# navi0105/LyricAlignment

Measured on AMD Instinct MI355X. Metric: aligned audio-sec/sec (RTF^-1), Whisper-medium 30 s clips, higher is better.
Workload: dtype bf16; 1 GPU; whisper-medium encoder + BiGRU/FC head + CTC forced alignment, batch 32 x 30 s mel per GPU (BASELINE.json configs[1]); clips_per_gpu=32, frames=1500, vocab=21129, labels_per_clip=5..26 (one per sung note), pipeline=2 encoder stream(s) + 1 head stream, head over 4 batches

## Files before the change

include/lyricalign.h:

```cpp
#ifndef LYRICALIGN_H
#define LYRICALIGN_H

#include <stddef.h>
#include <stdint.h>

#ifdef __cplusplus
extern "C" {
#endif

typedef enum la_status {
    LA_OK = 0,
    LA_EINVAL = 1,
    LA_EINFEASIBLE = 2,
    LA_EEMPTY = 3,
    LA_EHIP = 4,
    LA_ETIMEOUT = 5,
    LA_EUNSUPPORTED = 6
} la_status;

typedef enum la_dtype {
    LA_F32 = 0,
    LA_BF16 = 1,
    LA_F16 = 2
} la_dtype;

#define LA_Q_LOG2 0x100


typedef enum la_variant {
    LA_VARIANT_PLAIN = 0,
    LA_VARIANT_CTC = 1
} la_variant;

int la_version(void);
const char *la_last_error(void);
int la_device_arch_ok(void);

int la_timer_enable(const char *name);
int la_timer_disable(void);
int la_timer_read(double *total_ms, int64_t *launches);
int la_timer_reset(void);
int la_timer_sample(int32_t period);
int la_timer_read_work(double *total_ms, int64_t *timed_launches, double *timed_work, int64_t *all_launches);

int la_set_option(const char *name, int64_t value);
int la_get_option(const char *name, int64_t *value);
int la_has_experiments(void);

int la_viterbi_workspace_bytes(int32_t batch, int32_t max_frames, int32_t max_labels, size_t *bytes);

int la_viterbi_batch(const float *em, int64_t em_batch_stride, int64_t em_row_stride,
                     const int32_t *labels, int32_t labels_stride,
                     const int32_t *n_labels, const int32_t *n_frames,
                     int32_t batch, int32_t max_frames, int32_t max_labels,
                     int32_t *onset, int32_t *offset, int32_t out_stride,
                     double *final_score, int32_t *status,
                     void *workspace, size_t workspace_bytes, void *stream);

int la_viterbi_core(const float *em, int64_t em_row_stride, const int32_t *labels, int32_t n_labels_host,
                    int32_t n_frames_host, const int32_t *n_labels, const int32_t *n_frames,
                    double *dp, long long *bt, int32_t *scratch_i32, double *scratch_f64,
                    void *workspace, size_t workspace_bytes, void *stream);

int la_viterbi_spans_workspace_bytes(int32_t batch, int32_t max_frames, int32_t max_labels, size_t *bytes);

int la_viterbi_spans_batch(const float *em, int64_t em_batch_stride, int64_t em_row_stride,
                           const int32_t *labels, int32_t labels_stride,
                           const int32_t *n_labels, const int32_t *n_frames,
                           int32_t batch, int32_t max_frames, int32_t max_labels,
                           int32_t *onset, int32_t *offset, int32_t out_stride,
                           double *final_score, int32_t *status,
                           const int32_t *skip_from, int32_t skip_stride, double skip_penalty,
                           void *workspace, size_t workspace_bytes, void *stream);

int la_viterbi_windows_workspace_bytes(int32_t batch, int32_t max_frames, int32_t max_labels, size_t *bytes);

int la_viterbi_windows_batch(const float *em, int64_t em_batch_stride, int64_t em_row_stride,
                             const int32_t *labels, int32_t labels_stride,
                             const int32_t *n_labels, const int32_t *n_frames,
// ... 166 lines not shown
                               int32_t vocab, const int32_t *labels, int32_t labels_stride, const int32_t *n_labels,
                               const int32_t *n_frames, int32_t max_labels, const int32_t *skip_from, int32_t skip_stride,
                               double skip_penalty, const int32_t *win_lo, const int32_t *win_hi, int32_t win_stride, float scale,
                               float *loss, double *nll, int32_t *status, float *dlogits, int64_t d_batch_stride,
                               int64_t d_row_stride, void *workspace, size_t workspace_bytes, void *stream);

int la_grad_sqnorm_f32(const float *grad, int64_t n, double *sum_sq, void *stream);
int la_adamw_step_f32(float *param, const float *grad, float *exp_avg, float *exp_avg_sq, int64_t n, float lr,
                      float beta1, float beta2, float eps, float weight_decay, int32_t step,
                      const double *clip_sum_sq, float max_norm, float grad_prescale, void *stream);

int la_gru_layer_train_fwd(const float *gi, const float *w_hh, const float *b_hh, float *out, float *gates,
                           int32_t batch, int32_t frames, int32_t hidden, void *workspace, size_t workspace_bytes,
                           int32_t *timeout_flag, void *stream);
int la_gru_layer_bwd(const float *gates, const float *out, const float *dout, const float *w_hh, float *dgi, float *dgh,
                     int32_t batch, int32_t frames, int32_t hidden, void *workspace, size_t workspace_bytes,
                     int32_t *timeout_flag, void *stream);
int la_transpose_pad_f32(const float *in, int64_t ld_in, int32_t rows, int32_t cols, float *out, int64_t ld_out,
                         int32_t out_rows, int32_t out_cols, void *stream);
int la_colsum_f32(const float *in, int64_t ld, int32_t rows, int32_t cols, float *out, void *stream);
int la_mish_f32(const float *x, float *y, int64_t n, void *stream);
int la_mish_bwd_f32(const float *x, const float *dy, float *dx, int64_t n, void *stream);
int la_mask_scale_f32(const float *x, const unsigned char *mask, float scale, float *y, int64_t n, void *stream);

int la_gemm_fused_ln(int32_t dtype, int32_t M, int32_t N, int32_t K, int32_t batch, const void *A, int64_t lda, int64_t strideA,
                     const void *W, void *C, int64_t ldc, int64_t strideC, const float *bias, const float *residual, int64_t ldr,
                     int64_t strideR, int32_t epilogue, void *C2, int64_t ldc2, int64_t strideC2, const float *ln_stats,
                     const float *ln_csum, float *ln_part, void *stream);
int la_gemm_split(int32_t dtype, int32_t M, int32_t N, int32_t K, int32_t batch, const void *A, int64_t lda, int64_t strideA,
                  const void *W, void *hi, void *lo, int64_t ld, int64_t stride, const float *bias, const float *residual,
                  int64_t ldr, int64_t strideR, int32_t epilogue, float *ln_part, void *stream);
int la_layernorm_split(int32_t dtype, const void *hi, const void *lo, int64_t ldx, int32_t M, int32_t d, const float *gamma,
                       const float *beta, void *y, int64_t ldy, int32_t out_dtype, void *stream);
int la_ln_stats_finalize(const float *part, int32_t slots, int32_t M, float eps, float *stats, void *stream);
int la_row_stats16(int32_t dtype, const void *x, int64_t ldx, int32_t M, int32_t d, float eps, float *stats, void *stream);

int la_split_f16x2(const float *x, int64_t ldx, int32_t rows, int32_t cols, void *planes, int64_t kp, float *inv_scale, void *stream);
int la_split_f16x2_t(const float *x, int64_t ldx, int32_t rows, int32_t cols, void *planes_t, int64_t mp, float *inv_scale_t, void *stream);
int la_split_f16x2_act(const float *x, int64_t ldx, int32_t rows, int32_t cols, void *planes, int64_t kp, float *inv_scale, int32_t act, void *stream);
int la_split_f16x2_t_act(const float *x, int64_t ldx, int32_t rows, int32_t cols, void *planes_t, int64_t mp, float *inv_scale_t, int32_t act, void *stream);
int la_split_f16x2_t_colsum(const float *x, int64_t ldx, int32_t rows, int32_t cols, void *planes_t, int64_t mp, float *inv_scale_t, int32_t act,
                            float *colsum, void *stream);
int la_split_f16x2_max(const float *x, int64_t ldx, int32_t rows, int32_t cols, void *planes, int64_t kp, float *inv_scale, int32_t act,
                       uint32_t *tmax, void *stream);
int la_split_f16x2_t_tmax(const float *x, int64_t ldx, int32_t rows, int32_t cols, void *planes_t, int64_t mp, float *inv_scale_t, int32_t act,
                          float *colsum, const uint32_t *tmax, void *stream);
int la_gemm_f16x2(int32_t M, int32_t N, int32_t K, int32_t slots, const void *A, const float *sa, const void *W, const float *sw,
                  float *C, int64_t ldc, const float *bias, const float *residual, int64_t ldr, int32_t epilogue, void *stream);
int la_gemm_f16x2_small(int32_t M, int32_t N, int32_t K, int32_t slots, const void *A, const float *sa, const void *W, const float *sw,
                        float *C, int64_t ldc, const float *bias, const float *residual, int64_t ldr, int32_t epilogue, void *stream);
int la_gemm_f16x2_small_slots(int32_t M, int32_t N, int32_t K);
int la_layernorm_f16x2(const float *x, int64_t ldx, int32_t rows, int32_t d, const float *gamma, const float *beta, void *planes, int64_t kp,
                       float *inv_scale, void *stream);

int la_gemm_ex(int32_t dtype, int32_t M, int32_t N, int32_t K, int32_t batch, const void *A, int64_t lda, int64_t strideA,
               const void *W, int64_t ldw, int64_t strideW, void *C, int64_t ldc, int64_t strideC, const float *bias,
               int32_t epilogue, void *stream);
int la_transpose_pad_batched_f32(const float *in, int64_t ld_in, int64_t batch_stride_in, int32_t rows, int32_t cols,
                                 float *out, int64_t ld_out, int64_t batch_stride_out, int32_t out_rows, int32_t out_cols,
                                 int32_t batch, void *stream);
int la_gelu_f32(const float *x, float *y, int64_t n, void *stream);
int la_gelu_bwd_f32(const float *x, const float *dy, float *dx, int64_t n, void *stream);
int la_add_f32(const float *a, const float *b, float *y, int64_t n, void *stream);
int la_scale_f32(const float *x, float alpha, float *y, int64_t n, void *stream);
int la_layernorm_bwd_f32(const float *x, const float *dy, const float *gamma, int32_t M, int32_t d, float *dx, float *dy_xhat,
                         void *stream);
int la_layernorm_bwd_sums_f32(const float *x, const float *dy, const float *gamma, const float *residual, int32_t M, int32_t d, float *dx,
                              float *dgamma, float *dbeta, float *scratch, void *stream);
int la_softmax_rows_f32(float *s, int64_t ld, int64_t rows, int32_t cols, int32_t causal_q_len, void *stream);
int la_softmax_bwd_rows_f32(const float *p, float *dp, int64_t ld, int64_t rows, int32_t cols, void *stream);
int la_attention_bwd_workspace_bytes(int32_t batch, int32_t q_len, int32_t n_head, size_t *bytes);
int la_attention_bwd_f32(const float *q, int64_t ld_q, const float *k, const float *v, int64_t ld_kv, const float *o, int64_t ld_o,
                         const float *dout, int64_t ld_do, float *dq, int64_t ld_dq, float *dk, float *dv, int64_t ld_dkv,
                         int32_t batch, int32_t q_len, int32_t kv_len, int32_t n_head, int32_t causal, const float *lse,
                         void *workspace, size_t workspace_bytes, void *stream);
int la_attention_bwd_stats_f32(const float *q, int64_t ld_q, const float *k, int64_t ld_kv, const float *o, int64_t ld_o, const float *dout,
                               int64_t ld_do, int32_t batch, int32_t q_len, int32_t kv_len, int32_t n_head, int32_t causal,
                               const float *lse_in, float *lse, float *dvec, void *stream);
int la_attention_lse_f32(const float *q, int64_t ld_q, const float *k, const float *v, int64_t ld_kv, float *out, int64_t ld_out,
                         int32_t batch, int32_t q_len, int32_t kv_len, int32_t n_head, int32_t causal, float *lse, void *stream);
int la_attention_f16x2_workspace_bytes(int32_t batch, int32_t q_len, int32_t kv_len, int32_t n_head, size_t *bytes);
int la_attention_lse_f16x2(const float *q, int64_t ld_q, const float *k, const float *v, int64_t ld_kv, float *out, int64_t ld_out,
                           int32_t batch, int32_t q_len, int32_t kv_len, int32_t n_head, int32_t causal, float *lse, void *workspace,
                           size_t workspace_bytes, void *stream);
int la_attention_bwd_f16x2_workspace_bytes(int32_t batch, int32_t q_len, int32_t kv_len, int32_t n_head, size_t *bytes);
int la_attention_bwd_f16x2(const float *q, int64_t ld_q, const float *k, const float *v, int64_t ld_kv, const float *o, int64_t ld_o,
                           const float *dout, int64_t ld_do, float *dq, int64_t ld_dq, float *dk, float *dv, int64_t ld_dkv,
                           int32_t batch, int32_t q_len, int32_t kv_len, int32_t n_head, int32_t causal, const float *lse,
                           void *workspace, size_t workspace_bytes, void *stream);
int la_embed_tokens_bwd_f32(const float *dx, const int64_t *tokens, int32_t batch, int32_t n, int32_t d, int32_t n_vocab, float *dtok,
                            float *dpos, void *stream);
int la_cross_entropy_f32(const float *logits, int64_t ld, int32_t rows, int32_t vocab, const int64_t *target, float scale,
                         float *loss2, float *row_ws, float *dlogits, int64_t ld_d, void *stream);
int la_col2im3_f32(const float *dcols, int32_t batch, int32_t t_out, int32_t stride, int32_t channels, float *out,
                   int32_t rows_out, void *stream);

int la_resample_poly_f32(const float *x, int64_t n_in, const float *h, int64_t h_len, int32_t up, int32_t down,
                         int64_t skip, float *y, int64_t n_out, void *stream);

int la_cast_f32_to_bf16(const float *x, void *y, int64_t n, void *stream);
int la_cast_bf16_to_f32(const void *x, float *y, int64_t n, void *stream);

typedef struct la_encoder_block {
    const float *ln1_g, *ln1_b;
    const void *wqkv; const float *bqkv;
    const void *wo; const float *bo;
    const float *ln2_g, *ln2_b;
    const void *w1; const float *b1;
    const void *w2; const float *b2;
    const void *wqkv_ln; const float *cqkv, *bqkv_ln;
    const void *w1_ln; const float *c1, *b1_ln;
    const void *wqkv_x2; const float *wqkv_x2s;
    const void *wo_x2; const float *wo_x2s;
    const void *w1_x2; const float *w1_x2s;
    const void *w2_x2; const float *w2_x2s;
} la_encoder_block;

typedef struct la_encoder_weights {
    int32_t dtype, d, n_head, n_layer, n_mels;
    const void *conv1_w; const float *conv1_b;
    const void *conv2_w; const float *conv2_b;
    const float *pos;
    const float *lnp_g, *lnp_b;
    const la_encoder_block *blocks;
} la_encoder_weights;

int la_encoder_workspace_bytes(const la_encoder_weights *w, int32_t batch, size_t *bytes);
int la_encoder_forward(const la_encoder_weights *w, const float *mel, int64_t mel_batch_stride, int64_t mel_row_stride,
                       int32_t batch, void *out, int64_t ld_out, int32_t out_dtype, void *workspace, size_t workspace_bytes,
                       void *stream);

typedef struct la_head_weights {
    int32_t dtype, hidden, in_dim, vocab, n_layers;
    const void *w_ih[2]; const float *b_ih[2];
    const void *w_hh[2]; const float *b_hh[2];
    const void *w_fc; const float *b_fc;
    const void *w_ih_x2[2]; const float *w_ih_x2s[2];
    const void *w_fc_x2; const float *w_fc_x2s;
} la_head_weights;

int la_align_head_workspace_bytes(const la_head_weights *w, int32_t batch, int32_t frames, int32_t max_labels, size_t *bytes);
int la_align_head_forward(const la_head_weights *w, const void *feats, int64_t ld_feats, int64_t clip_stride_rows,
                          int32_t batch, int32_t frames, int32_t variant, const int32_t *labels, int32_t labels_stride,
                          const int32_t *n_labels, int32_t max_labels, int32_t *onset, int32_t *offset, int32_t out_stride,
                          double *final_score, int32_t *status, float *emissions_out, void *workspace, size_t workspace_bytes,
                          int32_t *timeout_flag, void *stream);
int la_align_head_forward_ragged(const la_head_weights *w, const void *feats, int64_t ld_feats, int64_t clip_stride_rows,
                                 int32_t batch, int32_t frames, const int32_t *n_frames, int32_t variant, const int32_t *labels,
                                 int32_t labels_stride, const int32_t *n_labels, int32_t max_labels, int32_t *onset, int32_t *offset,
                                 int32_t out_stride, double *final_score, int32_t *status, float *emissions_out, void *workspace,
                                 size_t workspace_bytes, int32_t *timeout_flag, void *stream);

#ifdef __cplusplus
}
#endif
#endif
```

lyricalignment_amd/_lib.py:

```python
from __future__ import annotations

import ctypes
import os
from ctypes import POINTER, c_char_p, c_double, c_int32, c_int64, c_size_t, c_void_p

import torch

HERE = os.path.dirname(os.path.abspath(__file__))
LIB_PATH = os.environ.get("LA_LIB_PATH") or os.path.join(HERE, "liblyricalign_hip.so")

LA_OK, LA_EINVAL, LA_EINFEASIBLE, LA_EEMPTY, LA_EHIP, LA_ETIMEOUT, LA_EUNSUPPORTED = range(7)
LA_F32, LA_BF16, LA_F16 = 0, 1, 2
LA_Q_LOG2 = 0x100
LA_VARIANT_PLAIN, LA_VARIANT_CTC = 0, 1
EPI_BIAS, EPI_GELU, EPI_RESIDUAL, EPI_OUT_F32, EPI_MISH = 1, 2, 4, 8, 16
EPI_GELU_ERF = 4096
EPI_RES_GELU_GRAD = 32
GEMM_TRANS_A, GEMM_TRANS_W = 512, 1024

_I32, _I64, _P, _SZ = c_int32, c_int64, c_void_p, c_size_t
SYMBOLS = {
    "la_version": (c_int32, []),
    "la_last_error": (c_char_p, []),
    "la_device_arch_ok": (c_int32, []),
    "la_timer_enable": (c_int32, [c_char_p]),
    "la_timer_disable": (c_int32, []),
    "la_timer_read": (c_int32, [POINTER(c_double), POINTER(c_int64)]),
    "la_timer_reset": (c_int32, []),
    "la_timer_sample": (c_int32, [c_int32]),
    "la_timer_read_work": (c_int32, [POINTER(c_double), POINTER(c_int64), POINTER(c_double), POINTER(c_int64)]),
    "la_split_f16x2": (c_int32, [_P, _I64, _I32, _I32, _P, _I64, _P, _P]),
    "la_split_f16x2_t": (c_int32, [_P, _I64, _I32, _I32, _P, _I64, _P, _P]),
    "la_split_f16x2_act": (c_int32, [_P, _I64, _I32, _I32, _P, _I64, _P, _I32, _P]),
    "la_split_f16x2_t_act": (c_int32, [_P, _I64, _I32, _I32, _P, _I64, _P, _I32, _P]),
    "la_split_f16x2_t_colsum": (c_int32, [_P, _I64, _I32, _I32, _P, _I64, _P, _I32, _P, _P]),
    "la_split_f16x2_max": (c_int32, [_P, _I64, _I32, _I32, _P, _I64, _P, _I32, _P, _P]),
    "la_split_f16x2_t_tmax": (c_int32, [_P, _I64, _I32, _I32, _P, _I64, _P, _I32, _P, _P, _P]),
    "la_gemm_f16x2": (c_int32, [_I32, _I32, _I32, _I32, _P, _P, _P, _P, _P, _I64, _P, _P, _I64, _I32, _P]),
    "la_gemm_f16x2_small": (c_int32, [_I32, _I32, _I32, _I32, _P, _P, _P, _P, _P, _I64, _P, _P, _I64, _I32, _P]),
    "la_gemm_f16x2_small_slots": (c_int32, [_I32, _I32, _I32]),
    "la_layernorm_f16x2": (c_int32, [_P, _I64, _I32, _I32, _P, _P, _P, _I64, _P, _P]),
    "la_fc_emissions_x2_workspace_bytes": (c_int32, [_I32, _I32, _I32, _I32, _I32, POINTER(_SZ)]),
    "la_fc_emissions_x2": (c_int32, [_P, _I64, _P, _P, _P, _P, _I32, _I32, _I32, _I32, _I32, _P, _I32, _P, _I32, _P, _I64, _I64, _P, _SZ, _P]),
    "la_set_option": (c_int32, [c_char_p, c_int64]),
    "la_get_option": (c_int32, [c_char_p, POINTER(c_int64)]),
    "la_has_experiments": (c_int32, []),
    "la_viterbi_workspace_bytes": (c_int32, [_I32, _I32, _I32, POINTER(_SZ)]),
    "la_viterbi_batch": (c_int32, [_P, _I64, _I64, _P, _I32, _P, _P, _I32, _I32, _I32, _P, _P, _I32, _P, _P, _P, _SZ, _P]),
    "la_viterbi_core": (c_int32, [_P, _I64, _P, _I32, _I32, _P, _P, _P, _P, _P, _P, _P, _SZ, _P]),
    "la_viterbi_spans_workspace_bytes": (c_int32, [_I32, _I32, _I32, POINTER(_SZ)]),
    "la_viterbi_spans_batch": (c_int32, [_P, _I64, _I64, _P, _I32, _P, _P, _I32, _I32, _I32, _P, _P, _I32, _P, _P, _P, _I32, c_double,
                                         _P, _SZ, _P]),
    "la_viterbi_windows_workspace_bytes": (c_int32, [_I32, _I32, _I32, POINTER(_SZ)]),
    "la_viterbi_windows_batch": (c_int32, [_P, _I64, _I64, _P, _I32, _P, _P, _I32, _I32, _I32, _P, _P, _I32, _P, _P, _P, _I32, c_double,
                                           _P, _P, _I32, _P, _SZ, _P]),
    "la_viterbi_lattice_workspace_bytes": (c_int32, [_I32, _I32, _I32, POINTER(_SZ)]),
    "la_viterbi_lattice_batch": (c_int32, [_P, _I64, _I64, _P, _I32, _P, _P, _I32, _I32, _I32, _P, _P, _I32, _P, _P, _P, _I32, c_double,
                                           _P, _P, _I32, _P, _SZ, _P]),
    "la_alignment_posteriors_workspace_bytes": (c_int32, [_I32, _I32, _I32, POINTER(_SZ)]),
    "la_alignment_posteriors": (c_int32, [_P, _I64, _I64, _P, _I32, _P, _P, _I32, _I32, _I32, _P, _P, _I32, _I32, _P, _P, _P, _P, _P,
                                          _P, _I64, _I64, _P, _SZ, _P]),
    "la_alignment_posteriors_spans_workspace_bytes": (c_int32, [_I32, _I32, _I32, POINTER(_SZ)]),
    "la_alignment_posteriors_spans": (c_int32, [_P, _I64, _I64, _P, _I32, _P, _P, _I32, _I32, _I32, _P, _P, _I32, _I32, _P, _I32, c_double,
                                                _P, _P, _P, _P, _P, _P, _P, _P, _I64, _I64, _P, _SZ, _P]),
    "la_alignment_posteriors_windows_workspace_bytes": (c_int32, [_I32, _I32, _I32, POINTER(_SZ)]),
    "la_alignment_posteriors_windows": (c_int32, [_P, _I64, _I64, _P, _I32, _P, _P, _I32, _I32, _I32, _P, _P, _I32, _I32, _P, _I32, c_double,
                                                  _P, _P, _I32, _P, _P, _P, _P, _P, _P, _P, _P, _I64, _I64, _P, _SZ, _P]),
    "la_emissions_from_logits": (c_int32, [_P, _I64, _I64, _I32, _I32, _I32, _I32, _P, _I32, _P, _I32, _P, _I64, _I64, _P]),
    "la_logmel_workspace_bytes": (c_int32, [_I32, _I32, POINTER(_SZ)]),
    "la_logmel_f32": (c_int32, [_P, _I32, _I32, _P, _P, _P, _I64, _I64, _P, _SZ, _P]),
    "la_logmel_constants_bytes": (c_int32, [POINTER(_SZ)]),
    "la_logmel_constants": (c_int32, [_P, _P, _P, _SZ, _P]),
    "la_logmel_f32_prepared": (c_int32, [_P, _I32, _I32, _P, _P, _I64, _I64, _P, _SZ, _P]),
    "la_gemm": (c_int32, [_I32, _I32, _I32, _I32, _I32, _P, _I64, _I64, _P, _P, _I64, _I64, _P, _P, _I64, _I64, _I32, _P]),
    "la_layernorm": (c_int32, [_P, _I64, _I32, _I32, _P, _P, _P, _I64, _I32, _P]),
    "la_attention": (c_int32, [_I32, _P, _I64, _P, _I64, _I32, _I32, _I32, _P]),
    "la_attention_ex": (c_int32, [_I32, _P, _I64, _P, _P, _I64, _P, _I64, _I32, _I32, _I32, _I32, _I32, _P]),
    "la_embed_tokens": (c_int32, [_P, _I32, _I32, _P, _I32, _P, _I32, _P, _P]),
    "la_mel_to_rows": (c_int32, [_P, _I64, _I64, _I32, _I32, _I32, _P, _I32, _I32, _P]),
    "la_gru_workspace_bytes": (c_int32, [_I32, _I32, _I32, POINTER(_SZ)]),
    "la_gru_layer": (c_int32, [_I32, _P, _P, _P, _P, _P, _I32, _I32, _I32, _P, _SZ, _P, _P]),
    "la_fc_emissions_workspace_bytes": (c_int32, [_I32, _I32, _I32, _I32, _I32, _I32, POINTER(_SZ)]),
    "la_fc_emissions": (c_int32, [_I32, _P, _I64, _P, _P, _I32, _I32, _I32, _I32, _I32, _P, _I32, _P, _I32, _P, _I64, _I64, _P, _SZ, _P]),
    "la_multitask_loss_workspace_bytes": (c_int32, [_I32, _I32, _I32, POINTER(_SZ)]),
    "la_multitask_loss": (c_int32, [_P, _I64, _I64, _I32, _I32, _I32, _P, _P, _I32, _P, _I32, _I32, _I32, ctypes.c_float, _P, _P, _I64, _I64, _P, _SZ, _P]),
    "la_anchored_alignment_loss_workspace_bytes": (c_int32, [_I32, _I32, _I32, POINTER(_SZ)]),
    "la_anchored_alignment_loss": (c_int32, [_P, _I64, _I64, _I32, _I32, _I32, _P, _I32, _P, _P, _I32, _P, _I32, c_double, _P, _P, _I32,
                                             ctypes.c_float, _P, _P, _P, _P, _I64, _I64, _P, _SZ, _P]),
    "la_grad_sqnorm_f32": (c_int32, [_P, _I64, _P, _P]),
    "la_adamw_step_f32": (c_int32, [_P, _P, _P, _P, _I64, ctypes.c_float, ctypes.c_float, ctypes.c_float, ctypes.c_float, ctypes.c_float, _I32, _P, ctypes.c_float, ctypes.c_float, _P]),
    "la_gru_layer_train_fwd": (c_int32, [_P, _P, _P, _P, _P, _I32, _I32, _I32, _P, _SZ, _P, _P]),
    "la_gru_layer_bwd": (c_int32, [_P, _P, _P, _P, _P, _P, _I32, _I32, _I32, _P, _SZ, _P, _P]),
    "la_transpose_pad_f32": (c_int32, [_P, _I64, _I32, _I32, _P, _I64, _I32, _I32, _P]),
    "la_colsum_f32": (c_int32, [_P, _I64, _I32, _I32, _P, _P]),
# ... 9 lines not shown
    "la_gemm_split": (c_int32, [_I32, _I32, _I32, _I32, _I32, _P, _I64, _I64, _P, _P, _P, _I64, _I64, _P, _P, _I64, _I64, _I32, _P, _P]),
    "la_layernorm_split": (c_int32, [_I32, _P, _P, _I64, _I32, _I32, _P, _P, _P, _I64, _I32, _P]),
    "la_row_stats16": (c_int32, [_I32, _P, _I64, _I32, _I32, ctypes.c_float, _P, _P]),
    "la_gemm_ex": (c_int32, [_I32, _I32, _I32, _I32, _I32, _P, _I64, _I64, _P, _I64, _I64, _P, _I64, _I64, _P, _I32, _P]),
    "la_transpose_pad_batched_f32": (c_int32, [_P, _I64, _I64, _I32, _I32, _P, _I64, _I64, _I32, _I32, _I32, _P]),
    "la_gelu_f32": (c_int32, [_P, _P, _I64, _P]),
    "la_gelu_bwd_f32": (c_int32, [_P, _P, _P, _I64, _P]),
    "la_add_f32": (c_int32, [_P, _P, _P, _I64, _P]),
    "la_scale_f32": (c_int32, [_P, ctypes.c_float, _P, _I64, _P]),
    "la_layernorm_bwd_f32": (c_int32, [_P, _P, _P, _I32, _I32, _P, _P, _P]),
    "la_layernorm_bwd_sums_f32": (c_int32, [_P, _P, _P, _P, _I32, _I32, _P, _P, _P, _P, _P]),
    "la_softmax_rows_f32": (c_int32, [_P, _I64, _I64, _I32, _I32, _P]),
    "la_attention_bwd_workspace_bytes": (c_int32, [_I32, _I32, _I32, POINTER(_SZ)]),
    "la_attention_bwd_stats_f32": (c_int32, [_P, _I64, _P, _I64, _P, _I64, _P, _I64, _I32, _I32, _I32, _I32, _I32, _P, _P, _P, _P]),
    "la_attention_bwd_f32": (c_int32, [_P, _I64, _P, _P, _I64, _P, _I64, _P, _I64, _P, _I64, _P, _P, _I64, _I32, _I32, _I32, _I32, _I32, _P, _P,
                                       _SZ, _P]),
    "la_attention_lse_f32": (c_int32, [_P, _I64, _P, _P, _I64, _P, _I64, _I32, _I32, _I32, _I32, _I32, _P, _P]),
    "la_attention_f16x2_workspace_bytes": (c_int32, [_I32, _I32, _I32, _I32, POINTER(_SZ)]),
    "la_attention_lse_f16x2": (c_int32, [_P, _I64, _P, _P, _I64, _P, _I64, _I32, _I32, _I32, _I32, _I32, _P, _P, _SZ, _P]),
    "la_attention_bwd_f16x2_workspace_bytes": (c_int32, [_I32, _I32, _I32, _I32, POINTER(_SZ)]),
    "la_attention_bwd_f16x2": (c_int32, [_P, _I64, _P, _P, _I64, _P, _I64, _P, _I64, _P, _I64, _P, _P, _I64, _I32, _I32, _I32, _I32, _I32, _P, _P,
                                         _SZ, _P]),
    "la_embed_tokens_bwd_f32": (c_int32, [_P, _P, _I32, _I32, _I32, _I32, _P, _P, _P]),
    "la_cross_entropy_f32": (c_int32, [_P, _I64, _I32, _I32, _P, ctypes.c_float, _P, _P, _P, _I64, _P]),
    "la_softmax_bwd_rows_f32": (c_int32, [_P, _P, _I64, _I64, _I32, _P]),
    "la_col2im3_f32": (c_int32, [_P, _I32, _I32, _I32, _I32, _P, _I32, _P]),
    "la_resample_poly_f32": (c_int32, [_P, _I64, _P, _I64, _I32, _I32, _I64, _P, _I64, _P]),
    "la_cast_f32_to_bf16": (c_int32, [_P, _P, _I64, _P]),
    "la_encoder_workspace_bytes": (c_int32, [_P, _I32, POINTER(_SZ)]),
    "la_encoder_forward": (c_int32, [_P, _P, _I64, _I64, _I32, _P, _I64, _I32, _P, _SZ, _P]),
    "la_align_head_workspace_bytes": (c_int32, [_P, _I32, _I32, _I32, POINTER(_SZ)]),
    "la_align_head_forward": (c_int32, [_P, _P, _I64, _I64, _I32, _I32, _I32, _P, _I32, _P, _I32, _P, _P, _I32, _P, _P, _P, _P, _SZ, _P, _P]),
    "la_cast_bf16_to_f32": (c_int32, [_P, _P, _I64, _P]),
    "la_logmel_ragged_workspace_bytes": (c_int32, [_I32, _I32, POINTER(_SZ)]),
    "la_logmel_ragged_f32_prepared": (c_int32, [_P, _P, _I32, _I32, _P, _P, _I64, _I64, _I32, _P, _SZ, _P]),
    "la_gru_layer_ragged": (c_int32, [_I32, _P, _P, _P, _P, _P, _I32, _I32, _P, _I32, _P, _SZ, _P, _P]),
    "la_align_head_forward_ragged": (c_int32, [_P, _P, _I64, _I64, _I32, _I32, _P, _I32, _P, _I32, _P, _I32, _P, _P, _I32, _P, _P, _P, _P, _SZ, _P, _P]),
}

LAB_SYMBOLS = {}




class EncoderBlockC(ctypes.Structure):
    _fields_ = [(n, c_void_p) for n in ("ln1_g", "ln1_b", "wqkv", "bqkv", "wo", "bo", "ln2_g", "ln2_b", "w1", "b1", "w2", "b2",
                                        "wqkv_ln", "cqkv", "bqkv_ln", "w1_ln", "c1", "b1_ln",
                                        "wqkv_x2", "wqkv_x2s", "wo_x2", "wo_x2s", "w1_x2", "w1_x2s", "w2_x2", "w2_x2s")]


class EncoderWeightsC(ctypes.Structure):
    _fields_ = [("dtype", c_int32), ("d", c_int32), ("n_head", c_int32), ("n_layer", c_int32), ("n_mels", c_int32),
                ("conv1_w", c_void_p), ("conv1_b", c_void_p), ("conv2_w", c_void_p), ("conv2_b", c_void_p), ("pos", c_void_p),
                ("lnp_g", c_void_p), ("lnp_b", c_void_p), ("blocks", POINTER(EncoderBlockC))]


class HeadWeightsC(ctypes.Structure):
    _fields_ = [("dtype", c_int32), ("hidden", c_int32), ("in_dim", c_int32), ("vocab", c_int32), ("n_layers", c_int32),
                ("w_ih", c_void_p * 2), ("b_ih", c_void_p * 2), ("w_hh", c_void_p * 2), ("b_hh", c_void_p * 2),
                ("w_fc", c_void_p), ("b_fc", c_void_p),
                ("w_ih_x2", c_void_p * 2), ("w_ih_x2s", c_void_p * 2), ("w_fc_x2", c_void_p), ("w_fc_x2s", c_void_p)]


_lib = None


class LyricAlignHipError(RuntimeError):
    pass


def lib() -> ctypes.CDLL:
    global _lib
    if _lib is None:
        if not os.path.exists(LIB_PATH):
            raise LyricAlignHipError(
                f"{LIB_PATH} is missing: the HIP extension is the product path and has no fallback. "
                "Build it with `python -m lyricalignment_amd.build`.")
        L = ctypes.CDLL(LIB_PATH)
        for name, (res, args) in SYMBOLS.items():
            fn = getattr(L, name)
            fn.restype = res
            fn.argtypes = args
        if L.la_has_experiments():
            for name, (res, args) in LAB_SYMBOLS.items():
                fn = getattr(L, name)
                fn.restype = res
                fn.argtypes = args
        _lib = L
    return _lib


def last_error() -> str:
    msg = lib().la_last_error()
    return msg.decode() if msg else ""


def check(rc: int, what: str = "") -> None:
    if rc == LA_OK:
        return
    detail = f"{what}: {last_error()}" if what else last_error()
    if rc == LA_EINVAL:
        raise ValueError(f"liblyricalign_hip invalid argument: {detail}")
    if rc == LA_EUNSUPPORTED:
        raise NotImplementedError(f"liblyricalign_hip unsupported shape: {detail}")
    if rc == LA_ETIMEOUT:
        raise TimeoutError(f"liblyricalign_hip in-kernel wait timed out: {detail}")
    raise LyricAlignHipError(f"liblyricalign_hip status {rc}: {detail}")
# ... 57 lines not shown
```

lyricalignment_amd/csrc/la_attention_f16x2.hip:

```cpp
#include <type_traits>

#include "la_x2.h"

namespace {

typedef __attribute__((ext_vector_type(16))) float f32x16;
typedef __attribute__((ext_vector_type(8))) _Float16 f16x8;
typedef __attribute__((ext_vector_type(4))) short s16x4;
typedef __attribute__((ext_vector_type(8))) short s16x8;

#ifndef LA_X2F_KO
#define LA_X2F_KO 0
#endif
constexpr int KT = 64;
constexpr int IMG = KT * 128;
constexpr float kLog2e = 1.4426950408889634f;
constexpr float kLn2 = 0.6931471805599453f;

struct FwdParams {
    const unsigned short *qp, *kp, *vp;
    const float *sq, *sk, *sv;
    float *out;
    int64_t ld_out;
    float *lse;
    int q_len, kv_len, n_head, causal, batch;
};

__global__ __launch_bounds__(1024) void heads_split_kernel(const float *x, int64_t ld, int T, int H, unsigned short *planes, float *inv_scale) {
    __shared__ float red[16];
    const int head = blockIdx.x, clip = blockIdx.y, tid = threadIdx.x;
    const int c4 = tid & 15, r0 = tid >> 4;
    const float *src = x + (int64_t)clip * T * ld + head * 64 + c4 * 4;
    constexpr int NV = 24;
    const bool cached = T <= 64 * NV;
    float4 v[NV];
    float mx = 0.f;
    if (cached) {
#pragma unroll
        for (int j = 0; j < NV; ++j) {
            const int r = r0 + 64 * j;
            v[j] = make_float4(0.f, 0.f, 0.f, 0.f);
            if (r < T) v[j] = *reinterpret_cast<const float4 *>(src + (int64_t)r * ld);
        }
#pragma unroll
        for (int j = 0; j < NV; ++j) mx = fmaxf(mx, fmaxf(fmaxf(fabsf(v[j].x), fabsf(v[j].y)), fmaxf(fabsf(v[j].z), fabsf(v[j].w))));
    } else {
        for (int r = r0; r < T; r += 64) {
            const float4 w = *reinterpret_cast<const float4 *>(src + (int64_t)r * ld);
            mx = fmaxf(mx, fmaxf(fmaxf(fabsf(w.x), fabsf(w.y)), fmaxf(fabsf(w.z), fabsf(w.w))));
        }
    }
#pragma unroll
    for (int o = 1; o < 64; o <<= 1) mx = fmaxf(mx, __shfl_xor(mx, o));
    if ((tid & 63) == 0) red[tid >> 6] = mx;
    __syncthreads();
    mx = red[0];
#pragma unroll
    for (int i = 1; i < 16; ++i) mx = fmaxf(mx, red[i]);
    float inv;
    const float s = la::x2::scale_for(mx, &inv);
    if (tid == 0 && blockIdx.z == 0) inv_scale[clip * H + head] = inv;
    const int64_t C = 64 * (int64_t)H;
    const int parts = gridDim.z, part = blockIdx.z;
    unsigned short *dst = planes + (int64_t)clip * T * 2 * C + head * 64 + c4 * 4;
    auto put = [&](int r, const float4 &w) {
        const unsigned a = la::x2::pack_hi_lo(w.x * s), b = la::x2::pack_hi_lo(w.y * s), c = la::x2::pack_hi_lo(w.z * s), d = la::x2::pack_hi_lo(w.w * s);
        *reinterpret_cast<uint2 *>(dst + (int64_t)r * 2 * C) = make_uint2((a & 0xffffu) | (b << 16), (c & 0xffffu) | (d << 16));
        *reinterpret_cast<uint2 *>(dst + (int64_t)r * 2 * C + C) = make_uint2((a >> 16) | (b & 0xffff0000u), (c >> 16) | (d & 0xffff0000u));
    };
    if (cached) {
#pragma unroll
        for (int j = 0; j < NV; ++j) {
            const int r = r0 + 64 * j;
            if (r < T && j % parts == part) put(r, v[j]);
        }
    } else {
        for (int r = r0, j = 0; r < T; r += 64, ++j)
            if (j % parts == part) put(r, *reinterpret_cast<const float4 *>(src + (int64_t)r * ld));
// ... 2 lines not shown

struct BlockCoord { int qt, head, clip; };
__device__ __forceinline__ BlockCoord block_coord(int nq, int n_head, int batch) {
    const int L = blockIdx.x, pairs = n_head * batch;
    int pair, qt;
    if ((pairs & 7) == 0) {
        const int x = L & 7, idx = L >> 3;
        pair = x + 8 * (idx / nq);
        qt = idx % nq;
    } else {
        pair = L / nq;
        qt = L % nq;
    }
    return BlockCoord{qt, pair % n_head, pair / n_head};
}
__device__ __forceinline__ int acc_row(int reg, int h) { return (reg & 3) + 8 * (reg >> 2) + 4 * h; }
__device__ __forceinline__ int kswz(int r) { return (r >> 1) & 7; }
__device__ __forceinline__ int vswz(int r) { return ((r >> 1) & 1) << 2; }
__device__ __forceinline__ f32x16 mfma(f16x8 a, f16x8 b, f32x16 c) { return __builtin_amdgcn_mfma_f32_32x32x16_f16(a, b, c, 0, 0, 0); }

template <int PER> struct KvOff { unsigned k[PER], v[PER]; };
template <int PER>
__device__ __forceinline__ KvOff<PER> kv_offsets(int64_t C, int key0, int T, int wave, int lane) {
    KvOff<PER> o;
#pragma unroll
    for (int i = 0; i < PER; ++i) {
        const int r = (wave * PER + i) * 8 + (lane >> 3), ps = lane & 7;
        const int rr = key0 + r < T ? r : T - 1 - key0;
        o.k[i] = (unsigned)(rr * C * 4) + ((ps ^ kswz(r)) << 4);
        o.v[i] = (unsigned)(rr * C * 4) + ((ps ^ vswz(r)) << 4);
    }
    return o;
}
template <int PER>
__device__ __forceinline__ void stage_tile(const unsigned short *base, int64_t C, int key0, const unsigned (&off)[PER], unsigned buf, int wave) {
    const unsigned short *src = base + (int64_t)key0 * 2 * C;
#pragma unroll
    for (int i = 0; i < PER; ++i) {
        const unsigned piece = (wave * PER + i) * 1024;
        la::glds16_so(off[i], src, buf + piece);
        la::glds16_so(off[i], src + C, buf + IMG + piece);
    }
}

__device__ __forceinline__ void split_pair(float a, float b, unsigned &hi, unsigned &lo) {
    typedef _Float16 h2 __attribute__((ext_vector_type(2)));
    const h2 hv = {(_Float16)a, (_Float16)b};
    hi = __builtin_bit_cast(unsigned, hv);
    asm("s_nop 0\n\tv_fma_mixlo_f16 %0, %1, -1.0, %2 op_sel_hi:[1,0,0]\n\ts_nop 0\n\tv_fma_mixhi_f16 %0, %1, -1.0, %3 op_sel:[1,0,0] op_sel_hi:[1,0,0]\n\ts_nop 1"
        : "=&v"(lo)
        : "v"(hi), "v"(a), "v"(b));
}

template <int NW>
__global__ __launch_bounds__(64 * NW, 2) void attention_x2_fwd_kernel(FwdParams p) {
    constexpr int QT = 32 * NW, PER = 8 / NW;
    __shared__ __attribute__((aligned(16))) unsigned char lds[8 * IMG];
    const int T = p.kv_len;
    const int64_t C = 64 * (int64_t)p.n_head;
    const BlockCoord bc = block_coord((p.q_len + QT - 1) / QT, p.n_head, p.batch);
    const int qt = bc.qt, head = bc.head, clip = bc.clip;
    const int tid = threadIdx.x, lane = tid & 63;
    const int wave = __builtin_amdgcn_readfirstlane(tid >> 6);
    const int i32 = lane & 31, h = lane >> 5;
    const unsigned short *kbase = p.kp + (int64_t)clip * T * 2 * C + head * 64;
    const unsigned short *vbase = p.vp + (int64_t)clip * T * 2 * C + head * 64;
    const int bh = clip * p.n_head + head;
    const float kScale = p.sq[bh] * p.sk[bh] * kLog2e;

    int qrow = qt * QT + wave * 32 + i32;
    const bool q_valid = qrow < p.q_len;
    qrow = q_valid ? qrow : p.q_len - 1;
    uint4 qh[4], ql[4];
    {
        const unsigned short *qb = p.qp + ((int64_t)clip * p.q_len + qrow) * 2 * C + head * 64 + 8 * h;
#pragma unroll
        for (int c = 0; c < 4; ++c) {
            qh[c] = *reinterpret_cast<const uint4 *>(qb + 16 * c);
            ql[c] = *reinterpret_cast<const uint4 *>(qb + C + 16 * c);
        }
    }
    f32x16 o[2];
#pragma unroll
    for (int b = 0; b < 2; ++b)
#pragma unroll
        for (int r = 0; r < 16; ++r) o[b][r] = 0.f;
    float m_run = -INFINITY, l_part = 0.f;

    int nkv = (T + KT - 1) / KT;
    const int nkv_all = nkv;
    if (p.causal) nkv = min(nkv, (min(p.q_len, (qt + 1) * QT) - 1) / KT + 1);
    const unsigned lds0 = __builtin_amdgcn_readfirstlane(la::lds_addr_u32(lds));
    const KvOff<PER> off_full = kv_offsets<PER>(C, 0, KT, wave, lane);
    const KvOff<PER> off_last = kv_offsets<PER>(C, (nkv_all - 1) * KT, T, wave, lane);
    auto stage = [&](int t, unsigned buf) __attribute__((always_inline)) {
        stage_tile<PER>(kbase, C, t * KT, t == nkv_all - 1 ? off_last.k : off_full.k, buf, wave);
        stage_tile<PER>(vbase, C, t * KT, t == nkv_all - 1 ? off_last.v : off_full.v, buf + 2 * IMG, wave);
    };
    stage(0, lds0);
    asm volatile("s_waitcnt vmcnt(0)" ::: "memory");
#pragma unroll
    for (int c = 0; c < 4; ++c) {
        typedef unsigned u32x4 __attribute__((ext_vector_type(4)));
        u32x4 t0 = __builtin_bit_cast(u32x4, qh[c]), t1 = __builtin_bit_cast(u32x4, ql[c]);
        asm volatile("" : "+v"(t0), "+v"(t1));
        qh[c] = __builtin_bit_cast(uint4, t0);
        ql[c] = __builtin_bit_cast(uint4, t1);
// ... 87 lines not shown
                for (int r = 0; r < 16; ++r) o[b][r] *= alpha;
        }
#pragma unroll
        for (int sub = 0; sub < 2; ++sub)
#pragma unroll
            for (int ks = 0; ks < 2; ++ks) {
                uint4 ph, pl;
                split_pair(s[sub][8 * ks + 0], s[sub][8 * ks + 1], ph.x, pl.x);
                split_pair(s[sub][8 * ks + 2], s[sub][8 * ks + 3], ph.y, pl.y);
                split_pair(s[sub][8 * ks + 4], s[sub][8 * ks + 5], ph.z, pl.z);
                split_pair(s[sub][8 * ks + 6], s[sub][8 * ks + 7], ph.w, pl.w);
                const f16x8 phv = __builtin_bit_cast(f16x8, ph), plv = __builtin_bit_cast(f16x8, pl);
#pragma unroll
                for (int b = 0; b < 2; ++b) {
                    const int key0 = sub * 32 + 16 * ks + 4 * (g >> 1);
                    const int slot = b * 4 + 2 * (g & 1) + (pp >> 1);
                    const int r0 = key0 + q4, r1 = key0 + 8 + q4;
                    const int a0 = r0 * 128 + ((slot ^ vswz(r0)) << 4) + (pp & 1) * 8, a1 = r1 * 128 + ((slot ^ vswz(r1)) << 4) + (pp & 1) * 8;
                    typedef __attribute__((address_space(3))) s16x4 *lds_s16x4;
                    f16x8 vh, vlo;
                    if constexpr (LA_X2F_KO & 2) {
                        vh = __builtin_bit_cast(f16x8, qh[(2 * sub + ks + b) & 3]);
                        vlo = __builtin_bit_cast(f16x8, ql[(2 * sub + ks + b) & 3]);
                    } else {
                        const s16x4 h0 = __builtin_amdgcn_ds_read_tr16_b64_v4i16((lds_s16x4)(vl + a0)), h1 = __builtin_amdgcn_ds_read_tr16_b64_v4i16((lds_s16x4)(vl + a1));
                        const s16x4 l0 = __builtin_amdgcn_ds_read_tr16_b64_v4i16((lds_s16x4)(vl + IMG + a0)), l1 = __builtin_amdgcn_ds_read_tr16_b64_v4i16((lds_s16x4)(vl + IMG + a1));
                        vh = __builtin_bit_cast(f16x8, __builtin_shufflevector(h0, h1, 0, 1, 2, 3, 4, 5, 6, 7));
                        vlo = __builtin_bit_cast(f16x8, __builtin_shufflevector(l0, l1, 0, 1, 2, 3, 4, 5, 6, 7));
                    }
                    if constexpr (LA_X2F_KO & 16) {
                        o[b][2 * sub + ks] += (float)vh[0] + (float)vlo[7] + (float)phv[0] + (float)plv[7];
                    } else {
                        o[b] = mfma(vlo, phv, o[b]);
                        o[b] = mfma(vh, plv, o[b]);
                        o[b] = mfma(vh, phv, o[b]);
                    }
                }
            }
        asm volatile("s_waitcnt vmcnt(0)" ::: "memory");
        if constexpr (!(LA_X2F_KO & 32)) __syncthreads();
    };
    auto step = [&](int t, auto curc) __attribute__((always_inline)) {
        if (__builtin_expect((t + 1) * KT > T || p.causal, 0)) tile(t, curc, std::true_type{});
        else tile(t, curc, std::false_type{});
    };
    for (int t = 0; t < nkv; t += 2) {
        step(t, std::integral_constant<int, 0>{});
        if (t + 1 < nkv) step(t + 1, std::integral_constant<int, 1>{});
    }

    const float l = l_part + __shfl_xor(l_part, 32);
    const float inv = p.sv[bh] / l;
    if (p.lse && q_valid && h == 0) p.lse[((int64_t)clip * p.n_head + head) * p.q_len + qrow] = fmaf(m_run - 13.0f, kLn2, __logf(l));
    if (q_valid) {
        float *orow = p.out + ((int64_t)clip * p.q_len + qrow) * p.ld_out + head * 64;
#pragma unroll
        for (int b = 0; b < 2; ++b)
#pragma unroll
            for (int r4 = 0; r4 < 4; ++r4)
                *reinterpret_cast<float4 *>(orow + 32 * b + 8 * r4 + 4 * h) =
                    make_float4(o[b][4 * r4 + 0] * inv, o[b][4 * r4 + 1] * inv, o[b][4 * r4 + 2] * inv, o[b][4 * r4 + 3] * inv);
    }
}

struct BwdParams {
    const unsigned short *qp, *kp, *vp, *dop;
    const float *sq, *sk, *sv, *sdo;
    const float *lse, *dvec;
    float *dq, *dk, *dv;
    int64_t ld_dq, ld_dkv;
    int q_len, kv_len, n_head, causal, batch;
};

__device__ __forceinline__ f16x8 row_frag(const unsigned char *img, int row, int c, int h) {
    return __builtin_bit_cast(f16x8, *reinterpret_cast<const uint4 *>(img + row * 128 + (((2 * c + h) ^ kswz(row)) << 4)));
}
struct TrLane { int g, q4, pp; };
__device__ __forceinline__ f16x8 tr_frag(const unsigned char *img, int tok0, int b, const TrLane &L) {
    const int key0 = tok0 + 4 * (L.g >> 1);
    const int slot = b * 4 + 2 * (L.g & 1) + (L.pp >> 1);
    const int r0 = key0 + L.q4, r1 = key0 + 8 + L.q4;
    typedef __attribute__((address_space(3))) s16x4 *lds_s16x4;
    const s16x4 v0 = __builtin_amdgcn_ds_read_tr16_b64_v4i16((lds_s16x4)(img + r0 * 128 + ((slot ^ vswz(r0)) << 4) + (L.pp & 1) * 8));
    const s16x4 v1 = __builtin_amdgcn_ds_read_tr16_b64_v4i16((lds_s16x4)(img + r1 * 128 + ((slot ^ vswz(r1)) << 4) + (L.pp & 1) * 8));
    return __builtin_bit_cast(f16x8, __builtin_shufflevector(v0, v1, 0, 1, 2, 3, 4, 5, 6, 7));
}
__device__ __forceinline__ f32x16 mma3(f16x8 ah, f16x8 al, f16x8 bh, f16x8 bl, f32x16 acc) {
    acc = mfma(al, bh, acc);
    acc = mfma(ah, bl, acc);
    return mfma(ah, bh, acc);
}
__device__ __forceinline__ void split8(const f32x16 &s, int ks, f16x8 &hi, f16x8 &lo) {
    uint4 ph, pl;
    split_pair(s[8 * ks + 0], s[8 * ks + 1], ph.x, pl.x);
    split_pair(s[8 * ks + 2], s[8 * ks + 3], ph.y, pl.y);
    split_pair(s[8 * ks + 4], s[8 * ks + 5], ph.z, pl.z);
    split_pair(s[8 * ks + 6], s[8 * ks + 7], ph.w, pl.w);
    hi = __builtin_bit_cast(f16x8, ph);
    lo = __builtin_bit_cast(f16x8, pl);
}

constexpr int BWD_NW = 8;
constexpr int KV_BUF = 8 * IMG;
constexpr int KV_LDS = 2 * KV_BUF + 2 * 2 * 64 * 4;
constexpr int Q_BUF = 6 * IMG;
constexpr int Q_LDS = 2 * Q_BUF;

// ... 300 lines not shown
    const int64_t row = item / H;
    const int head = (int)(item % H);
    const float4 a = *reinterpret_cast<const float4 *>(o + row * ld_o + head * 64 + part * 4);
    const float4 g = *reinterpret_cast<const float4 *>(dout + row * ld_do + head * 64 + part * 4);
    float s = (a.x * g.x + a.y * g.y) + (a.z * g.z + a.w * g.w);
    s += __shfl_xor(s, 1); s += __shfl_xor(s, 2); s += __shfl_xor(s, 4); s += __shfl_xor(s, 8);
    if (part == 0) dvec[((int64_t)(row / Tq) * H + head) * Tq + row % Tq] = s;
}

struct FwdWorkspace {
    unsigned short *qp, *kp, *vp;
    float *sq, *sk, *sv;
    size_t bytes;
};
FwdWorkspace fwd_workspace(void *base, int B, int Tq, int Tk, int H) {
    auto up = [](size_t x) { return (x + 255) & ~(size_t)255; };
    const size_t C = 64 * (size_t)H;
    size_t off = 0;
    auto take = [&](size_t n) { size_t o = off; off += up(n); return o; };
    const size_t oq = take((size_t)B * Tq * 2 * C * 2), ok = take((size_t)B * Tk * 2 * C * 2), ov = take((size_t)B * Tk * 2 * C * 2);
    const size_t osq = take((size_t)B * H * 4), osk = take((size_t)B * H * 4), osv = take((size_t)B * H * 4);
    char *b = reinterpret_cast<char *>(base);
    return FwdWorkspace{reinterpret_cast<unsigned short *>(b + oq), reinterpret_cast<unsigned short *>(b + ok), reinterpret_cast<unsigned short *>(b + ov),
                        reinterpret_cast<float *>(b + osq), reinterpret_cast<float *>(b + osk), reinterpret_cast<float *>(b + osv), off};
}

}

extern "C" int la_attention_f16x2_workspace_bytes(int32_t batch, int32_t q_len, int32_t kv_len, int32_t n_head, size_t *bytes) {
    LA_CHECK_ARG(bytes && batch >= 0 && q_len >= 0 && kv_len >= 0 && n_head > 0, "attention_f16x2_workspace_bytes: bad arguments");
    *bytes = fwd_workspace(nullptr, batch, q_len, kv_len, n_head).bytes;
    return LA_OK;
}

extern "C" int la_attention_lse_f16x2(const float *q, int64_t ld_q, const float *k, const float *v, int64_t ld_kv, float *out, int64_t ld_out,
                                      int32_t batch, int32_t q_len, int32_t kv_len, int32_t n_head, int32_t causal, float *lse, void *workspace,
                                      size_t workspace_bytes, void *stream_) {
    hipStream_t stream = (hipStream_t)stream_;
    if (batch == 0 || q_len == 0) return LA_OK;
    LA_CHECK_ARG(q && k && v && out && batch > 0 && q_len > 0 && kv_len > 0 && n_head > 0, "attention_lse_f16x2: bad arguments");
    LA_CHECK_ARG(!causal || q_len == kv_len, "attention_lse_f16x2: causal masking is defined for self-attention (q_len == kv_len)");
    LA_CHECK_ARG(ld_q >= n_head * 64 && ld_kv >= n_head * 64 && ld_out >= n_head * 64, "attention_lse_f16x2: leading dimensions too small");
    LA_CHECK_ARG(ld_q % 4 == 0 && ld_kv % 4 == 0 && ld_out % 4 == 0 && (uintptr_t)q % 16 == 0 && (uintptr_t)k % 16 == 0 && (uintptr_t)v % 16 == 0 &&
                     (uintptr_t)out % 16 == 0, "attention_lse_f16x2: rows must be 16-byte aligned");
    const FwdWorkspace ws = fwd_workspace(workspace, batch, q_len, kv_len, n_head);
    LA_CHECK_ARG(workspace && (uintptr_t)workspace % 256 == 0 && workspace_bytes >= ws.bytes, "attention_lse_f16x2: workspace missing, misaligned or too small");
    la::TimerScope ts("attention_f16x2", stream);
    const dim3 sgrid = heads_split_grid(n_head, batch);
    hipLaunchKernelGGL(heads_split_kernel, sgrid, dim3(1024), 0, stream, q, ld_q, q_len, n_head, ws.qp, ws.sq);
    hipLaunchKernelGGL(heads_split_kernel, sgrid, dim3(1024), 0, stream, k, ld_kv, kv_len, n_head, ws.kp, ws.sk);
    hipLaunchKernelGGL(heads_split_kernel, sgrid, dim3(1024), 0, stream, v, ld_kv, kv_len, n_head, ws.vp, ws.sv);
    FwdParams p{ws.qp, ws.kp, ws.vp, ws.sq, ws.sk, ws.sv, out, ld_out, lse, q_len, kv_len, n_head, causal ? 1 : 0, batch};
    hipLaunchKernelGGL((attention_x2_fwd_kernel<8>), dim3(la::cdiv(q_len, 256) * n_head * batch), dim3(512), 0, stream, p);
    LA_LAUNCH_CHECK();
    return LA_OK;
}

namespace {
struct BwdWorkspace {
    unsigned short *qp, *kp, *vp, *dop;
    float *sq, *sk, *sv, *sdo, *lse, *dvec;
    size_t bytes;
};
BwdWorkspace bwd_workspace(void *base, int B, int Tq, int Tk, int H) {
    auto up = [](size_t x) { return (x + 255) & ~(size_t)255; };
    const size_t C = 64 * (size_t)H;
    size_t off = 0;
    auto take = [&](size_t n) { size_t o = off; off += up(n); return o; };
    const size_t oq = take((size_t)B * Tq * 2 * C * 2), ok = take((size_t)B * Tk * 2 * C * 2), ov = take((size_t)B * Tk * 2 * C * 2),
                 og = take((size_t)B * Tq * 2 * C * 2);
    const size_t osq = take((size_t)B * H * 4), osk = take((size_t)B * H * 4), osv = take((size_t)B * H * 4), osg = take((size_t)B * H * 4);
    const size_t ol = take((size_t)B * H * Tq * 4), od = take((size_t)B * H * Tq * 4);
    char *b = reinterpret_cast<char *>(base);
    auto us = [&](size_t o) { return reinterpret_cast<unsigned short *>(b + o); };
    auto fl = [&](size_t o) { return reinterpret_cast<float *>(b + o); };
    return BwdWorkspace{us(oq), us(ok), us(ov), us(og), fl(osq), fl(osk), fl(osv), fl(osg), fl(ol), fl(od), off};
}
}

extern "C" int la_attention_bwd_stats_f32(const float *q, int64_t ld_q, const float *k, int64_t ld_kv, const float *o, int64_t ld_o, const float *dout,
                                          int64_t ld_do, int32_t batch, int32_t q_len, int32_t kv_len, int32_t n_head, int32_t causal,
                                          const float *lse_in, float *lse, float *dvec, void *stream);

extern "C" int la_attention_bwd_f16x2_workspace_bytes(int32_t batch, int32_t q_len, int32_t kv_len, int32_t n_head, size_t *bytes) {
    LA_CHECK_ARG(bytes && batch >= 0 && q_len >= 0 && kv_len >= 0 && n_head > 0, "attention_bwd_f16x2_workspace_bytes: bad arguments");
    *bytes = bwd_workspace(nullptr, batch, q_len, kv_len, n_head).bytes;
    return LA_OK;
}

extern "C" int la_attention_bwd_f16x2(const float *q, int64_t ld_q, const float *k, const float *v, int64_t ld_kv, const float *o, int64_t ld_o,
                                      const float *dout, int64_t ld_do, float *dq, int64_t ld_dq, float *dk, float *dv, int64_t ld_dkv,
                                      int32_t batch, int32_t q_len, int32_t kv_len, int32_t n_head, int32_t causal, const float *lse,
                                      void *workspace, size_t workspace_bytes, void *stream_) {
    hipStream_t stream = (hipStream_t)stream_;
    if (batch == 0 || q_len == 0 || kv_len == 0) return LA_OK;
    LA_CHECK_ARG(q && k && v && o && dout && dq && dk && dv && workspace, "attention_bwd_f16x2: null pointer");
    LA_CHECK_ARG(batch > 0 && q_len > 0 && kv_len > 0 && n_head > 0, "attention_bwd_f16x2: bad sizes");
    LA_CHECK_ARG(!causal || q_len == kv_len, "attention_bwd_f16x2: the causal mask needs q_len == kv_len");
    LA_CHECK_ARG(ld_q % 4 == 0 && ld_kv % 4 == 0 && ld_o % 4 == 0 && ld_do % 4 == 0 && ld_dq % 4 == 0 && ld_dkv % 4 == 0 &&
                     ld_q >= n_head * 64 && ld_kv >= n_head * 64 && ld_o >= n_head * 64 && ld_do >= n_head * 64 && ld_dq >= n_head * 64 &&
                     ld_dkv >= n_head * 64, "attention_bwd_f16x2: leading dimensions must be multiples of 4 and at least n_head * 64");
    LA_CHECK_ARG(((uintptr_t)q | (uintptr_t)k | (uintptr_t)v | (uintptr_t)o | (uintptr_t)dout | (uintptr_t)dq | (uintptr_t)dk | (uintptr_t)dv) % 16 == 0,
                 "attention_bwd_f16x2: operands must be 16-byte aligned");
    const BwdWorkspace ws = bwd_workspace(workspace, batch, q_len, kv_len, n_head);
    LA_CHECK_ARG((uintptr_t)workspace % 256 == 0 && workspace_bytes >= ws.bytes, "attention_bwd_f16x2: workspace misaligned or too small");
    static la::DeviceOnce attr_once;
// ... 29 lines not shown
```

lyricalignment_amd/csrc/la_common.h:

```cpp
#pragma once
#include <hip/hip_runtime.h>
#include <stdint.h>
#include <stdio.h>
#include <stdlib.h>
#include <string.h>

#include "../../include/lyricalign.h"

namespace la {

char *err_buf();
void set_error(const char *fmt, ...);

enum { SCRATCH_SPLITK = 0, SCRATCH_COLSUM = 1, SCRATCH_X2 = 2 };
void *stream_scratch(hipStream_t stream, int purpose, size_t bytes);

#define LA_CHECK_ARG(cond, ...)                \
    do {                                       \
        if (!(cond)) {                         \
            la::set_error(__VA_ARGS__);        \
            return LA_EINVAL;                  \
        }                                      \
    } while (0)

#define LA_HIP(expr)                                                                     \
    do {                                                                                 \
        hipError_t _e = (expr);                                                          \
        if (_e != hipSuccess) {                                                          \
            la::set_error("%s:%d %s -> %s", __FILE__, __LINE__, #expr, hipGetErrorString(_e)); \
            return LA_EHIP;                                                              \
        }                                                                                \
    } while (0)

#define LA_LAUNCH_CHECK()                                                               \
    do {                                                                                \
        hipError_t _e = hipGetLastError();                                              \
        if (_e != hipSuccess) {                                                         \
            la::set_error("%s:%d launch -> %s", __FILE__, __LINE__, hipGetErrorString(_e)); \
            return LA_EHIP;                                                             \
        }                                                                               \
    } while (0)

struct Options {
    int gemm_tile = 0, gemm_loop = 0, gemm_splitk = 1, attn_nw = 0, gru_nw = 0, gru_fence = 0, gru_handoff = 0, gru_poll_delay = 0, viterbi_dpp = 1,
        head_clip_cap = 0, ln_fusion = 1, resid_split = 1, x2_inference = 1, gru_timeout_us = 0, gru_fault_step = 0, x2_small = 0;
};
Options &opts();
#ifdef LA_EXPERIMENTS
inline const char *dev_env(const char *name) { return getenv(name); }
#define LA_DEV_BIT(word, bits) ((word) & (bits))
#else
inline const char *dev_env(const char *) { return nullptr; }
#define LA_DEV_BIT(word, bits) false
#endif

struct DeviceOnce {
    unsigned long long done[4] = {0, 0, 0, 0};
    static int current() {
        int d = 0;
        if (hipGetDevice(&d) != hipSuccess) d = 0;
        return d & 255;
    }
    bool pending() const {
        const int d = current();
        return !((__atomic_load_n(&done[d >> 6], __ATOMIC_ACQUIRE) >> (d & 63)) & 1ull);
    }
    void mark() {
        const int d = current();
        __atomic_fetch_or(&done[d >> 6], 1ull << (d & 63), __ATOMIC_RELEASE);
    }
};

struct TimerScope {
    bool active;
    hipStream_t stream;
    TimerScope(const char *family, hipStream_t s, double work = 0.0);
    ~TimerScope();
};

int gemm_run(int dtype, int M, int N, int K, int batch, const void *A, int64_t lda, int64_t strideA, const void *W,
             int64_t strideW, void *C, int64_t ldc, int64_t strideC, const float *bias, int64_t strideBias,
             const float *residual, int64_t ldr, int64_t strideR, int epilogue, hipStream_t stream);

inline int64_t round_up(int64_t x, int64_t m) { return (x + m - 1) / m * m; }
inline int cdiv(int64_t a, int64_t b) { return (int)((a + b - 1) / b); }

typedef unsigned short bf16_t;

__device__ __forceinline__ float bf16_to_f32(bf16_t v) { return __uint_as_float(((unsigned)v) << 16); }

__device__ __forceinline__ bf16_t f32_to_bf16(float f) {
    __bf16 b = (__bf16)f;
    return __builtin_bit_cast(unsigned short, b);
}

typedef _Float16 f16_t;

template <typename T> struct Pack4;
// ... 158 lines not shown
```

lyricalignment_amd/csrc/la_f32x2.hip:

```cpp
#include <algorithm>

#include "la_gemm_core.h"
#include "la_gemm_epilogue.h"
#include "la_gemm_params.h"

using namespace la::gemm;

namespace {

__device__ __forceinline__ float x2_scale(float mx, float *inv) {
    if (!(mx > 0.f) || !(mx < 3.0e38f)) { *inv = 1.f; return 1.f; }
    int e;
    (void)frexpf(mx, &e);
    int sh = 14 - e;
    sh = sh > 126 ? 126 : (sh < -126 ? -126 : sh);
    *inv = ldexpf(1.f, -sh);
    return ldexpf(1.f, sh);
}

__device__ __forceinline__ void x2_split(float xs, unsigned short &hi, unsigned short &lo) {
    const _Float16 h = (_Float16)xs;
    const _Float16 l = (_Float16)(xs - (float)h);
    hi = __builtin_bit_cast(unsigned short, h);
    lo = __builtin_bit_cast(unsigned short, l);
}

__device__ __forceinline__ float x2_act(float v, int act) { return act == 1 ? la::gelu_erf(v) : v; }

__global__ __launch_bounds__(256) void split_rows_kernel(const float *x, int64_t ldx, int rows, int cols, unsigned short *planes, int64_t kp,
                                                         float *inv_scale, int act, unsigned *tmax) {
    const int lane = threadIdx.x & 63;
    const int row = blockIdx.x * 4 + (threadIdx.x >> 6);
    if (row >= rows) return;
    const float *xr = x + (int64_t)row * ldx;
    const bool vec = (ldx % 4 == 0) && ((uintptr_t)x % 16 == 0);
    const int c4 = vec ? cols / 4 : 0;
    unsigned short *hi = planes + (int64_t)row * 2 * kp, *lo = hi + kp;
    float mx = 0.f;
    constexpr int NV = 16;
    const bool cached = c4 <= 64 * NV;
    float4 v[NV];
    if (cached) {
#pragma unroll
        for (int j = 0; j < NV; ++j) {
            const int i = lane + 64 * j;
            v[j] = make_float4(0.f, 0.f, 0.f, 0.f);
            if (i < c4) v[j] = reinterpret_cast<const float4 *>(xr)[i];
        }
#pragma unroll
        for (int j = 0; j < NV; ++j) {
            if (act) v[j] = make_float4(x2_act(v[j].x, act), x2_act(v[j].y, act), x2_act(v[j].z, act), x2_act(v[j].w, act));
            mx = fmaxf(mx, fmaxf(fmaxf(fabsf(v[j].x), fabsf(v[j].y)), fmaxf(fabsf(v[j].z), fabsf(v[j].w))));
        }
    } else {
        for (int i = lane; i < c4; i += 64) {
            const float4 w = reinterpret_cast<const float4 *>(xr)[i];
            mx = fmaxf(mx, fmaxf(fmaxf(fabsf(x2_act(w.x, act)), fabsf(x2_act(w.y, act))), fmaxf(fabsf(x2_act(w.z, act)), fabsf(x2_act(w.w, act)))));
        }
    }
    for (int i = c4 * 4 + lane; i < cols; i += 64) mx = fmaxf(mx, fabsf(x2_act(xr[i], act)));
#pragma unroll
    for (int o = 32; o > 0; o >>= 1) mx = fmaxf(mx, __shfl_xor(mx, o));
    float inv;
    const float s = x2_scale(mx, &inv);
    if (tmax && lane == 0) atomicMax(tmax + (row & 63) * 32, __float_as_uint(mx != mx ? __uint_as_float(0x7f800000u) : mx));
    if (cached) {
#pragma unroll
        for (int j = 0; j < NV; ++j) {
            const int i = lane + 64 * j;
            if (i < c4) {
                ushort4 h, l;
                x2_split(v[j].x * s, h.x, l.x); x2_split(v[j].y * s, h.y, l.y); x2_split(v[j].z * s, h.z, l.z); x2_split(v[j].w * s, h.w, l.w);
                reinterpret_cast<ushort4 *>(hi)[i] = h;
                reinterpret_cast<ushort4 *>(lo)[i] = l;
            }
        }
    } else {
        for (int i = lane; i < c4; i += 64) {
            const float4 w = reinterpret_cast<const float4 *>(xr)[i];
            ushort4 h, l;
            x2_split(x2_act(w.x, act) * s, h.x, l.x); x2_split(x2_act(w.y, act) * s, h.y, l.y); x2_split(x2_act(w.z, act) * s, h.z, l.z);
            x2_split(x2_act(w.w, act) * s, h.w, l.w);
            reinterpret_cast<ushort4 *>(hi)[i] = h;
            reinterpret_cast<ushort4 *>(lo)[i] = l;
        }
    }
    for (int i = c4 * 4 + lane; i < kp; i += 64) {
        unsigned short h = 0, l = 0;
        if (i < cols) x2_split(x2_act(xr[i], act) * s, h, l);
        hi[i] = h; lo[i] = l;
    }
    if (lane == 0) inv_scale[row] = inv;
}

__global__ __launch_bounds__(256) void ln_split_rows_kernel(const float *x, int64_t ldx, int rows, int d, const float *gamma, const float *beta,
                                                            unsigned short *planes, int64_t kp, float *inv_scale) {
    const int lane = threadIdx.x & 63;
    const int row = blockIdx.x * 4 + (threadIdx.x >> 6);
    if (row >= rows) return;
    const float *xr = x + (int64_t)row * ldx;
    constexpr int NV = 16;
    float4 v[NV];
    float sum = 0.f;
#pragma unroll
    for (int j = 0; j < NV; ++j) {
        const int c = (lane + 64 * j) * 4;
        v[j] = make_float4(0.f, 0.f, 0.f, 0.f);
        if (c < d) {
            v[j] = *reinterpret_cast<const float4 *>(xr + c);
            sum += (v[j].x + v[j].y) + (v[j].z + v[j].w);
        }
    }
#pragma unroll
    for (int o = 32; o > 0; o >>= 1) sum += __shfl_xor(sum, o);
    const float mean = sum / (float)d;
    float sq = 0.f;
#pragma unroll
    for (int j = 0; j < NV; ++j) {
        const int c = (lane + 64 * j) * 4;
        if (c < d) {
            const float a = v[j].x - mean, b = v[j].y - mean, c2 = v[j].z - mean, d2 = v[j].w - mean;
            sq += (a * a + b * b) + (c2 * c2 + d2 * d2);
        }
    }
#pragma unroll
    for (int o = 32; o > 0; o >>= 1) sq += __shfl_xor(sq, o);
    const float rstd = 1.0f / sqrtf(sq / (float)d + 1e-5f);
    float mx = 0.f;
#pragma unroll
    for (int j = 0; j < NV; ++j) {
        const int c = (lane + 64 * j) * 4;
        if (c < d) {
            const float4 g = *reinterpret_cast<const float4 *>(gamma + c), bt = *reinterpret_cast<const float4 *>(beta + c);
            v[j] = make_float4((v[j].x - mean) * rstd * g.x + bt.x, (v[j].y - mean) * rstd * g.y + bt.y, (v[j].z - mean) * rstd * g.z + bt.z,
                               (v[j].w - mean) * rstd * g.w + bt.w);
            mx = fmaxf(mx, fmaxf(fmaxf(fabsf(v[j].x), fabsf(v[j].y)), fmaxf(fabsf(v[j].z), fabsf(v[j].w))));
        }
    }
#pragma unroll
    for (int o = 32; o > 0; o >>= 1) mx = fmaxf(mx, __shfl_xor(mx, o));
    float inv;
    const float s = x2_scale(mx, &inv);
    unsigned short *hi = planes + (int64_t)row * 2 * kp, *lo = hi + kp;
#pragma unroll
    for (int j = 0; j < NV; ++j) {
        const int i = lane + 64 * j;
        if (i * 4 < d) {
            ushort4 h, l;
            x2_split(v[j].x * s, h.x, l.x); x2_split(v[j].y * s, h.y, l.y); x2_split(v[j].z * s, h.z, l.z); x2_split(v[j].w * s, h.w, l.w);
            reinterpret_cast<ushort4 *>(hi)[i] = h;
            reinterpret_cast<ushort4 *>(lo)[i] = l;
        }
    }
    for (int i = d + lane; i < kp; i += 64) { hi[i] = 0; lo[i] = 0; }
    if (lane == 0) inv_scale[row] = inv;
}

__global__ __launch_bounds__(256) void colmax_kernel(const float *x, int64_t ldx, int rows, int cols, int rows_per_block, unsigned *colmax, int act) {
    __shared__ float red[4][64];
    const int cx = threadIdx.x & 63, ry = threadIdx.x >> 6;
    const int col = blockIdx.x * 64 + cx;
    const int r0 = blockIdx.y * rows_per_block, r1 = min(rows, r0 + rows_per_block);
    float mx = 0.f;
    if (col < cols)
        for (int r = r0 + ry; r < r1; r += 4) mx = fmaxf(mx, fabsf(x2_act(x[(int64_t)r * ldx + col], act)));
    red[ry][cx] = mx;
    __syncthreads();
    if (ry == 0 && col < cols) {
        mx = fmaxf(fmaxf(red[0][cx], red[1][cx]), fmaxf(red[2][cx], red[3][cx]));
        if (mx != mx) mx = __uint_as_float(0x7f800000u);
        atomicMax(colmax + col, __float_as_uint(mx));
    }
}

template <bool SUMS>
__global__ __launch_bounds__(256) void colmax4_kernel(const float *x, int64_t ldx, int rows, int cols, int rows_per_block, unsigned *colmax, int act,
                                                      double *part) {
    __shared__ float4 red[4][64];
    __shared__ double reds[SUMS ? 4 : 1][SUMS ? 64 : 1][4];
    double sm[4] = {0.0, 0.0, 0.0, 0.0};
    const int cx = threadIdx.x & 63, ry = threadIdx.x >> 6;
    const int col = blockIdx.x * 256 + cx * 4;
    const int r0 = blockIdx.y * rows_per_block, r1 = min(rows, r0 + rows_per_block);
    float4 mx = make_float4(0.f, 0.f, 0.f, 0.f);
    auto take = [&](const float4 &v) {
        mx.x = fmaxf(mx.x, fabsf(x2_act(v.x, act))); mx.y = fmaxf(mx.y, fabsf(x2_act(v.y, act)));
        mx.z = fmaxf(mx.z, fabsf(x2_act(v.z, act))); mx.w = fmaxf(mx.w, fabsf(x2_act(v.w, act)));
        if constexpr (SUMS) { sm[0] += (double)v.x; sm[1] += (double)v.y; sm[2] += (double)v.z; sm[3] += (double)v.w; }
    };
    if (col < cols) {
        const float *p = x + col;
        int r = r0 + ry;
        for (; r + 12 < r1; r += 16) {
            const float4 a = *reinterpret_cast<const float4 *>(p + (int64_t)r * ldx), b = *reinterpret_cast<const float4 *>(p + (int64_t)(r + 4) * ldx);
            const float4 c = *reinterpret_cast<const float4 *>(p + (int64_t)(r + 8) * ldx), d = *reinterpret_cast<const float4 *>(p + (int64_t)(r + 12) * ldx);
            take(a); take(b); take(c); take(d);
        }
        for (; r < r1; r += 4) take(*reinterpret_cast<const float4 *>(p + (int64_t)r * ldx));
    }
    red[ry][cx] = mx;
    if constexpr (SUMS) {
#pragma unroll
        for (int e = 0; e < 4; ++e) reds[ry][cx][e] = sm[e];
    }
    __syncthreads();
    if (ry == 0 && col < cols) {
        if constexpr (SUMS) {
#pragma unroll
// ... 78 lines not shown
    if (i >= (int64_t)M * N) return;
    const int m = (int)(i / N), n = (int)(i - (int64_t)m * N);
    float v = 0.f;
    for (int s = 0; s < S; ++s) v += P[(int64_t)s * M * N + i];
    if ((epilogue & LA_EPI_BIAS) && bias) v += bias[n];
    if (epilogue & LA_EPI_GELU) v = la::gelu_erf(v);
    if ((epilogue & LA_EPI_RESIDUAL) && residual) {
        const float t = residual[(int64_t)m * ldr + n];
        v = (epilogue & LA_EPI_RES_GELU_GRAD) ? v * la::gelu_erf_grad(t) : v + t;
    }
    C[(int64_t)m * ldc + n] = v;
}

}

extern "C" int la_split_f16x2_max(const float *x, int64_t ldx, int32_t rows, int32_t cols, void *planes, int64_t kp, float *inv_scale,
                                  int32_t act, uint32_t *tmax, void *stream_) {
    if (rows == 0) return LA_OK;
    LA_CHECK_ARG(act == 0 || act == 1, "split_f16x2: act is 0 (none) or 1 (GELU)");
    LA_CHECK_ARG(x && planes && inv_scale && rows > 0 && cols > 0, "split_f16x2: bad arguments");
    LA_CHECK_ARG(kp >= cols && kp % 8 == 0 && ldx >= cols && (uintptr_t)planes % 16 == 0, "split_f16x2: kp must be >= cols and a multiple of 8, planes 16-byte aligned");
    hipStream_t stream = (hipStream_t)stream_;
    la::TimerScope ts("split_f16x2", stream, (double)rows * cols * 8.0);
    hipLaunchKernelGGL(split_rows_kernel, dim3(la::cdiv(rows, 4)), dim3(256), 0, stream, x, ldx, rows, cols,
                       reinterpret_cast<unsigned short *>(planes), kp, inv_scale, act, tmax);
    LA_LAUNCH_CHECK();
    return LA_OK;
}

extern "C" int la_split_f16x2_act(const float *x, int64_t ldx, int32_t rows, int32_t cols, void *planes, int64_t kp, float *inv_scale,
                                  int32_t act, void *stream_) {
    return la_split_f16x2_max(x, ldx, rows, cols, planes, kp, inv_scale, act, nullptr, stream_);
}

extern "C" int la_split_f16x2(const float *x, int64_t ldx, int32_t rows, int32_t cols, void *planes, int64_t kp, float *inv_scale, void *stream_) {
    return la_split_f16x2_act(x, ldx, rows, cols, planes, kp, inv_scale, 0, stream_);
}

extern "C" int la_layernorm_f16x2(const float *x, int64_t ldx, int32_t rows, int32_t d, const float *gamma, const float *beta, void *planes,
                                  int64_t kp, float *inv_scale, void *stream_) {
    if (rows == 0) return LA_OK;
    LA_CHECK_ARG(x && gamma && beta && planes && inv_scale && rows > 0, "layernorm_f16x2: bad arguments");
    LA_CHECK_ARG(d > 0 && d % 4 == 0 && d <= 4096 && ldx % 4 == 0 && ldx >= d && (uintptr_t)x % 16 == 0 && (uintptr_t)gamma % 16 == 0 && (uintptr_t)beta % 16 == 0,
                 "layernorm_f16x2: d=%d unsupported (a multiple of 4, at most 4096) or misaligned rows", d);
    LA_CHECK_ARG(kp >= d && kp % 8 == 0 && (uintptr_t)planes % 16 == 0, "layernorm_f16x2: kp must be >= d and a multiple of 8, planes 16-byte aligned");
    hipStream_t stream = (hipStream_t)stream_;
    la::TimerScope ts("split_f16x2", stream, (double)rows * d * 8.0);
    hipLaunchKernelGGL(ln_split_rows_kernel, dim3(la::cdiv(rows, 4)), dim3(256), 0, stream, x, ldx, rows, d, gamma, beta,
                       reinterpret_cast<unsigned short *>(planes), kp, inv_scale);
    LA_LAUNCH_CHECK();
    return LA_OK;
}

extern "C" int la_colsum_f32(const float *in, int64_t ld, int32_t rows, int32_t cols, float *out, void *stream);

extern "C" int la_split_f16x2_t_tmax(const float *x, int64_t ldx, int32_t rows, int32_t cols, void *planes_t, int64_t mp, float *inv_scale_t,
                                     int32_t act, float *colsum, const uint32_t *tmax, void *stream_) {
    if (cols == 0) return LA_OK;
    LA_CHECK_ARG(act == 0 || act == 1, "split_f16x2_t: act is 0 (none) or 1 (GELU)");
    LA_CHECK_ARG(!colsum || act == 0, "split_f16x2_t: column sums are those of x itself (act = 0)");
    LA_CHECK_ARG(x && planes_t && inv_scale_t && rows > 0 && cols > 0, "split_f16x2_t: bad arguments");
    LA_CHECK_ARG(mp >= rows && mp % 16 == 0 && ldx >= cols && (uintptr_t)planes_t % 16 == 0, "split_f16x2_t: mp must be >= rows and a multiple of 16, planes 16-byte aligned");
    hipStream_t stream = (hipStream_t)stream_;
    la::TimerScope ts("split_f16x2", stream, (double)rows * cols * 12.0);
    unsigned short *pl = reinterpret_cast<unsigned short *>(planes_t);
    const dim3 tgrid(la::cdiv(cols, 64), la::cdiv(mp, 64));
    if (tmax) {
        if (colsum) {
            double *part = static_cast<double *>(la::stream_scratch(stream, la::SCRATCH_COLSUM, sizeof(double) * (size_t)tgrid.y * cols));
            if (!part) { la::set_error("split_f16x2_t: scratch allocation failed"); return LA_EHIP; }
            hipLaunchKernelGGL((split_transposed_kernel<true, true>), tgrid, dim3(256), 0, stream, x, ldx, rows, cols, tmax, pl, mp, inv_scale_t, act, part);
            hipLaunchKernelGGL(colsum_blocks_kernel, dim3(la::cdiv(cols, 32)), dim3(256), 0, stream, part, (int)tgrid.y, cols, colsum);
        } else {
            hipLaunchKernelGGL((split_transposed_kernel<true, false>), tgrid, dim3(256), 0, stream, x, ldx, rows, cols, tmax, pl, mp, inv_scale_t, act,
                               (double *)nullptr);
        }
        LA_LAUNCH_CHECK();
        return LA_OK;
    }
    unsigned *colmax = static_cast<unsigned *>(la::stream_scratch(stream, la::SCRATCH_X2, (size_t)cols * sizeof(unsigned)));
    if (!colmax) { la::set_error("split_f16x2_t: scratch allocation failed"); return LA_EHIP; }
    LA_HIP(hipMemsetAsync(colmax, 0, (size_t)cols * sizeof(unsigned), stream));
    const int rpb = 512;
    if (cols % 4 == 0 && ldx % 4 == 0 && (uintptr_t)x % 16 == 0) {
        const dim3 grid(la::cdiv(cols, 256), la::cdiv(rows, 128));
        if (colsum) {
            double *part = static_cast<double *>(la::stream_scratch(stream, la::SCRATCH_COLSUM, sizeof(double) * (size_t)grid.y * cols));
            if (!part) { la::set_error("split_f16x2_t: scratch allocation failed"); return LA_EHIP; }
            hipLaunchKernelGGL(colmax4_kernel<true>, grid, dim3(256), 0, stream, x, ldx, rows, cols, 128, colmax, act, part);
            hipLaunchKernelGGL(colsum_blocks_kernel, dim3(la::cdiv(cols, 32)), dim3(256), 0, stream, part, (int)grid.y, cols, colsum);
        } else {
            hipLaunchKernelGGL(colmax4_kernel<false>, grid, dim3(256), 0, stream, x, ldx, rows, cols, 128, colmax, act, (double *)nullptr);
        }
    } else {
        hipLaunchKernelGGL(colmax_kernel, dim3(la::cdiv(cols, 64), la::cdiv(rows, rpb)), dim3(256), 0, stream, x, ldx, rows, cols, rpb, colmax, act);
        if (colsum) {
            const int rc = la_colsum_f32(x, ldx, rows, cols, colsum, stream_);
            if (rc != LA_OK) return rc;
        }
    }
    LA_LAUNCH_CHECK();
    hipLaunchKernelGGL((split_transposed_kernel<false, false>), tgrid, dim3(256), 0, stream, x, ldx, rows, cols, colmax, pl, mp, inv_scale_t, act,
                       (double *)nullptr);
    LA_LAUNCH_CHECK();
    return LA_OK;
}

extern "C" int la_split_f16x2_t_colsum(const float *x, int64_t ldx, int32_t rows, int32_t cols, void *planes_t, int64_t mp, float *inv_scale_t,
                                       int32_t act, float *colsum, void *stream_) {
    return la_split_f16x2_t_tmax(x, ldx, rows, cols, planes_t, mp, inv_scale_t, act, colsum, nullptr, stream_);
}

extern "C" int la_split_f16x2_t_act(const float *x, int64_t ldx, int32_t rows, int32_t cols, void *planes_t, int64_t mp, float *inv_scale_t,
                                    int32_t act, void *stream_) {
    return la_split_f16x2_t_colsum(x, ldx, rows, cols, planes_t, mp, inv_scale_t, act, nullptr, stream_);
}

extern "C" int la_split_f16x2_t(const float *x, int64_t ldx, int32_t rows, int32_t cols, void *planes_t, int64_t mp, float *inv_scale_t, void *stream_) {
    return la_split_f16x2_t_act(x, ldx, rows, cols, planes_t, mp, inv_scale_t, 0, stream_);
}

extern "C" int la_gemm_f16x2(int32_t M, int32_t N, int32_t K, int32_t slots, const void *A, const float *sa, const void *W, const float *sw,
                             float *C, int64_t ldc, const float *bias, const float *residual, int64_t ldr, int32_t epilogue, void *stream_) {
    if (M == 0 || N == 0) return LA_OK;
    LA_CHECK_ARG(A && sa && W && sw && C, "gemm_f16x2: null pointer");
    LA_CHECK_ARG(M > 0 && N > 0 && K > 0 && slots >= 1, "gemm_f16x2: bad sizes");
    LA_CHECK_ARG((epilogue & ~(LA_EPI_BIAS | LA_EPI_GELU | LA_EPI_RESIDUAL | LA_EPI_RES_GELU_GRAD)) == 0,
                 "gemm_f16x2: epilogue takes BIAS, GELU, RESIDUAL, RES_GELU_GRAD only");
    LA_CHECK_ARG(!(epilogue & LA_EPI_RES_GELU_GRAD) || (epilogue & LA_EPI_RESIDUAL), "gemm_f16x2: RES_GELU_GRAD reads the residual operand (set RESIDUAL too)");
    LA_CHECK_ARG(!(epilogue & LA_EPI_BIAS) || bias, "gemm_f16x2: bias epilogue without pointer");
    LA_CHECK_ARG(!(epilogue & LA_EPI_RESIDUAL) || residual, "gemm_f16x2: residual epilogue without pointer");
    LA_CHECK_ARG((uintptr_t)A % 16 == 0 && (uintptr_t)W % 16 == 0, "gemm_f16x2: planes must be 16-byte aligned");
    const int Kc = K / slots;
    if (K % slots != 0 || Kc % 128 != 0 || Kc < 256 || N <= 128 || (int64_t)la::cdiv(M, 256) * la::cdiv(N, 256) * slots < 192) {
        la::set_error("gemm_f16x2: M=%d N=%d K=%d slots=%d outside the 256x256 kernel's domain (K / slots a multiple of 128 and >= 256, N > 128, "
                      ">= 192 tiles x slots)", M, N, K, slots);
        return LA_EUNSUPPORTED;
    }
    hipStream_t stream = (hipStream_t)stream_;
    float *out = C;
    int64_t out_ld = ldc, out_stride = 0;
    int epi = epilogue | LA_EPI_OUT_F32;
    if (slots > 1) {
        out = static_cast<float *>(la::stream_scratch(stream, la::SCRATCH_SPLITK, (size_t)slots * M * N * sizeof(float)));
        if (!out) { la::set_error("gemm_f16x2: split-K scratch allocation failed"); return LA_EHIP; }
        out_ld = N; out_stride = (int64_t)M * N;
        epi = LA_EPI_OUT_F32;
    }
    GemmParams p{M, N, Kc, A, (int64_t)2 * K, (int64_t)Kc, W, (int64_t)2 * K, (int64_t)Kc, out, out_ld, out_stride,
                 slots > 1 ? nullptr : bias, 0, slots > 1 ? nullptr : residual, ldr, 0, epi, 0, la::cdiv(N, BN), pick_group(3 * Kc, 2, la::cdiv(N, BN))};
    p.plane_a = K; p.plane_w = K;
    p.ln_stats = sa; p.ln_csum = sw;
    const int rc = launch_x2_f16(p, slots, stream);
    if (rc != LA_OK || slots == 1) return rc;
    const int64_t total = (int64_t)M * N;
    hipLaunchKernelGGL(x2_reduce_kernel, dim3((unsigned)la::cdiv(total, (int64_t)256)), dim3(256), 0, stream, out, slots, M, N, C, ldc, bias,
                       residual, ldr, epilogue);
    LA_LAUNCH_CHECK();
    return LA_OK;
}

namespace {

typedef Cfg<2, 2> SmallX2;

__device__ __forceinline__ unsigned x2s_off(int s, bool is_w, unsigned plane_bytes) {
    const int col = s / 3, seg = s - 3 * col;
    const bool lo = is_w ? seg == 1 : seg == 0;
    return (lo ? plane_bytes : 0u) + (unsigned)col * 64u;
}

__device__ __forceinline__ void x2s_stage(const unsigned char *src, int64_t ld_bytes, int row0, int last_row, unsigned off0, unsigned off1,
                                          unsigned char *lds_tile, int wave, int lane) {
    const int r8 = lane >> 3, slot = lane & 7;
#pragma unroll
    for (int i = 0; i < 4; ++i) {
        const int piece = wave * 4 + i;
        const int rt = piece * 8 + r8;
        int row = row0 + rt;
        row = row > last_row ? last_row : row;
        const int ls = slot ^ swz(rt);
        const unsigned off = (ls < 4 ? off0 : off1) + (unsigned)(ls & 3) * 16u;
        la::glds16(src + (int64_t)row * ld_bytes + off, lds_tile + piece * 1024);
    }
}

__global__ __launch_bounds__(SmallX2::THREADS, 2) void gemm_f16x2_small_kernel(GemmParams p) {
    extern __shared__ __attribute__((aligned(16))) unsigned char lds[];
    const int nwg = p.tiles_m * p.tiles_n;
    const int tile = xcd_remap(blockIdx.x, nwg);
    const TileCoord tc = tile_coord(tile, p.tiles_m, p.tiles_n, p.group);
    const int m0 = tc.tm * SmallX2::TM, n0 = tc.tn * BN;
    const int z = blockIdx.y;
    const unsigned char *A = reinterpret_cast<const unsigned char *>(p.A) + (int64_t)z * p.strideA * 2;
    const unsigned char *W = reinterpret_cast<const unsigned char *>(p.W) + (int64_t)z * p.strideW * 2;
    const int tid = threadIdx.x, lane = tid & 63, wave = tid >> 6;
    const int wm = wave >> 1, wn = wave & 1;
    const int r = lane & 15, q = lane >> 4;
    const int64_t lda_b = p.lda * 2, ldw_b = p.ldw * 2;
    const unsigned pa = (unsigned)(p.plane_a * 2), pw = (unsigned)(p.plane_w * 2);
    const int nsub = 3 * (p.K / 32), nk = (nsub + 1) / 2;

    f32x4 acc[4][4];
#pragma unroll
    for (int mi = 0; mi < 4; ++mi)
#pragma unroll
        for (int ni = 0; ni < 4; ++ni) acc[mi][ni] = f32x4{0.f, 0.f, 0.f, 0.f};

    auto stage = [&](int kt, int buf) {
        unsigned char *st = lds + buf * SmallX2::STAGE;
        const int s0 = 2 * kt, s1 = 2 * kt + 1 < nsub ? 2 * kt + 1 : s0;
        x2s_stage(A, lda_b, m0, p.M - 1, x2s_off(s0, false, pa), x2s_off(s1, false, pa), st, wave, lane);
// ... 157 lines not shown
```

lyricalignment_amd/csrc/la_gemm_epilogue.h:

```cpp
#pragma once
#include <type_traits>

#include "la_gemm_params.h"
#include "la_gemm_pp.h"

namespace la {
namespace gemm {

__device__ __forceinline__ float row16_sum(float x) {
    x += __int_as_float(__builtin_amdgcn_update_dpp(0, __float_as_int(x), 0xB1, 0xf, 0xf, true));
    x += __int_as_float(__builtin_amdgcn_update_dpp(0, __float_as_int(x), 0x4E, 0xf, 0xf, true));
    x += __int_as_float(__builtin_amdgcn_update_dpp(0, __float_as_int(x), 0x124, 0xf, 0xf, true));
    x += __int_as_float(__builtin_amdgcn_update_dpp(0, __float_as_int(x), 0x128, 0xf, 0xf, true));
    return x;
}
__device__ __forceinline__ float half_bits_to_f32(unsigned short b, bf16_t) { return __uint_as_float((unsigned)b << 16); }
__device__ __forceinline__ float half_bits_to_f32(unsigned short b, la::f16_t) { return (float)__builtin_bit_cast(_Float16, b); }

template <typename T16>
__device__ __forceinline__ float2 segment_stats(const ushort4 pk) {
    const float e0 = half_bits_to_f32(pk.x, T16{}), e1 = half_bits_to_f32(pk.y, T16{}), e2 = half_bits_to_f32(pk.z, T16{}),
                e3 = half_bits_to_f32(pk.w, T16{});
    const float mean = row16_sum((e0 + e1) + (e2 + e3)) * (1.0f / 64.0f);
    const float d0 = e0 - mean, d1 = e1 - mean, d2 = e2 - mean, d3 = e3 - mean;
    return make_float2(mean, row16_sum(fmaf(d0, d0, d1 * d1) + fmaf(d2, d2, d3 * d3)));
}

constexpr int EPI_PITCH = 272;
template <bool OUT_F32, int LNM>
__device__ __forceinline__ void epi_quad(f32x4 &v, const float (&b4)[4], const float (&cs4)[4], float2 st, bool has_bias, bool do_gelu, int epilogue) {
    if constexpr (LNM == 2) {
        const float rs = st.y, bm = -st.x * st.y;
#pragma unroll
        for (int j = 0; j < 4; ++j) v[j] = fmaf(v[j], rs, fmaf(bm, cs4[j], b4[j]));
    } else if constexpr (LNM == 6) {
        const float rs = st.y;
#pragma unroll
        for (int j = 0; j < 4; ++j) v[j] = fmaf(v[j] * rs, cs4[j], b4[j]);
    } else if (has_bias) {
#pragma unroll
        for (int j = 0; j < 4; ++j) v[j] += b4[j];
    }
    if (do_gelu) {
        if constexpr (!OUT_F32) {
            if (epilogue & 4096) {
                const la::f32x2 lo = la::gelu_pk(la::f32x2{v[0], v[1]}), hi = la::gelu_pk(la::f32x2{v[2], v[3]});
                v = f32x4{lo.x, lo.y, hi.x, hi.y};
            } else if (LA_DEV_BIT(epilogue, 8192)) {
#pragma unroll
                for (int j = 0; j < 4; ++j) v[j] = la::gelu_sig(v[j]);
            } else {
                const la::f32x2 lo = la::gelu_sig2(la::f32x2{v[0], v[1]}), hi = la::gelu_sig2(la::f32x2{v[2], v[3]});
                v = f32x4{lo.x, lo.y, hi.x, hi.y};
            }
        } else {
#pragma unroll
            for (int j = 0; j < 4; ++j) v[j] = la::gelu_erf(v[j]);
        }
    }
}

template <bool OUT_F32, typename T16, int LNM, int STG = 0>
__device__ __forceinline__ void wave_epilogue(const GemmParams &p, int z, f32x4 (&acc)[8][4], int wrow0, int wcol0, bool has_bias,
                                              float bias_l, float csum_l, unsigned char *reg, const float2 *stats_tab = nullptr,
                                              int tile_m0 = 0, unsigned char *reg_edge = nullptr, float2 sr0 = float2{0.f, 1.f},
                                              float2 sr1 = float2{0.f, 1.f}, int lane_in = -1) {
    constexpr bool LNC = LNM == 2 || LNM == 4 || LNM == 5 || LNM == 6;
    constexpr int EQ = LNM == 6 ? 6 : (LNC ? 2 : LNM);
    constexpr int NPASS = STG ? 8 : 4, NIT = STG ? 4 : 8, RP = STG ? 16 : 32;
    const int lane = lane_in >= 0 ? lane_in : (int)(threadIdx.x & 63);
    const int r = lane & 15, q = lane >> 4;
    typedef typename std::conditional<OUT_F32, float, T16>::type TC;
    TC *C = reinterpret_cast<TC *>(p.C) + (int64_t)z * p.strideC;
    const float *R = p.residual ? p.residual + (int64_t)z * p.strideR : nullptr;
    const bool do_gelu = p.epilogue & LA_EPI_GELU;
    const bool do_res = (p.epilogue & LA_EPI_RESIDUAL) && R;
    const int epi = p.epilogue;
    float b4[4], cs4[4];
#pragma unroll
    for (int j = 0; j < 4; ++j) {
        b4[j] = __int_as_float(__builtin_amdgcn_ds_bpermute((r * 4 + j) * 4, __float_as_int(bias_l)));
        cs4[j] = LNC ? __int_as_float(__builtin_amdgcn_ds_bpermute((r * 4 + j) * 4, __float_as_int(csum_l))) : 0.f;
    }
    const float2 *stats = reinterpret_cast<const float2 *>(p.ln_stats);
    constexpr int PITCH = EPI_PITCH;
    const bool fast_c = ((p.ldc * (int64_t)sizeof(TC)) % 16 == 0) && ((uintptr_t)C % 16 == 0);
    const bool fast_r = do_res && (p.ldr % 4 == 0) && ((uintptr_t)R % 16 == 0);
    if (wrow0 + 128 <= p.M && wcol0 + 64 <= p.N && fast_c && (!do_res || fast_r)) {
        TC *cw = C + (int64_t)wrow0 * p.ldc + wcol0 + r * 4;
        const float *rw = do_res ? R + (int64_t)wrow0 * p.ldr + wcol0 + r * 4 : nullptr;
        T16 *c2w = nullptr;
        float2 *part = nullptr;
        if constexpr (LNM == 1 && OUT_F32) {
            c2w = reinterpret_cast<T16 *>(p.C2) + (int64_t)z * p.strideC + (int64_t)wrow0 * p.ldc + wcol0 + r * 4;
            if (p.ln_part) part = reinterpret_cast<float2 *>(p.ln_part) + (int64_t)(wcol0 >> 6) * p.M + wrow0;
        }
        auto fast = [&](auto resc) {
            constexpr bool RES = decltype(resc)::value;
#pragma unroll
            for (int h = 0; h < NPASS; ++h) {
                float4 t[NIT];
                float2 st[NIT];
                if constexpr (RES) {
                    if (LA_DEV_BIT(epi, 1 << 16)) {
#pragma unroll
                        for (int it = 0; it < NIT; ++it) t[it] = make_float4(0.f, 0.f, 0.f, 0.f);
                    } else {
#pragma unroll
                        for (int it = 0; it < NIT; ++it) t[it] = *reinterpret_cast<const float4 *>(rw + (int64_t)(h * RP + it * 4 + q) * p.ldr);
                    }
                }
                if constexpr (LNM == 2) {
#pragma unroll
                    for (int it = 0; it < NIT; ++it) st[it] = stats[wrow0 + h * RP + it * 4 + q];
                }
                if constexpr (LNM == 4 || LNM == 6) {
#pragma unroll
                    for (int it = 0; it < NIT; ++it) st[it] = stats_tab[wrow0 - tile_m0 + h * RP + it * 4 + q];
                }
                if constexpr (LNM == 5) {
#pragma unroll
                    for (int it = 0; it < NIT; ++it) {
                        const int src = (((h * RP + it * 4) & 63) + q) * 4;
                        const float2 sr = h * RP >= 64 ? sr1 : sr0;
                        st[it] = make_float2(__int_as_float(__builtin_amdgcn_ds_bpermute(src, __float_as_int(sr.x))),
                                             __int_as_float(__builtin_amdgcn_ds_bpermute(src, __float_as_int(sr.y))));
                    }
                }
                if constexpr (STG == 0) {
#pragma unroll
                    for (int mm = 0; mm < 2; ++mm)
#pragma unroll
                        for (int ni = 0; ni < 4; ++ni)
                            *reinterpret_cast<f32x4 *>(reg + (mm * 16 + r) * PITCH + (ni * 16 + q * 4) * 4) = acc[2 * h + mm][ni];
                } else {
#pragma unroll
                    for (int ni = 0; ni < 4; ++ni)
                        *reinterpret_cast<f32x4 *>(reg + r * 256 + (((ni * 4 + q) ^ r) << 4)) = acc[h][ni];
                }
#pragma unroll
                for (int it = 0; it < NIT; ++it) {
                    const int rl = it * 4 + q;
                    f32x4 v = STG == 0 ? *reinterpret_cast<const f32x4 *>(reg + rl * PITCH + r * 16)
                                       : *reinterpret_cast<const f32x4 *>(reg + rl * 256 + ((r ^ rl) << 4));
                    epi_quad<OUT_F32, EQ>(v, b4, cs4, LNC ? st[it] : make_float2(0.f, 0.f), has_bias, do_gelu, epi);
                    if constexpr (RES) {
                        if (LNM == 6 && (epi & LA_EPI_RES_GELU_GRAD)) {
                            v[0] *= la::gelu_erf_grad(t[it].x); v[1] *= la::gelu_erf_grad(t[it].y);
                            v[2] *= la::gelu_erf_grad(t[it].z); v[3] *= la::gelu_erf_grad(t[it].w);
                        } else { v[0] += t[it].x; v[1] += t[it].y; v[2] += t[it].z; v[3] += t[it].w; }
                    }
                    const int64_t off = (int64_t)(h * RP + rl) * p.ldc;
                    TC *c = cw + off;
                    if constexpr (sizeof(TC) == 4) {
                        if (!LA_DEV_BIT(epi, 2 << 16) || v[0] == 12345.678f)
                            *reinterpret_cast<float4 *>(c) = make_float4(v[0], v[1], v[2], v[3]);
                        if constexpr (LNM == 1) {
                            const ushort4 pk = la::Pack4<T16>::run(v[0], v[1], v[2], v[3]);
                            if (!LA_DEV_BIT(epi, 4 << 16) || v[1] == 12345.678f)
                                *reinterpret_cast<ushort4 *>(c2w + off) = pk;
                            if (part) {
                                const float2 sg = segment_stats<T16>(pk);
                                if (r == 0) part[h * RP + rl] = sg;
                            }
                        }
                    } else {
                        if (!LA_DEV_BIT(epi, 2 << 16) || v[0] == 12345.678f)
                            *reinterpret_cast<ushort4 *>(c) = la::Pack4<TC>::run(v[0], v[1], v[2], v[3]);
                    }
                }
            }
        };
        if (do_res) fast(std::true_type{}); else fast(std::false_type{});
        return;
    }
    T16 *C2 = nullptr;
    if constexpr (LNM == 1 && OUT_F32) C2 = reinterpret_cast<T16 *>(p.C2) + (int64_t)z * p.strideC;
    if (reg_edge) reg = reg_edge;
#pragma unroll
    for (int h = 0; h < 4; ++h) {
#pragma unroll
        for (int mm = 0; mm < 2; ++mm)
#pragma unroll
            for (int ni = 0; ni < 4; ++ni)
                *reinterpret_cast<f32x4 *>(reg + (mm * 16 + r) * PITCH + (ni * 16 + q * 4) * 4) = acc[2 * h + mm][ni];
#pragma unroll
        for (int it = 0; it < 8; ++it) {
            const int rl = it * 4 + q;
            const int m = wrow0 + h * 32 + rl;
            const int n = wcol0 + r * 4;
            f32x4 v = *reinterpret_cast<const f32x4 *>(reg + rl * PITCH + r * 16);
            float2 st = make_float2(0.f, 0.f);
            if constexpr (LNM == 2) st = stats[min(m, p.M - 1)];
            if constexpr (LNM == 4 || LNM == 6) st = stats_tab[wrow0 - tile_m0 + h * 32 + rl];
            if constexpr (LNM == 5) {
                const int src = (((h * 32 + it * 4) & 63) + q) * 4;
                const float2 sr = h * 32 >= 64 ? sr1 : sr0;
                st = make_float2(__int_as_float(__builtin_amdgcn_ds_bpermute(src, __float_as_int(sr.x))),
                                 __int_as_float(__builtin_amdgcn_ds_bpermute(src, __float_as_int(sr.y))));
            }
            epi_quad<OUT_F32, EQ>(v, b4, cs4, st, has_bias, do_gelu, epi);
            if (m >= p.M || n >= p.N) continue;
            const int nv = min(4, p.N - n);
            if (do_res) {
                const float *rr = R + (int64_t)m * p.ldr + n;
                if (LNM == 6 && (epi & LA_EPI_RES_GELU_GRAD)) {
                    for (int j = 0; j < nv; ++j) v[j] *= la::gelu_erf_grad(rr[j]);
                } else if (fast_r && nv == 4) {
                    const float4 t = *reinterpret_cast<const float4 *>(rr);
                    v[0] += t.x; v[1] += t.y; v[2] += t.z; v[3] += t.w;
                } else {
                    for (int j = 0; j < nv; ++j) v[j] += rr[j];
                }
            }
            TC *c = C + (int64_t)m * p.ldc + n;
            if (fast_c && nv == 4) {
                if constexpr (sizeof(TC) == 4) {
                    *reinterpret_cast<float4 *>(c) = make_float4(v[0], v[1], v[2], v[3]);
                } else {
                    *reinterpret_cast<ushort4 *>(c) = la::Pack4<TC>::run(v[0], v[1], v[2], v[3]);
                }
            } else {
                for (int j = 0; j < nv; ++j) la::Elem<TC>::store(c + j, v[j]);
            }
            if constexpr (LNM == 1) {
                for (int j = 0; j < nv; ++j) la::Elem<T16>::store(C2 + (int64_t)m * p.ldc + n + j, v[j]);
                if (p.ln_part) {
                    const float2 sg = segment_stats<T16>(la::Pack4<T16>::run(v[0], v[1], v[2], v[3]));
                    if (r == 0) reinterpret_cast<float2 *>(p.ln_part)[(int64_t)(wcol0 >> 6) * p.M + m] = sg;
                }
            }
        }
    }
}

template <typename T16, int STG = 0>
__device__ __forceinline__ void wave_epilogue_split(const GemmParams &p, int z, f32x4 (&acc)[8][4], int wrow0, int wcol0, bool has_bias,
                                                    float bias_l, unsigned char *reg, unsigned char *reg_edge = nullptr, int lane_in = -1) {
    constexpr int NPASS = STG ? 8 : 4, NIT = STG ? 4 : 8, RP = STG ? 16 : 32;
    const int lane = lane_in >= 0 ? lane_in : (int)(threadIdx.x & 63);
    const int r = lane & 15, q = lane >> 4;
    unsigned char *LO = reinterpret_cast<unsigned char *>(p.C) + (int64_t)z * p.strideC;
    T16 *HI = reinterpret_cast<T16 *>(p.C2) + (int64_t)z * p.strideC;
    const float *R = p.residual ? p.residual + (int64_t)z * p.strideR : nullptr;
    const bool do_gelu = p.epilogue & LA_EPI_GELU;
    const bool res_f32 = (p.epilogue & LA_EPI_RESIDUAL) && R;
    const bool res_split = p.epilogue & LA_EPI_SPLIT_INPLACE;
    const int epi = p.epilogue;
    float b4[4];
    const float cs4[4] = {0.f, 0.f, 0.f, 0.f};
#pragma unroll
    for (int j = 0; j < 4; ++j) b4[j] = __int_as_float(__builtin_amdgcn_ds_bpermute((r * 4 + j) * 4, __float_as_int(bias_l)));
    constexpr int PITCH = EPI_PITCH;
    const bool fast_c = (p.ldc % 4 == 0) && ((uintptr_t)LO % 4 == 0) && ((uintptr_t)HI % 8 == 0) && (p.strideC % 4 == 0);
    const bool fast_r = res_f32 && (p.ldr % 4 == 0) && ((uintptr_t)R % 16 == 0);
    if (wrow0 + 128 <= p.M && wcol0 + 64 <= p.N && fast_c && (!res_f32 || fast_r)) {
// ... 121 lines not shown
```

lyricalignment_amd/csrc/la_gemm_params.h:

```cpp
#pragma once
#include "la_common.h"

namespace la {
namespace gemm {

struct GemmParams {
    int M, N, K;
    const void *A;
    int64_t lda, strideA;
    const void *W;
    int64_t ldw, strideW;
    void *C;
    int64_t ldc, strideC;
    const float *bias;
    int64_t strideBias;
    const float *residual;
    int64_t ldr, strideR;
    int epilogue;
    int tiles_m, tiles_n, group;
    int mblock = 0;
    void *C2 = nullptr;
    int64_t ldc2 = 0, strideC2 = 0;
    const float *ln_stats = nullptr;
    const float *ln_csum = nullptr;
    int K_tail = 0;
    int64_t plane_a = 0, plane_w = 0;
    float *ln_part = nullptr;
};

constexpr int LA_EPI_SPLIT_INPLACE = 1 << 20;
constexpr int LA_EPI_SPLIT_PASS32 = 1 << 21;
constexpr int LA_EPI_Q4_PRIO = 1 << 23;

int launch_pp_bf16(GemmParams p, int batch, bool out_f32, hipStream_t stream);
int launch_pp_f16(GemmParams p, int batch, bool out_f32, hipStream_t stream);
int launch_split_bf16(GemmParams p, int batch, hipStream_t stream);
int launch_split_f16(GemmParams p, int batch, hipStream_t stream);
int launch_x2_f16(GemmParams p, int batch, hipStream_t stream);

#ifdef LA_EXPERIMENTS
bool lab_try_launch(GemmParams &p, int batch, bool out_f32, int lnm, bool duo, hipStream_t stream, int *rc);
int lab_set_tile_stamps(void *buf);
#endif

}
}
```

lyricalignment_amd/csrc/la_gemm_pp_f16.hip:

```cpp
#ifdef LA_TILE_STAMPS
#undef LA_TILE_STAMPS
#endif
#include "la_gemm_pp_kernel.h"

namespace la {
namespace gemm {

int launch_pp_f16(GemmParams p, int batch, bool out_f32, hipStream_t stream) {
    return out_f32 ? launch_pp<true, la::f16_t>(p, batch, stream) : launch_pp<false, la::f16_t>(p, batch, stream);
}

int launch_split_f16(GemmParams p, int batch, hipStream_t stream) { return launch_split<la::f16_t>(p, batch, stream); }

int launch_x2_f16(GemmParams p, int batch, hipStream_t stream) { return launch_pp_loop<true, true, la::f16_t, 6>(p, batch, stream); }

}
}
```

lyricalignment_amd/csrc/la_gemm_pp_kernel.h:

```cpp
#pragma once
#include <algorithm>

#include "la_gemm_epilogue.h"

namespace la {
namespace gemm {

#ifdef LA_TILE_STAMPS
static __device__ unsigned long long *g_tile_stamps = nullptr;
static inline int set_tile_stamps_here(void *buf) {
    unsigned long long *b = static_cast<unsigned long long *>(buf);
    return hipMemcpyToSymbol(HIP_SYMBOL(g_tile_stamps), &b, sizeof(b)) == hipSuccess ? LA_OK : LA_EHIP;
}
#endif

template <bool OUT_F32, bool DUO, typename T16, int LNM = 0>
__global__ __launch_bounds__(PP::THREADS, 2) void gemm_pp_kernel(GemmParams p) {
    extern __shared__ __attribute__((aligned(16))) unsigned char lds[];
#ifdef LA_TILE_STAMPS
    const unsigned long long stamp_t0 = __builtin_amdgcn_s_memrealtime();
    unsigned long long stamp_t1 = stamp_t0;
#endif
    const int nwg = p.tiles_m * p.tiles_n;
    const int tile = xcd_remap(blockIdx.x, nwg);
    const TileCoord tc = tile_coord_mb(tile, p.tiles_m, p.tiles_n, p.group, p.mblock);
    const int m0 = tc.tm * PP::TM, n0 = tc.tn * PP::TN;
    const int z = blockIdx.y;
    const T16 *A = reinterpret_cast<const T16 *>(p.A) + (int64_t)z * p.strideA;
    const T16 *W = reinterpret_cast<const T16 *>(p.W) + (int64_t)z * p.strideW;
    const float *bias = p.bias ? p.bias + (int64_t)z * p.strideBias : nullptr;

    const int lane = threadIdx.x & 63, wave = threadIdx.x >> 6;
    const int wr = wave >> 2, wc = wave & 3;
    const bool has_bias = (p.epilogue & LA_EPI_BIAS) && bias;
    const int ncol = min(n0 + wc * 64 + lane, p.N - 1);
    const float bias_l = has_bias ? bias[ncol] : 0.f;
    float csum_l = 0.f;
    if constexpr (LNM == 2 || LNM == 4 || LNM == 6) csum_l = p.ln_csum[ncol];
    float2 st_pre = make_float2(0.f, 1.f);
    if constexpr (LNM == 2) {
        if (lane < 32) st_pre = reinterpret_cast<const float2 *>(p.ln_stats)[min(m0 + wr * 128 + wc * 32 + lane, p.M - 1)];
    }
    if constexpr (LNM == 6) {
        if (lane < 32) st_pre = make_float2(0.f, p.ln_stats[min(m0 + wr * 128 + wc * 32 + lane, p.M - 1)]);
    }

    f32x4 acc[8][4];
#ifdef LA_TILE_STAMPS
#define LA_STAMP_ARG , stamp_t1
#else
#define LA_STAMP_ARG
#endif
    float sacc[4] = {0.f, 0.f, 0.f, 0.f};
    float2 *stats_tab = reinterpret_cast<float2 *>(lds + 120 * 1024);
    if constexpr (LNM == 4) {
        static_assert(DUO || LNM != 4, "the main loop takes the row statistics only in its hand-placed form");
        const int wc_u = __builtin_amdgcn_readfirstlane(wc);
        switch (wc_u) {
            case 0: mainloop_duo_asm<T16, 0>(A, p.lda, p.M, W, p.ldw, p.N, p.K, m0, n0, lds, acc LA_STAMP_ARG, sacc); break;
            case 1: mainloop_duo_asm<T16, 1>(A, p.lda, p.M, W, p.ldw, p.N, p.K, m0, n0, lds, acc LA_STAMP_ARG, sacc); break;
            case 2: mainloop_duo_asm<T16, 2>(A, p.lda, p.M, W, p.ldw, p.N, p.K, m0, n0, lds, acc LA_STAMP_ARG, sacc); break;
            default: mainloop_duo_asm<T16, 3>(A, p.lda, p.M, W, p.ldw, p.N, p.K, m0, n0, lds, acc LA_STAMP_ARG, sacc); break;
        }
        const float inv_k = 1.0f / (float)p.K;
#pragma unroll
        for (int i = 0; i < 2; ++i) {
            float s1 = sacc[2 * i], s2 = sacc[2 * i + 1];
            s1 += __shfl_xor(s1, 16); s2 += __shfl_xor(s2, 16);
            s1 += __shfl_xor(s1, 32); s2 += __shfl_xor(s2, 32);
            const float mean = s1 * inv_k;
            const float var = fmaxf(fmaf(-mean, mean, s2 * inv_k), 0.f);
            if (lane < 16) stats_tab[wr * 128 + (2 * wc + i) * 16 + lane] = make_float2(mean, 1.0f / sqrtf(var + 1e-5f));
        }
    } else if constexpr (LNM == 6) {
        static_assert(DUO || LNM != 6, "the segmented-K loop is the hand-placed one");
        mainloop_duo_seg_asm<T16>(A, p.lda, p.M, W, p.ldw, p.N, p.K, p.plane_a, p.plane_w, m0, n0, lds, acc);
    } else if constexpr (DUO) {
        mainloop_duo_asm<T16>(A, p.lda, p.M, W, p.ldw, p.N, p.K, m0, n0, lds, acc LA_STAMP_ARG);
    } else {
        mainloop_pp<T16>(A, p.lda, p.M, W, p.ldw, p.N, p.K, m0, n0, lds, acc);
    }
    if constexpr (LNM == 2 || LNM == 6) {
        if (lane < 32) stats_tab[wr * 128 + wc * 32 + lane] = st_pre;
    }
#ifdef LA_TILE_STAMPS
    const unsigned long long stamp_t2 = __builtin_amdgcn_s_memrealtime();
#endif

    __syncthreads();
    if constexpr (LNM == 3) {
        if (p.epilogue & LA_EPI_SPLIT_PASS32) wave_epilogue_split<T16, 0>(p, z, acc, m0 + wr * 128, n0 + wc * 64, has_bias, bias_l, lds + wave * (32 * EPI_PITCH));
        else wave_epilogue_split<T16, 1>(p, z, acc, m0 + wr * 128, n0 + wc * 64, has_bias, bias_l, lds + wave * (32 * EPI_PITCH), lds + wave * (32 * EPI_PITCH));
    } else wave_epilogue<OUT_F32, T16, LNM == 2 ? 4 : LNM>(p, z, acc, m0 + wr * 128, n0 + wc * 64, has_bias, bias_l, csum_l, lds + wave * (32 * EPI_PITCH), stats_tab, m0);
#ifdef LA_TILE_STAMPS
    if (threadIdx.x == 0 && g_tile_stamps) {
        unsigned long long *o = g_tile_stamps + ((size_t)blockIdx.y * gridDim.x + blockIdx.x) * 8;
        o[0] = stamp_t0; o[1] = stamp_t1; o[2] = stamp_t2; o[3] = __builtin_amdgcn_s_memrealtime();
        unsigned hw_id, xcc_id;
        asm volatile("s_getreg_b32 %0, hwreg(HW_REG_HW_ID)" : "=s"(hw_id));
        asm volatile("s_getreg_b32 %0, hwreg(HW_REG_XCC_ID)" : "=s"(xcc_id));
        o[4] = hw_id; o[5] = xcc_id;
        o[6] = tile;
    }
#endif
}

template <bool OUT_F32, bool DUO, typename T16, int LNM = 0>
int launch_pp_loop(GemmParams p, int batch, hipStream_t stream) {
    auto kern = gemm_pp_kernel<OUT_F32, DUO, T16, LNM>;
    static la::DeviceOnce attr_once;
    if (attr_once.pending()) {
        LA_HIP(hipFuncSetAttribute(reinterpret_cast<const void *>(kern), hipFuncAttributeMaxDynamicSharedMemorySize, PP::LDS));
        attr_once.mark();
    }
    p.tiles_m = la::cdiv(p.M, PP::TM);
    p.tiles_n = la::cdiv(p.N, PP::TN);
    p.group = la::dev_env("LA_GEMM_GROUP") ? std::min(p.group, p.tiles_n) : std::min(p.tiles_n, std::max(4, p.group / 2));
    p.mblock = p.tiles_n > p.group ? (LNM == 6 ? 8 : 32) : 0;
    if (const char *g = la::dev_env("LA_GEMM_MBLOCK")) p.mblock = atoi(g);
    if (const char *g = la::dev_env("LA_GELU_PK")) p.epilogue |= atoi(g) == 2 ? 8192 : 4096;
    if (const char *g = la::dev_env("LA_EPI_PROBE")) p.epilogue |= (atoi(g) & 7) << 16;
    la::TimerScope ts(LNM == 6 ? "gemm_f16x2" : "gemm_bf16", stream, 2.0 * p.M * p.N * p.K * batch);
    hipLaunchKernelGGL(kern, dim3(p.tiles_m * p.tiles_n, batch), dim3(PP::THREADS), PP::LDS, stream, p);
    LA_LAUNCH_CHECK();
    return LA_OK;
}

template <bool OUT_F32, typename T16>
int launch_pp(GemmParams p, int batch, hipStream_t stream) {
    const bool duo = p.K % 128 == 0 && p.K >= 256 && la::opts().gemm_loop != 99;
    const int lnm = p.ln_stats ? 2 : (p.ln_csum ? 4 : ((OUT_F32 && p.C2) ? 1 : 0));
#ifdef LA_EXPERIMENTS
    if constexpr (std::is_same<T16, bf16_t>::value) {
        int rc = LA_OK;
        if (lab_try_launch(p, batch, OUT_F32, lnm, duo, stream, &rc)) return rc;
    }
#endif
    if (lnm == 4) {
        la::set_error("gemm_fused_ln: the in-loop row statistics (ln_csum without ln_stats) were measured slower than la_row_stats16 and live "
                      "in the experiment build only (tools/build_variant.sh, bfloat16)");
        return LA_EUNSUPPORTED;
    }
    if (lnm == 2) return duo ? launch_pp_loop<OUT_F32, true, T16, 2>(p, batch, stream) : launch_pp_loop<OUT_F32, false, T16, 2>(p, batch, stream);
    if constexpr (OUT_F32) {
        if (lnm == 1) return duo ? launch_pp_loop<OUT_F32, true, T16, 1>(p, batch, stream) : launch_pp_loop<OUT_F32, false, T16, 1>(p, batch, stream);
    }
    return duo ? launch_pp_loop<OUT_F32, true, T16>(p, batch, stream) : launch_pp_loop<OUT_F32, false, T16>(p, batch, stream);
}

template <typename T16>
int launch_split(GemmParams p, int batch, hipStream_t stream) {
    const bool duo = p.K % 128 == 0 && p.K >= 256 && la::opts().gemm_loop != 99;
    if (const char *e = la::dev_env("LA_EPI_SPLIT_PASS")) { if (atoi(e) == 32) p.epilogue |= LA_EPI_SPLIT_PASS32; }
#ifdef LA_EXPERIMENTS
    if constexpr (std::is_same<T16, bf16_t>::value) {
        int rc = LA_OK;
        if (lab_try_launch(p, batch, true, 3, duo, stream, &rc)) return rc;
    }
#endif
    return duo ? launch_pp_loop<true, true, T16, 3>(p, batch, stream) : launch_pp_loop<true, false, T16, 3>(p, batch, stream);
}

}
}
```

lyricalignment_amd/csrc/la_model.cpp:

```cpp
#include "la_common.h"

namespace {

constexpr int N_FRAMES = 3000, N_CTX = 1500, C_PAD = 128;

struct Carve {
    unsigned char *base;
    size_t off = 0;
    explicit Carve(void *p) : base(static_cast<unsigned char *>(p)) {}
    void *take(size_t bytes) {
        void *p = base ? base + off : nullptr;
        off += (size_t)la::round_up((int64_t)bytes, 256);
        return p;
    }
};

size_t esize(int dtype) { return dtype == LA_F32 ? 4 : 2; }

struct EncBufs {
    void *rows0, *y1, *h, *qkv, *att, *u;
    float *x, *stats;
    void *pl_d = nullptr, *pl_u = nullptr, *attn_ws = nullptr;
    float *inv = nullptr;
    size_t attn_ws_bytes = 0;
    size_t total;
};

bool x2_big_ok(int64_t M, int N, int K) { return K % 128 == 0 && K >= 256 && N > 128 && la::cdiv(M, 256) * la::cdiv(N, 256) >= 192; }

bool encoder_x2(const la_encoder_weights *w, int batch) {
    if ((w->dtype & 0xff) != LA_F32 || w->n_layer < 1 || !la::opts().x2_inference) return false;
    const int d = w->d;
    const bool small = la::opts().x2_small != 0;
    if (small ? (d % 32 != 0 || d > 1024 * 4) : (d % 128 != 0 || d < 256 || d > 1024 * 4)) return false;
    for (int l = 0; l < w->n_layer; ++l) {
        const la_encoder_block &k = w->blocks[l];
        if (!(k.wqkv_x2 && k.wqkv_x2s && k.wo_x2 && k.wo_x2s && k.w1_x2 && k.w1_x2s && k.w2_x2 && k.w2_x2s)) return false;
    }
    return small || la::cdiv((int64_t)batch * N_CTX, 256) * la::cdiv(d, 256) >= 192;
}

int x2_gemm(int M, int N, int K, const void *A, const float *sa, const void *W, const float *sw, float *C, int64_t ldc, const float *bias,
            const float *residual, int64_t ldr, int epilogue, hipStream_t stream) {
    if (x2_big_ok(M, N, K)) return la_gemm_f16x2(M, N, K, 1, A, sa, W, sw, C, ldc, bias, residual, ldr, epilogue, stream);
    return la_gemm_f16x2_small(M, N, K, 0, A, sa, W, sw, C, ldc, bias, residual, ldr, epilogue, stream);
}

EncBufs carve_encoder(void *ws, int dtype, int batch, int d, bool x2 = false, int n_head = 0) {
    Carve c(ws);
    const size_t es = esize(dtype), M = (size_t)batch * N_CTX;
    EncBufs b;
    const size_t stem = (size_t)la::round_up((int64_t)((size_t)batch * (N_FRAMES + 2) * C_PAD * es), 256) + (size_t)batch * (N_FRAMES + 2) * d * es;
    const size_t u_bytes = M * 4 * d * es;
    b.u = c.take(u_bytes > stem ? u_bytes : stem);
    b.rows0 = b.u;
    b.y1 = b.u ? static_cast<unsigned char *>(b.u) + (size_t)la::round_up((int64_t)((size_t)batch * (N_FRAMES + 2) * C_PAD * es), 256) : nullptr;
    b.x = static_cast<float *>(c.take(M * d * 4));
    b.h = c.take(M * d * es);
    b.qkv = c.take(M * 3 * d * es);
    b.att = c.take(M * d * es);
    b.stats = static_cast<float *>(c.take(M * 2 * 4));
    if (x2) {
        b.pl_d = c.take(M * 2 * d * 2);
        b.pl_u = c.take(M * 2 * 4 * d * 2);
        b.inv = static_cast<float *>(c.take(M * 4));
        la_attention_f16x2_workspace_bytes(batch, N_CTX, N_CTX, n_head, &b.attn_ws_bytes);
        b.attn_ws = c.take(b.attn_ws_bytes);
    }
    b.total = c.off;
    return b;
}

bool encoder_fused_ln(const la_encoder_weights *w, int batch) {
    if ((w->dtype & 0xff) == LA_F32 || w->n_layer < 1 || !w->blocks[0].wqkv_ln || w->d <= 128) return false;
    if (!la::opts().ln_fusion) return false;
    const int64_t M = (int64_t)batch * N_CTX;
    return la::cdiv(M, 256) * la::cdiv(w->d, 256) >= 192 && (int64_t)la::cdiv(N_CTX, 256) * la::cdiv(w->d, 256) * batch >= 192;
}

#define LA_TRY(expr)                   \
    do {                               \
        const int rc_ = (expr);        \
        if (rc_ != LA_OK) return rc_;  \
    } while (0)

}

extern "C" int la_encoder_workspace_bytes(const la_encoder_weights *w, int32_t batch, size_t *bytes) {
    LA_CHECK_ARG(w && bytes && batch > 0 && w->d > 0, "encoder_workspace_bytes: bad arguments");
    *bytes = carve_encoder(nullptr, w->dtype & 0xff, batch, w->d, encoder_x2(w, batch), w->n_head).total;
    return LA_OK;
}

extern "C" int la_encoder_forward(const la_encoder_weights *w, const float *mel, int64_t mel_batch_stride, int64_t mel_row_stride,
                                  int32_t batch, void *out, int64_t ld_out, int32_t out_dtype, void *workspace,
                                  size_t workspace_bytes, void *stream_) {
    hipStream_t stream = (hipStream_t)stream_;
    if (batch == 0) return LA_OK;
    LA_CHECK_ARG(w && mel && out && workspace && batch > 0, "encoder_forward: null pointer / bad batch");
    LA_CHECK_ARG(((w->dtype & 0xff) == LA_F32 && !(w->dtype & LA_Q_LOG2)) || (w->dtype & ~LA_Q_LOG2) == LA_BF16 || (w->dtype & ~LA_Q_LOG2) == LA_F16,
                 "encoder_forward: bad compute dtype");
    LA_CHECK_ARG(w->d > 0 && w->d % 64 == 0 && w->n_head * 64 == w->d, "encoder_forward: kernels are built for head_dim 64 (d = %d, heads = %d)", w->d, w->n_head);
    LA_CHECK_ARG(w->n_mels > 0 && w->n_mels <= C_PAD && w->n_layer >= 0 && (w->n_layer == 0 || w->blocks), "encoder_forward: bad dimensions");
    LA_CHECK_ARG((uintptr_t)workspace % 256 == 0, "encoder_forward: workspace must be 256-byte aligned");
    const int dt = w->dtype & 0xff, dt_attn = w->dtype, d = w->d, M = batch * N_CTX;
    const bool x2 = encoder_x2(w, batch);
    const EncBufs b = carve_encoder(workspace, dt, batch, d, x2, w->n_head);
    LA_CHECK_ARG(workspace_bytes >= b.total, "encoder_forward: workspace too small (%zu < %zu)", workspace_bytes, b.total);
    const size_t es = esize(dt);
    const int out_f32 = dt == LA_F32 ? 0 : LA_EPI_OUT_F32;

    LA_TRY(la_mel_to_rows(mel, mel_batch_stride, mel_row_stride, batch, w->n_mels, N_FRAMES, b.rows0, C_PAD, dt, stream));
    const size_t clip1 = (size_t)(N_FRAMES + 2) * d * es;
    LA_HIP(hipMemset2DAsync(b.y1, clip1, 0, (size_t)d * es, batch, stream));
    LA_HIP(hipMemset2DAsync(static_cast<unsigned char *>(b.y1) + (size_t)(N_FRAMES + 1) * d * es, clip1, 0, (size_t)d * es, batch, stream));
    LA_TRY(la_gemm(dt, N_FRAMES, d, 3 * C_PAD, batch, b.rows0, C_PAD, (int64_t)(N_FRAMES + 2) * C_PAD, w->conv1_w,
                   static_cast<unsigned char *>(b.y1) + (size_t)d * es, d, (int64_t)(N_FRAMES + 2) * d, w->conv1_b, nullptr, 0, 0,
                   LA_EPI_BIAS | LA_EPI_GELU, stream));
    const bool fused = encoder_fused_ln(w, batch);
    const int epi2 = LA_EPI_BIAS | LA_EPI_GELU | LA_EPI_RESIDUAL | out_f32;
    const bool split = fused && la::opts().resid_split;
    unsigned char *lo = reinterpret_cast<unsigned char *>(b.x);
    const char *stats_env = la::dev_env("LA_LN_STATS");
    const char *dbg_env = la::dev_env("LA_PP_DBG");
    const bool stats_in_loop = fused && dt == LA_BF16 && d % 128 == 0 && d >= 256 && stats_env && strcmp(stats_env, "loop") == 0 &&
                               !(dbg_env && (atoi(dbg_env) == 99 || atoi(dbg_env) == 73));
    const float *ln_stats = stats_in_loop ? nullptr : b.stats;
    if (split) {
        LA_TRY(la_gemm_split(dt, N_CTX, d, 3 * d, batch, b.y1, 2 * d, (int64_t)(N_FRAMES + 2) * d, w->conv2_w, b.h, lo, d, (int64_t)N_CTX * d,
                             w->conv2_b, w->pos, d, 0, LA_EPI_BIAS | LA_EPI_GELU | LA_EPI_RESIDUAL, nullptr, stream));
        if (!stats_in_loop) LA_TRY(la_row_stats16(dt, b.h, d, M, d, 1e-5f, b.stats, stream));
    } else if (fused) {
        LA_TRY(la_gemm_fused_ln(dt, N_CTX, d, 3 * d, batch, b.y1, 2 * d, (int64_t)(N_FRAMES + 2) * d, w->conv2_w, b.x, d, (int64_t)N_CTX * d,
                                w->conv2_b, w->pos, d, 0, epi2, b.h, d, (int64_t)N_CTX * d, nullptr, nullptr, nullptr, stream));
        if (!stats_in_loop) LA_TRY(la_row_stats16(dt, b.h, d, M, d, 1e-5f, b.stats, stream));
    } else {
        LA_TRY(la_gemm(dt, N_CTX, d, 3 * d, batch, b.y1, 2 * d, (int64_t)(N_FRAMES + 2) * d, w->conv2_w, b.x, d, (int64_t)N_CTX * d,
                       w->conv2_b, w->pos, d, 0, epi2, stream));
    }
    const int epi_res = LA_EPI_BIAS | LA_EPI_RESIDUAL | out_f32;
    for (int l = 0; l < w->n_layer; ++l) {
        const la_encoder_block &k = w->blocks[l];
        if (fused) {
            LA_CHECK_ARG(k.wqkv_ln && k.cqkv && k.bqkv_ln && k.w1_ln && k.c1 && k.b1_ln, "encoder_forward: block %d lacks the LayerNorm-folded weights", l);
            LA_TRY(la_gemm_fused_ln(dt, M, 3 * d, d, 1, b.h, d, 0, k.wqkv_ln, b.qkv, 3 * d, 0, k.bqkv_ln, nullptr, 0, 0, LA_EPI_BIAS, nullptr, 0, 0,
                                    ln_stats, k.cqkv, nullptr, stream));
            LA_TRY(la_attention(dt_attn, b.qkv, 3 * d, b.att, d, batch, N_CTX, w->n_head, stream));
            if (split) LA_TRY(la_gemm_split(dt, M, d, d, 1, b.att, d, 0, k.wo, b.h, lo, d, 0, k.bo, nullptr, 0, 0, LA_EPI_BIAS | LA_EPI_RESIDUAL, nullptr, stream));
            else LA_TRY(la_gemm_fused_ln(dt, M, d, d, 1, b.att, d, 0, k.wo, b.x, d, 0, k.bo, b.x, d, 0, epi_res, b.h, d, 0, nullptr, nullptr, nullptr, stream));
            if (!stats_in_loop) LA_TRY(la_row_stats16(dt, b.h, d, M, d, 1e-5f, b.stats, stream));
            LA_TRY(la_gemm_fused_ln(dt, M, 4 * d, d, 1, b.h, d, 0, k.w1_ln, b.u, 4 * d, 0, k.b1_ln, nullptr, 0, 0, LA_EPI_BIAS | LA_EPI_GELU, nullptr, 0, 0,
                                    ln_stats, k.c1, nullptr, stream));
            if (split) LA_TRY(la_gemm_split(dt, M, d, 4 * d, 1, b.u, 4 * d, 0, k.w2, b.h, lo, d, 0, k.b2, nullptr, 0, 0, LA_EPI_BIAS | LA_EPI_RESIDUAL, nullptr, stream));
            else LA_TRY(la_gemm_fused_ln(dt, M, d, 4 * d, 1, b.u, 4 * d, 0, k.w2, b.x, d, 0, k.b2, b.x, d, 0, epi_res, b.h, d, 0, nullptr, nullptr, nullptr, stream));
            if (!stats_in_loop) LA_TRY(la_row_stats16(dt, b.h, d, M, d, 1e-5f, b.stats, stream));
        } else if (x2) {
            float *qkv = static_cast<float *>(b.qkv), *att = static_cast<float *>(b.att), *u = static_cast<float *>(b.u);
            LA_TRY(la_layernorm_f16x2(b.x, d, M, d, k.ln1_g, k.ln1_b, b.pl_d, d, b.inv, stream));
            LA_TRY(x2_gemm(M, 3 * d, d, b.pl_d, b.inv, k.wqkv_x2, k.wqkv_x2s, qkv, 3 * d, k.bqkv, nullptr, 0, LA_EPI_BIAS, stream));
            LA_TRY(la_attention_lse_f16x2(qkv, 3 * d, qkv + d, qkv + 2 * d, 3 * d, att, d, batch, N_CTX, N_CTX, w->n_head, 0, nullptr, b.attn_ws,
                                          b.attn_ws_bytes, stream));
            LA_TRY(la_split_f16x2(att, d, M, d, b.pl_d, d, b.inv, stream));
            LA_TRY(x2_gemm(M, d, d, b.pl_d, b.inv, k.wo_x2, k.wo_x2s, b.x, d, k.bo, b.x, d, LA_EPI_BIAS | LA_EPI_RESIDUAL, stream));
            LA_TRY(la_layernorm_f16x2(b.x, d, M, d, k.ln2_g, k.ln2_b, b.pl_d, d, b.inv, stream));
            LA_TRY(x2_gemm(M, 4 * d, d, b.pl_d, b.inv, k.w1_x2, k.w1_x2s, u, 4 * d, k.b1, nullptr, 0, LA_EPI_BIAS, stream));
            LA_TRY(la_split_f16x2_act(u, 4 * d, M, 4 * d, b.pl_u, 4 * d, b.inv, 1 , stream));
            LA_TRY(x2_gemm(M, d, 4 * d, b.pl_u, b.inv, k.w2_x2, k.w2_x2s, b.x, d, k.b2, b.x, d, LA_EPI_BIAS | LA_EPI_RESIDUAL, stream));
        } else {
            LA_TRY(la_layernorm(b.x, d, M, d, k.ln1_g, k.ln1_b, b.h, d, dt, stream));
            LA_TRY(la_gemm(dt, M, 3 * d, d, 1, b.h, d, 0, k.wqkv, b.qkv, 3 * d, 0, k.bqkv, nullptr, 0, 0, LA_EPI_BIAS, stream));
            LA_TRY(la_attention(dt_attn, b.qkv, 3 * d, b.att, d, batch, N_CTX, w->n_head, stream));
            LA_TRY(la_gemm(dt, M, d, d, 1, b.att, d, 0, k.wo, b.x, d, 0, k.bo, b.x, d, 0, epi_res, stream));
            LA_TRY(la_layernorm(b.x, d, M, d, k.ln2_g, k.ln2_b, b.h, d, dt, stream));
            LA_TRY(la_gemm(dt, M, 4 * d, d, 1, b.h, d, 0, k.w1, b.u, 4 * d, 0, k.b1, nullptr, 0, 0, LA_EPI_BIAS | LA_EPI_GELU, stream));
            LA_TRY(la_gemm(dt, M, d, 4 * d, 1, b.u, 4 * d, 0, k.w2, b.x, d, 0, k.b2, b.x, d, 0, epi_res, stream));
        }
    }
    if (split) return la_layernorm_split(dt, b.h, lo, d, M, d, w->lnp_g, w->lnp_b, out, ld_out, out_dtype, stream);
    return la_layernorm(b.x, d, M, d, w->lnp_g, w->lnp_b, out, ld_out, out_dtype, stream);
}

namespace {

int head_clip_cap(const la_head_weights *w, int frames) {
    const int nsplit = w->hidden / (16 * (w->dtype == LA_F32 ? 2 : 4));
    const int64_t by_cus = (224 / (2 * nsplit)) * 16;
    const int64_t by_desc = (int64_t)2147483647 / ((int64_t)frames * 2 * w->hidden * (int64_t)esize(w->dtype));
    int64_t cap = by_cus < by_desc ? by_cus : by_desc;
    if (cap > 256) cap = 256;
    const int force = la::opts().head_clip_cap;
    if (force > 0 && force < cap) cap = force;
    return cap < 1 ? 1 : (int)cap;
}

struct HeadBufs {
    float *gi, *em;
    void *gru[2], *act, *gru_ws, *fc_ws, *vit_ws;
    int32_t *n_frames;
    void *planes = nullptr;
    float *inv = nullptr;
    size_t gru_ws_bytes, fc_ws_bytes, vit_ws_bytes, total;
};

bool head_x2(const la_head_weights *w) {
    return w->dtype == LA_F32 && la::opts().x2_inference && w->w_ih_x2[0] && w->w_ih_x2s[0] && w->w_ih_x2[1] && w->w_ih_x2s[1] && w->w_fc_x2 && w->w_fc_x2s;
}
bool proj_x2_ok(int64_t rows, int K, int H) { return x2_big_ok(rows, 6 * H, K) || (la::opts().x2_small && K % 32 == 0); }

int carve_head(void *ws, const la_head_weights *w, int batch, int frames, int max_labels, HeadBufs *b) {
    Carve c(ws);
    const size_t es = esize(w->dtype);
    const int H = w->hidden, cap = head_clip_cap(w, frames), bb = batch < cap ? batch : cap;
// ... 117 lines not shown
```

lyricalignment_amd/csrc/la_runtime.cpp:

```cpp
#include <stdarg.h>
#include <stdlib.h>

#include <mutex>
#include <string>
#include <vector>

#include "la_common.h"

namespace la {

char *err_buf() {
    static thread_local char buf[512] = {0};
    return buf;
}

void set_error(const char *fmt, ...) {
    va_list ap;
    va_start(ap, fmt);
    vsnprintf(err_buf(), 512, fmt, ap);
    va_end(ap);
}

void *stream_scratch(hipStream_t stream, int purpose, size_t bytes) {
    struct Slot { int dev; hipStream_t stream; int purpose; void *ptr; size_t bytes; };
    static std::mutex mu;
    static std::vector<Slot> slots;
    int dev = 0;
    if (hipGetDevice(&dev) != hipSuccess) return nullptr;
    std::lock_guard<std::mutex> lock(mu);
    for (Slot &sl : slots)
        if (sl.dev == dev && sl.stream == stream && sl.purpose == purpose) {
            if (sl.bytes >= bytes) return sl.ptr;
            if (hipStreamSynchronize(stream) != hipSuccess) return nullptr;
            (void)hipFree(sl.ptr);
            sl.ptr = nullptr; sl.bytes = 0;
            if (hipMalloc(&sl.ptr, bytes) != hipSuccess) return nullptr;
            sl.bytes = bytes;
            return sl.ptr;
        }
    Slot sl{dev, stream, purpose, nullptr, bytes < ((size_t)1 << 20) ? ((size_t)1 << 20) : bytes};
    if (hipMalloc(&sl.ptr, sl.bytes) != hipSuccess) return nullptr;
    slots.push_back(sl);
    return sl.ptr;
}

namespace {
struct OptionDesc { const char *name, *env; int Options::*field; bool env_inverts; };
const OptionDesc kOptions[] = {
    {"gemm_tile", "LA_GEMM_TILE", &Options::gemm_tile, false},       {"gemm_loop", "LA_PP_DBG", &Options::gemm_loop, false},
    {"gemm_splitk", "LA_GEMM_NO_SPLITK", &Options::gemm_splitk, true}, {"attn_nw", "LA_ATTN_NW", &Options::attn_nw, false},
    {"gru_nw", "LA_GRU_NW", &Options::gru_nw, false},                 {"gru_fence", "LA_GRU_FENCE", &Options::gru_fence, false},
    {"gru_handoff", "LA_GRU_HANDOFF", &Options::gru_handoff, false}, {"gru_poll_delay", "LA_GRU_POLL_DELAY", &Options::gru_poll_delay, false},
    {"viterbi_dpp", "LA_VITERBI_NO_DPP", &Options::viterbi_dpp, true}, {"head_clip_cap", "LA_HEAD_CLIP_CAP", &Options::head_clip_cap, false},
    {"ln_fusion", "LA_LN_FUSION", &Options::ln_fusion, false},       {"resid_split", "LA_RESID_SPLIT", &Options::resid_split, false},
    {"x2_inference", "LA_X2_INFERENCE", &Options::x2_inference, false}, {"x2_small", "LA_X2_SMALL", &Options::x2_small, false},
    {"gru_timeout_us", "LA_GRU_TIMEOUT_US", &Options::gru_timeout_us, false}, {"gru_fault_step", "LA_GRU_FAULT_STEP", &Options::gru_fault_step, false},
};
}

Options &opts() {
    static Options o = [] {
        Options v;
        for (const OptionDesc &d : kOptions) {
            const char *e = getenv(d.env);
            if (!e) continue;
            v.*(d.field) = d.env_inverts ? 0 : atoi(e);
        }
        return v;
    }();
    return o;
}

namespace {
struct TimerState {
    std::mutex mu;
    bool enabled = false;
    std::string family;
    std::vector<std::pair<hipEvent_t, hipEvent_t>> pairs;
    std::vector<std::pair<hipEvent_t, hipEvent_t>> pool;
    int period = 1;
    int64_t seen = 0;
    double work = 0.0;
};
TimerState &ts() {
    static TimerState s;
    return s;
}
}

TimerScope::TimerScope(const char *family, hipStream_t s, double work) : active(false), stream(s) {
    TimerState &t = ts();
    if (!t.enabled) return;
    std::lock_guard<std::mutex> lk(t.mu);
    if (!t.enabled || t.family != family) return;
    if (t.seen++ % t.period != 0) return;
    std::pair<hipEvent_t, hipEvent_t> pr;
    if (!t.pool.empty()) {
        pr = t.pool.back();
        t.pool.pop_back();
    } else {
        if (hipEventCreate(&pr.first) != hipSuccess) return;
        if (hipEventCreate(&pr.second) != hipSuccess) { (void)hipEventDestroy(pr.first); return; }
    }
    (void)hipEventRecord(pr.first, stream);
    t.pairs.push_back(pr);
    t.work += work;
    active = true;
}
// ... 116 lines not shown
```

lyricalignment_amd/engine.py:

```python
from __future__ import annotations

from dataclasses import dataclass, field
from typing import Dict, List, Optional, Sequence, Tuple

import ctypes
import os

import torch

from . import _lib, ops
from ._lib import LA_VARIANT_CTC, LA_VARIANT_PLAIN

N_FRAMES = 3000
N_CTX = 1500
C_PAD = 128
LN_FUSION = os.environ.get("LA_LN_FUSION", "1") != "0"
LN_STATS = os.environ.get("LA_LN_STATS", "pass")
LN_STATS_IN_EPILOGUE = LN_STATS == "epilogue"
RESID_SPLIT = os.environ.get("LA_RESID_SPLIT", "1") != "0"
ENGINE_PY = os.environ.get("LA_ENGINE_PY", "0") == "1"
HEAD_CLIPS_MAX = 256


def _f32(t: torch.Tensor, device) -> torch.Tensor:
    return t.detach().to(device=device, dtype=torch.float32).contiguous()


@dataclass
class BlockWeights:
    ln1_g: torch.Tensor; ln1_b: torch.Tensor
    wqkv: torch.Tensor; bqkv: torch.Tensor
    wo: torch.Tensor; bo: torch.Tensor
    ln2_g: torch.Tensor; ln2_b: torch.Tensor
    w1: torch.Tensor; b1: torch.Tensor
    w2: torch.Tensor; b2: torch.Tensor
    wqkv_ln: Optional[torch.Tensor] = None; cqkv: Optional[torch.Tensor] = None; bqkv_ln: Optional[torch.Tensor] = None
    w1_ln: Optional[torch.Tensor] = None; c1: Optional[torch.Tensor] = None; b1_ln: Optional[torch.Tensor] = None
    x2: Optional[List[Tuple[torch.Tensor, torch.Tensor]]] = None


def _x2_planes(w: torch.Tensor) -> Tuple[torch.Tensor, torch.Tensor]:
    N, K = w.shape
    planes = torch.empty((N, 2, K), dtype=torch.float16, device=w.device)
    inv = torch.empty((N,), dtype=torch.float32, device=w.device)
    _lib.check(_lib.lib().la_split_f16x2(_lib.ptr(w), w.stride(0), N, K, _lib.ptr(planes), K, _lib.ptr(inv), _lib.stream_ptr()), "split_f16x2")
    return planes, inv


def x2_inference_on() -> bool:
    return _lib.get_option("x2_inference") != 0


def _x2_domain(M: int, N: int, K: int) -> bool:
    return K % 128 == 0 and K >= 256 and N > 128 and -(-M // 256) * -(-N // 256) >= 192


def x2_small_on() -> bool:
    return _lib.get_option("x2_small") != 0


def _x2_gemm(a, w, out: Optional[torch.Tensor] = None, bias: Optional[torch.Tensor] = None, residual: Optional[torch.Tensor] = None) -> torch.Tensor:
    from . import f32x2
    if _x2_domain(a.rows, w.rows, a.kp):
        return f32x2.gemm(a, w, out=out, bias=bias, residual=residual)
    return f32x2.gemm_small(a, w, out=out, bias=bias, residual=residual)


def _x2_linear(x: torch.Tensor, w_x2: Tuple[torch.Tensor, torch.Tensor], bias: Optional[torch.Tensor], out: Optional[torch.Tensor] = None,
               residual: Optional[torch.Tensor] = None, x_planes=None) -> torch.Tensor:
    from . import f32x2
    planes, inv = w_x2
    N, _, K = planes.shape
    a = x_planes if x_planes is not None else f32x2.split(x, K)
    return _x2_gemm(a, f32x2.Planes(planes, inv, N, K, K), out=out, bias=bias, residual=residual)


X2_PACK = os.environ.get("LA_X2_PACK", "1") != "0"


def _fold_ln(w: torch.Tensor, b: torch.Tensor, gamma: torch.Tensor, beta: torch.Tensor, dtype: torch.dtype, device):
    w, b, gamma, beta = (t.detach().double().cpu() for t in (w, b, gamma, beta))
    wl = (w * gamma[None, :]).to(dtype)
    return (wl.to(device).contiguous(), wl.double().sum(dim=1).float().to(device).contiguous(),
            (b + w @ beta).float().to(device).contiguous())


@dataclass
class EncoderWeights:
    d: int
    n_head: int
    n_mels: int
    dtype: torch.dtype
    conv1_w: torch.Tensor; conv1_b: torch.Tensor
    conv2_w: torch.Tensor; conv2_b: torch.Tensor
    pos: torch.Tensor
    blocks: List[BlockWeights]
    lnp_g: torch.Tensor; lnp_b: torch.Tensor
    q_log2: bool = False


@dataclass
class HeadWeights:
    hidden: int
    in_dim: int
    vocab: int
    dtype: torch.dtype
    w_ih: List[torch.Tensor]
    b_ih: List[torch.Tensor]
    w_hh: List[torch.Tensor]
    b_hh: List[torch.Tensor]
    w_fc: torch.Tensor
    b_fc: torch.Tensor
    w_ih_x2: Optional[List[Tuple[torch.Tensor, torch.Tensor]]] = None
    w_fc_x2: Optional[Tuple[torch.Tensor, torch.Tensor]] = None


def pack_encoder(sd: Dict[str, torch.Tensor], n_head: int, dtype: torch.dtype, device, prefix: str = "encoder.") -> EncoderWeights:
    g = lambda k: sd[prefix + k]
    d, n_mels, _ = g("conv1.weight").shape
    if d % 64 or d // n_head != 64:
        raise NotImplementedError(f"encoder width {d} / heads {n_head}: kernels are built for head_dim 64")
    c1 = torch.zeros((d, 3, C_PAD), dtype=torch.float32)
    c1[:, :, :n_mels] = g("conv1.weight").detach().float().cpu().permute(0, 2, 1)
    c2 = g("conv2.weight").detach().float().cpu().permute(0, 2, 1).reshape(d, 3 * d)
    pos = g("positional_embedding")
    blocks = []
    i = 0
    scale = 64 ** -0.5
    q_log2 = dtype == torch.bfloat16 and os.environ.get("LA_ATTN_Q_LOG2", "1") != "0"
    if q_log2:
        scale *= 1.4426950408889634
    while f"{prefix}blocks.{i}.attn.query.weight" in sd:
        b = f"blocks.{i}."
        wq, bq = g(b + "attn.query.weight").detach().float() * scale, g(b + "attn.query.bias").detach().float() * scale
        wk = g(b + "attn.key.weight").detach().float()
        wv, bv = g(b + "attn.value.weight").detach().float(), g(b + "attn.value.bias").detach().float()
        wqkv = torch.cat([wq, wk, wv], dim=0)
        bqkv = torch.cat([bq, torch.zeros_like(bq), bv], dim=0)
        blk = BlockWeights(
            _f32(g(b + "attn_ln.weight"), device), _f32(g(b + "attn_ln.bias"), device),
            wqkv.to(device=device, dtype=dtype).contiguous(), _f32(bqkv, device),
            g(b + "attn.out.weight").detach().to(device=device, dtype=dtype).contiguous(), _f32(g(b + "attn.out.bias"), device),
            _f32(g(b + "mlp_ln.weight"), device), _f32(g(b + "mlp_ln.bias"), device),
            g(b + "mlp.0.weight").detach().to(device=device, dtype=dtype).contiguous(), _f32(g(b + "mlp.0.bias"), device),
            g(b + "mlp.2.weight").detach().to(device=device, dtype=dtype).contiguous(), _f32(g(b + "mlp.2.bias"), device))
        if dtype == torch.float32 and X2_PACK and d % 128 == 0 and d >= 256 and torch.device(device).type == "cuda":
            blk.x2 = [_x2_planes(t) for t in (blk.wqkv, blk.wo, blk.w1, blk.w2)]
        if dtype in (torch.bfloat16, torch.float16):
            blk.wqkv_ln, blk.cqkv, blk.bqkv_ln = _fold_ln(wqkv, bqkv, g(b + "attn_ln.weight"), g(b + "attn_ln.bias"), dtype, device)
            blk.w1_ln, blk.c1, blk.b1_ln = _fold_ln(g(b + "mlp.0.weight"), g(b + "mlp.0.bias"), g(b + "mlp_ln.weight"),
                                                    g(b + "mlp_ln.bias"), dtype, device)
        blocks.append(blk)
        i += 1
    return EncoderWeights(d, n_head, n_mels, dtype,
                          c1.reshape(d, 3 * C_PAD).to(device=device, dtype=dtype).contiguous(), _f32(g("conv1.bias"), device),
                          c2.to(device=device, dtype=dtype).contiguous(), _f32(g("conv2.bias"), device),
                          _f32(pos, device), blocks, _f32(g("ln_post.weight"), device), _f32(g("ln_post.bias"), device), q_log2)


@dataclass
class DecoderBlockWeights:
    ln1_g: torch.Tensor; ln1_b: torch.Tensor
    wqkv: torch.Tensor; bqkv: torch.Tensor
    wo: torch.Tensor; bo: torch.Tensor
    lnc_g: torch.Tensor; lnc_b: torch.Tensor
    wq_c: torch.Tensor; bq_c: torch.Tensor
    wkv_c: torch.Tensor; bkv_c: torch.Tensor
    wo_c: torch.Tensor; bo_c: torch.Tensor
    ln2_g: torch.Tensor; ln2_b: torch.Tensor
    w1: torch.Tensor; b1: torch.Tensor
    w2: torch.Tensor; b2: torch.Tensor


@dataclass
class DecoderWeights:
    d: int
    n_head: int
    dtype: torch.dtype
    tok_emb_f32: torch.Tensor
    tok_emb: torch.Tensor
    pos: torch.Tensor
    blocks: List[DecoderBlockWeights]
    ln_g: torch.Tensor; ln_b: torch.Tensor


def pack_decoder(sd: Dict[str, torch.Tensor], n_head: int, dtype: torch.dtype, device, prefix: str = "decoder.") -> DecoderWeights:
    g = lambda k: sd[prefix + k].detach().float()
    w = lambda t: t.to(device=device, dtype=dtype).contiguous()
    d = g("token_embedding.weight").shape[1]
    if d // n_head != 64:
        raise NotImplementedError("decoder: kernels are built for head_dim 64")
    scale = 64 ** -0.5
    blocks, i = [], 0
    while f"{prefix}blocks.{i}.attn.query.weight" in sd:
        b = f"blocks.{i}."
        bq = g(b + "attn.query.bias") * scale
        wqkv = torch.cat([g(b + "attn.query.weight") * scale, g(b + "attn.key.weight"), g(b + "attn.value.weight")], 0)
        bqkv = torch.cat([bq, torch.zeros_like(bq), g(b + "attn.value.bias")], 0)
        wkv_c = torch.cat([g(b + "cross_attn.key.weight"), g(b + "cross_attn.value.weight")], 0)
        bv_c = g(b + "cross_attn.value.bias")
# ... 15 lines not shown
def pack_head(sd: Dict[str, torch.Tensor], dtype: torch.dtype, device, prefix: str = "align_rnn.") -> HeadWeights:
    g = lambda k: sd[prefix + k].detach()
    H = g("rnn.weight_hh_l0").shape[1]
    bidir = f"{prefix}rnn.weight_ih_l0_reverse" in sd
    w_ih, b_ih, w_hh, b_hh = [], [], [], []
    layer = 0
    while f"{prefix}rnn.weight_ih_l{layer}" in sd:
        wf, bf_, hf, cf = g(f"rnn.weight_ih_l{layer}").float(), g(f"rnn.bias_ih_l{layer}").float(), g(f"rnn.weight_hh_l{layer}").float(), g(f"rnn.bias_hh_l{layer}").float()
        if bidir:
            wr, br, hr, cr = (g(f"rnn.{n}_l{layer}_reverse").float() for n in ("weight_ih", "bias_ih", "weight_hh", "bias_hh"))
        else:
            if layer > 0:
                wf = torch.cat([wf, torch.zeros_like(wf)], dim=1)
            wr, br, hr, cr = torch.zeros_like(wf), torch.zeros_like(bf_), torch.zeros_like(hf), torch.zeros_like(cf)
        w_ih.append(torch.cat([wf, wr], 0).to(device=device, dtype=dtype).contiguous())
        b_ih.append(_f32(torch.cat([bf_, br], 0), device))
        w_hh.append(torch.stack([hf, hr], 0).to(device=device, dtype=dtype).contiguous())
        b_hh.append(_f32(torch.stack([cf, cr], 0), device))
        layer += 1
    w_fc = g("fc.weight").float()
    if not bidir:
        w_fc = torch.cat([w_fc, torch.zeros_like(w_fc)], dim=1)
    hw = HeadWeights(H, w_ih[0].shape[1], w_fc.shape[0], dtype, w_ih, b_ih, w_hh, b_hh,
                     w_fc.to(device=device, dtype=dtype).contiguous(), _f32(g("fc.bias"), device))
    if (dtype == torch.float32 and X2_PACK and torch.device(device).type == "cuda" and len(w_ih) == 2
            and all(w.shape[1] % 8 == 0 for w in w_ih) and hw.w_fc.shape[1] % 8 == 0):
        hw.w_ih_x2 = [_x2_planes(w) for w in hw.w_ih]
        hw.w_fc_x2 = _x2_planes(hw.w_fc)
    return hw


class AlignEngine:

    def __init__(self, enc: EncoderWeights, head: Optional[HeadWeights], device="cuda", dec: Optional[DecoderWeights] = None):
        _lib.require_gpu()
        self.enc, self.head, self.dec, self.device = enc, head, dec, torch.device(device)
        self._buf: Dict[Tuple, torch.Tensor] = {}
        self._ws: Dict[str, torch.Tensor] = {}
        self._enc_c = self._encoder_struct(enc)
        self._head_c = self._head_struct(head) if head is not None and len(head.w_ih) == 2 else None
        self._gru_flag: Optional[torch.Tensor] = None

    @staticmethod
    def _encoder_struct(e: EncoderWeights):
        P = lambda t: ctypes.c_void_p(t.data_ptr()) if t is not None else None
        blocks = (_lib.EncoderBlockC * max(1, len(e.blocks)))()
        for i, b in enumerate(e.blocks):
            x2 = [P(t) for pair in (b.x2 or [(None, None)] * 4) for t in pair]
            blocks[i] = _lib.EncoderBlockC(P(b.ln1_g), P(b.ln1_b), P(b.wqkv), P(b.bqkv), P(b.wo), P(b.bo), P(b.ln2_g), P(b.ln2_b),
                                           P(b.w1), P(b.b1), P(b.w2), P(b.b2), P(b.wqkv_ln), P(b.cqkv), P(b.bqkv_ln), P(b.w1_ln), P(b.c1), P(b.b1_ln), *x2)
        c = _lib.EncoderWeightsC(_lib.dtype_code(e.dtype) | (_lib.LA_Q_LOG2 if e.q_log2 else 0), e.d, e.n_head, len(e.blocks), e.n_mels, P(e.conv1_w), P(e.conv1_b), P(e.conv2_w),
                                 P(e.conv2_b), P(e.pos), P(e.lnp_g), P(e.lnp_b), blocks)
        c._keep = blocks
        return c

    @staticmethod
    def _head_struct(h: HeadWeights):
        V2 = ctypes.c_void_p * 2
        P = lambda t: t.data_ptr()
        Pn = lambda t: t.data_ptr() if t is not None else None
        ih = h.w_ih_x2 or [(None, None)] * 2
        fc = h.w_fc_x2 or (None, None)
        return _lib.HeadWeightsC(_lib.dtype_code(h.dtype), h.hidden, h.in_dim, h.vocab, 2, V2(P(h.w_ih[0]), P(h.w_ih[1])), V2(P(h.b_ih[0]), P(h.b_ih[1])),
                                 V2(P(h.w_hh[0]), P(h.w_hh[1])), V2(P(h.b_hh[0]), P(h.b_hh[1])), P(h.w_fc), P(h.b_fc),
                                 V2(Pn(ih[0][0]), Pn(ih[1][0])), V2(Pn(ih[0][1]), Pn(ih[1][1])), Pn(fc[0]), Pn(fc[1]))

    def _get(self, name: str, shape, dtype, zero: bool = False) -> torch.Tensor:
        key = (name, tuple(shape), dtype)
        t = self._buf.get(key)
        if t is None:
            for k in [k for k in self._buf if k[0] == name]:
                del self._buf[k]
            t = (torch.zeros if zero else torch.empty)(shape, dtype=dtype, device=self.device)
            self._buf[key] = t
        return t

    def encode(self, mel: torch.Tensor, out_dtype: Optional[torch.dtype] = None, slot: int = 0,
               out: Optional[torch.Tensor] = None) -> torch.Tensor:
        e = self.enc
        if mel.dim() != 3 or mel.shape[1] != e.n_mels or mel.shape[2] != N_FRAMES:
            raise AssertionError("incorrect audio shape")
        mel = mel.to(device=self.device, dtype=torch.float32)
        if mel.stride(2) != 1:
            mel = mel.contiguous()
        B, d, dt = mel.shape[0], e.d, e.dtype
        M = B * N_CTX
        if not ENGINE_PY and (LN_FUSION or dt == torch.float32) and not LN_STATS_IN_EPILOGUE:
            out_dtype = out_dtype or dt
            y = out if out is not None else self._get(f"enc_out{slot}", (M, d), out_dtype)
            return ops.encoder_forward(self._enc_c, mel, y, self._ws)
        rows0 = ops.mel_to_rows(mel, C_PAD, dt)
        y1 = self._get("y1", (B, N_FRAMES + 2, d), dt, zero=True)
        ops.gemm(rows0, e.conv1_w, y1.view(-1)[d:], bias=e.conv1_b, gelu=True, M=N_FRAMES, lda=C_PAD, batch=B,
                 stride_a=(N_FRAMES + 2) * C_PAD, stride_c=(N_FRAMES + 2) * d, ldc=d)
        x = self._get("x", (M, d), torch.float32)
        h = self._get("h", (M, d), dt)
        qkv = self._get("qkv", (M, 3 * d), dt)
        att = self._get("att", (M, d), dt)
        u = self._get("u", (M, 4 * d), dt)
        fused = (LN_FUSION and dt in (torch.bfloat16, torch.float16) and e.blocks and e.blocks[0].wqkv_ln is not None and d > 128
                 and -(-M // 256) * -(-d // 256) >= 192 and -(-N_CTX // 256) * -(-d // 256) * B >= 192)
        split = fused and RESID_SPLIT
        if split:
            lo = x.view(torch.uint8).view(-1)[: M * d].view(M, d)
            ops.gemm_split(y1, e.conv2_w, h, lo, bias=e.conv2_b, gelu=True, residual=e.pos, M=N_CTX, lda=2 * d, batch=B,
                           stride_a=(N_FRAMES + 2) * d, stride_c=N_CTX * d, ld=d, ldr=d, stride_r=0)
        else:
            ops.gemm(y1, e.conv2_w, x, bias=e.conv2_b, gelu=True, residual=e.pos, out_f32=True, M=N_CTX, lda=2 * d, batch=B,
                     stride_a=(N_FRAMES + 2) * d, stride_c=N_CTX * d, ldc=d, ldr=d, stride_r=0, out16=h if fused else None)
        if fused:
            stats = self._get("ln_stats", (M, 2), torch.float32)
            part = self._get("ln_part", (d // 64, M, 2), torch.float32) if (LN_STATS_IN_EPILOGUE and d % 64 == 0) else None

            in_loop = (LN_STATS == "loop" and dt == torch.bfloat16 and d % 128 == 0 and d >= 256 and _lib.has_experiments()
                       and os.environ.get("LA_PP_DBG") not in ("99", "73"))
            if in_loop:
                stats = None

            def row_stats():
                if in_loop:
                    return
                if part is not None:
                    ops.ln_stats_finalize(part, out=stats)
                else:
                    ops.row_stats16(h, out=stats)

            if not in_loop:
                ops.row_stats16(h, out=stats)
            for blk in e.blocks:
                ops.gemm(h, blk.wqkv_ln, qkv, bias=blk.bqkv_ln, ln_stats=stats, ln_csum=blk.cqkv)
                ops.attention(qkv, B, N_CTX, e.n_head, out=att, q_log2=e.q_log2)
                if split:
                    ops.gemm_split(att, blk.wo, h, lo, bias=blk.bo, in_place=True, ln_part=part)
                else:
                    ops.gemm(att, blk.wo, x, bias=blk.bo, residual=x, out_f32=True, out16=h, ln_part=part)
                row_stats()
                ops.gemm(h, blk.w1_ln, u, bias=blk.b1_ln, gelu=True, ln_stats=stats, ln_csum=blk.c1)
                if split:
                    ops.gemm_split(u, blk.w2, h, lo, bias=blk.b2, in_place=True, ln_part=part)
                else:
                    ops.gemm(u, blk.w2, x, bias=blk.b2, residual=x, out_f32=True, out16=h, ln_part=part)
                row_stats()
        elif (dt == torch.float32 and e.blocks and all(b_.x2 is not None for b_ in e.blocks) and x2_inference_on() and d <= 4096
              and (-(-M // 256) * -(-d // 256) >= 192 or (x2_small_on() and d % 32 == 0))):
            from . import f32x2
            pl = lambda t: f32x2.Planes(t[0], t[1], t[0].shape[0], t[0].shape[2], t[0].shape[2])
            for blk in e.blocks:
                wq, wo_, w1_, w2_ = (pl(t) for t in blk.x2)
                _x2_gemm(f32x2.layernorm_split(x, blk.ln1_g, blk.ln1_b), wq, out=qkv, bias=blk.bqkv)
                ops.attention_ex(qkv[:, :d], qkv[:, d:2 * d], qkv[:, 2 * d:], B, N_CTX, N_CTX, e.n_head, out=att, x2=True)
                _x2_gemm(f32x2.split(att, d), wo_, out=x, bias=blk.bo, residual=x)
                _x2_gemm(f32x2.layernorm_split(x, blk.ln2_g, blk.ln2_b), w1_, out=u, bias=blk.b1)
                _x2_gemm(f32x2.split(u, 4 * d, act="gelu"), w2_, out=x, bias=blk.b2, residual=x)
        else:
            for blk in e.blocks:
                ops.layernorm(x, blk.ln1_g, blk.ln1_b, dt, out=h)
                ops.gemm(h, blk.wqkv, qkv, bias=blk.bqkv)
                ops.attention(qkv, B, N_CTX, e.n_head, out=att, q_log2=e.q_log2)
                ops.gemm(att, blk.wo, x, bias=blk.bo, residual=x, out_f32=True)
                ops.layernorm(x, blk.ln2_g, blk.ln2_b, dt, out=h)
                ops.gemm(h, blk.w1, u, bias=blk.b1, gelu=True)
                ops.gemm(u, blk.w2, x, bias=blk.b2, residual=x, out_f32=True)
        out_dtype = out_dtype or dt
        y = out if out is not None else self._get(f"enc_out{slot}", (M, d), out_dtype)
        if split:
            ops.layernorm_split(h, lo, e.lnp_g, e.lnp_b, out_dtype, out=y)
        else:
            ops.layernorm(x, e.lnp_g, e.lnp_b, out_dtype, out=y)
        return y

    def decode(self, tokens: torch.Tensor, xa: torch.Tensor, n_audio: int = N_CTX) -> torch.Tensor:
        dw = self.dec
        if dw is None:
            raise _lib.LyricAlignHipError("this engine was packed without decoder weights")
        B, n = tokens.shape
        d, dt, H = dw.d, dw.dtype, dw.n_head
        tokens = tokens.to(device=self.device, dtype=torch.int64)
        x = ops.embed_tokens(tokens, dw.tok_emb_f32, dw.pos)
        h = torch.empty((B * n, d), dtype=dt, device=self.device)
        for blk in dw.blocks:
            ops.layernorm(x, blk.ln1_g, blk.ln1_b, dt, out=h)
            qkv = ops.gemm(h, blk.wqkv, bias=blk.bqkv)
            a = ops.attention_ex(qkv[:, :d], qkv[:, d:2 * d], qkv[:, 2 * d:], B, n, n, H, causal=True)
            ops.gemm(a, blk.wo, x, bias=blk.bo, residual=x, out_f32=True)
            ops.layernorm(x, blk.lnc_g, blk.lnc_b, dt, out=h)
            q = ops.gemm(h, blk.wq_c, bias=blk.bq_c)
            kv = ops.gemm(xa, blk.wkv_c, bias=blk.bkv_c)
            a = ops.attention_ex(q, kv[:, :d], kv[:, d:], B, n, n_audio, H, causal=False)
            ops.gemm(a, blk.wo_c, x, bias=blk.bo_c, residual=x, out_f32=True)
            ops.layernorm(x, blk.ln2_g, blk.ln2_b, dt, out=h)
            u = ops.gemm(h, blk.w1, bias=blk.b1, gelu=True)
            ops.gemm(u, blk.w2, x, bias=blk.b2, residual=x, out_f32=True)
        ops.layernorm(x, dw.ln_g, dw.ln_b, dt, out=h)
        logits = ops.gemm(h, dw.tok_emb, out_f32=True)
        return logits.view(B, n, dw.tok_emb.shape[0])

    def _token_step(self, tok: torch.Tensor, t: int, caches, kv_cross, n_audio_clips: int, rows_per_clip: int, n_max: int,
                    n_audio: int) -> torch.Tensor:
        dw = self.dec
        d, dt, H = dw.d, dw.dtype, dw.n_head
        N = tok.shape[0]
        x = ops.embed_tokens(tok.view(N, 1).contiguous(), dw.tok_emb_f32, dw.pos[t:])
# ... 399 lines not shown
```

lyricalignment_amd/f32x2.py:

```python
from __future__ import annotations

import os
from dataclasses import dataclass
from typing import Optional

import torch

from . import _lib
from ._lib import check, lib, ptr, stream_ptr

ENABLED = os.environ.get("LA_F32X2", "1") != "0"
FUSE_ACT = os.environ.get("LA_F32X2_ACT", "1") != "0"
MIN_TILES = 192


def _rup(x: int, m: int) -> int:
    return (x + m - 1) // m * m


@dataclass
class Planes:
    planes: torch.Tensor
    inv_scale: torch.Tensor
    rows: int
    k: int
    kp: int


ACT = {None: 0, "gelu": 1}
REUSE_MAX = os.environ.get("LA_F32X2_TMAX", "1") != "0"


class OperandMax:

    WORDS = 64 * 32

    def __init__(self, device, words: Optional[torch.Tensor] = None):
        self.words = words if words is not None else torch.zeros((self.WORDS,), dtype=torch.int32, device=device)
        self.act: Optional[str] = None
        self.valid = False

    @classmethod
    def many(cls, device, count: int):
        buf = torch.zeros((count, cls.WORDS), dtype=torch.int32, device=device)
        return [cls(device, buf[i]) for i in range(count)]


def split(x: torch.Tensor, kp: Optional[int] = None, act: Optional[str] = None, omax: Optional[OperandMax] = None) -> Planes:
    if x.dtype != torch.float32 or x.dim() != 2 or x.stride(1) != 1:
        raise ValueError("f32x2.split: a float32 [rows, k] row view is expected")
    rows, k = x.shape
    kp = _rup(k, 128) if kp is None else kp
    planes = torch.empty((rows, 2, kp), dtype=torch.float16, device=x.device)
    inv = torch.empty((rows,), dtype=torch.float32, device=x.device)
    if omax is not None and REUSE_MAX:
        check(lib().la_split_f16x2_max(ptr(x), x.stride(0), rows, k, ptr(planes), kp, ptr(inv), ACT[act], ptr(omax.words), stream_ptr()), "split_f16x2")
        omax.act, omax.valid = act, True
    else:
        check(lib().la_split_f16x2_act(ptr(x), x.stride(0), rows, k, ptr(planes), kp, ptr(inv), ACT[act], stream_ptr()), "split_f16x2")
    return Planes(planes, inv, rows, k, kp)


def layernorm_split(x: torch.Tensor, gamma: torch.Tensor, beta: torch.Tensor, kp: Optional[int] = None) -> Planes:
    if x.dtype != torch.float32 or x.dim() != 2 or x.stride(1) != 1:
        raise ValueError("f32x2.layernorm_split: a float32 [rows, d] row view is expected")
    rows, d = x.shape
    kp = d if kp is None else kp
    planes = torch.empty((rows, 2, kp), dtype=torch.float16, device=x.device)
    inv = torch.empty((rows,), dtype=torch.float32, device=x.device)
    check(lib().la_layernorm_f16x2(ptr(x), x.stride(0), rows, d, ptr(gamma.contiguous()), ptr(beta.contiguous()), ptr(planes), kp, ptr(inv), stream_ptr()),
          "layernorm_f16x2")
    return Planes(planes, inv, rows, d, kp)


def split_t(x: torch.Tensor, mp: Optional[int] = None, act: Optional[str] = None, colsum: Optional[torch.Tensor] = None,
            omax: Optional[OperandMax] = None) -> Planes:
    if x.dtype != torch.float32 or x.dim() != 2 or x.stride(1) != 1:
        raise ValueError("f32x2.split_t: a float32 [m, k] row view is expected")
    m, k = x.shape
    mp = _rup(m, 128) if mp is None else mp
    planes = torch.empty((k, 2, mp), dtype=torch.float16, device=x.device)
    inv = torch.empty((k,), dtype=torch.float32, device=x.device)
    words = omax.words if (omax is not None and omax.valid and omax.act == act and REUSE_MAX) else None
    check(lib().la_split_f16x2_t_tmax(ptr(x), x.stride(0), m, k, ptr(planes), mp, ptr(inv), ACT[act], ptr(colsum), ptr(words), stream_ptr()),
          "split_f16x2_t")
    return Planes(planes, inv, k, m, mp)


class WeightPlanes:

    def __init__(self):
        self.planes = {}

    def put(self, orient: str, length: int, value: "Planes") -> None:
        for k in [k for k in self.planes if k[0] == orient]:
            del self.planes[k]
        self.planes[(orient, length)] = value


def slots_for(M: int, N: int) -> int:
    tiles = -(-M // 256) * -(-N // 256)
    return max(1, -(-MIN_TILES // tiles))


def eligible(M: int, N: int, K: int) -> bool:
    if not ENABLED or N <= 128 or K < 256:
        return False
    s = slots_for(M, N)
    return s <= 16 and K // s >= 256


def padded_k(M: int, N: int, K: int) -> int:
    s = slots_for(M, N)
    return s * _rup(-(-K // s), 128)


def gemm(a: Planes, w: Planes, out: Optional[torch.Tensor] = None, bias: Optional[torch.Tensor] = None,
         residual: Optional[torch.Tensor] = None, gelu: bool = False, gelu_grad_of: Optional[torch.Tensor] = None) -> torch.Tensor:
    if a.kp != w.kp:
        raise ValueError(f"f32x2.gemm: operands were split to different plane lengths ({a.kp}, {w.kp})")
    M, N = a.rows, w.rows
    if out is None:
        out = torch.empty((M, N), dtype=torch.float32, device=a.planes.device)
    epi = 0
    if bias is not None:
# ... 116 lines not shown
```

Measured before the change: 23640 audio-sec/sec.

## Emit split f16 planes directly from attention and MLP-up GEMM epilogues

In the f32x2 encoder path, the attention kernel now writes its output straight into the hi/lo f16 planes. It scales each row by the largest V head scale, so the separate f32 store and re-split kernel are no longer needed. The MLP first GEMM also writes GELU output directly as planes. Its per-row output scale comes from an a-priori bound (LayerNorm row norm times the max W1 row norm plus the max bias) that the layernorm kernel computes. This removes two f32 intermediate round trips and two split launches per layer, at the cost of possibly looser scaling and lower precision in the plane representation.

```diff
diff --git a/include/lyricalign.h b/include/lyricalign.h
--- a/include/lyricalign.h
+++ b/include/lyricalign.h
@@ -25,6 +25,7 @@
 } la_dtype;
 
 #define LA_Q_LOG2 0x100
+#define LA_X2_BOUNDS 0x200
 
 
 typedef enum la_variant {
@@ -297,6 +298,13 @@
 int la_gemm_f16x2_small_slots(int32_t M, int32_t N, int32_t K);
 int la_layernorm_f16x2(const float *x, int64_t ldx, int32_t rows, int32_t d, const float *gamma, const float *beta, void *planes, int64_t kp,
                        float *inv_scale, void *stream);
+int la_layernorm_f16x2_bound(const float *x, int64_t ldx, int32_t rows, int32_t d, const float *gamma, const float *beta, void *planes,
+                             int64_t kp, float *inv_scale, float wmax, float bmax, float *inv_out, void *stream);
+int la_gemm_f16x2_planes(int32_t M, int32_t N, int32_t K, const void *A, const float *sa, const void *W, const float *sw, void *planes_out,
+                         int64_t kp_out, const float *inv_out, const float *bias, int32_t epilogue, void *stream);
+int la_attention_f16x2_planes(const float *q, int64_t ld_q, const float *k, const float *v, int64_t ld_kv, void *planes_out, float *inv_out,
+                              int32_t batch, int32_t q_len, int32_t kv_len, int32_t n_head, int32_t causal, void *workspace,
+                              size_t workspace_bytes, void *stream);
 
 int la_gemm_ex(int32_t dtype, int32_t M, int32_t N, int32_t K, int32_t batch, const void *A, int64_t lda, int64_t strideA,
                const void *W, int64_t ldw, int64_t strideW, void *C, int64_t ldc, int64_t strideC, const float *bias,
@@ -368,6 +376,7 @@
     const float *pos;
     const float *lnp_g, *lnp_b;
     const la_encoder_block *blocks;
+    const float *x2_bounds;
 } la_encoder_weights;
 
 int la_encoder_workspace_bytes(const la_encoder_weights *w, int32_t batch, size_t *bytes);
diff --git a/lyricalignment_amd/_lib.py b/lyricalignment_amd/_lib.py
--- a/lyricalignment_amd/_lib.py
+++ b/lyricalignment_amd/_lib.py
@@ -11,6 +11,7 @@
 
 LA_OK, LA_EINVAL, LA_EINFEASIBLE, LA_EEMPTY, LA_EHIP, LA_ETIMEOUT, LA_EUNSUPPORTED = range(7)
 LA_F32, LA_BF16, LA_F16 = 0, 1, 2
+LA_X2_BOUNDS = 0x200
 LA_Q_LOG2 = 0x100
 LA_VARIANT_PLAIN, LA_VARIANT_CTC = 0, 1
 EPI_BIAS, EPI_GELU, EPI_RESIDUAL, EPI_OUT_F32, EPI_MISH = 1, 2, 4, 8, 16
@@ -40,6 +41,9 @@
     "la_gemm_f16x2_small": (c_int32, [_I32, _I32, _I32, _I32, _P, _P, _P, _P, _P, _I64, _P, _P, _I64, _I32, _P]),
     "la_gemm_f16x2_small_slots": (c_int32, [_I32, _I32, _I32]),
     "la_layernorm_f16x2": (c_int32, [_P, _I64, _I32, _I32, _P, _P, _P, _I64, _P, _P]),
+    "la_layernorm_f16x2_bound": (c_int32, [_P, _I64, _I32, _I32, _P, _P, _P, _I64, _P, ctypes.c_float, ctypes.c_float, _P, _P]),
+    "la_gemm_f16x2_planes": (c_int32, [_I32, _I32, _I32, _P, _P, _P, _P, _P, _I64, _P, _P, _I32, _P]),
+    "la_attention_f16x2_planes": (c_int32, [_P, _I64, _P, _P, _I64, _P, _P, _I32, _I32, _I32, _I32, _I32, _P, _SZ, _P]),
     "la_fc_emissions_x2_workspace_bytes": (c_int32, [_I32, _I32, _I32, _I32, _I32, POINTER(_SZ)]),
     "la_fc_emissions_x2": (c_int32, [_P, _I64, _P, _P, _P, _P, _I32, _I32, _I32, _I32, _I32, _P, _I32, _P, _I32, _P, _I64, _I64, _P, _SZ, _P]),
     "la_set_option": (c_int32, [c_char_p, c_int64]),
@@ -155,7 +159,8 @@
 class EncoderWeightsC(ctypes.Structure):
     _fields_ = [("dtype", c_int32), ("d", c_int32), ("n_head", c_int32), ("n_layer", c_int32), ("n_mels", c_int32),
                 ("conv1_w", c_void_p), ("conv1_b", c_void_p), ("conv2_w", c_void_p), ("conv2_b", c_void_p), ("pos", c_void_p),
-                ("lnp_g", c_void_p), ("lnp_b", c_void_p), ("blocks", POINTER(EncoderBlockC))]
+                ("lnp_g", c_void_p), ("lnp_b", c_void_p), ("blocks", POINTER(EncoderBlockC)),
+                ("x2_bounds", POINTER(ctypes.c_float))]
 
 
 class HeadWeightsC(ctypes.Structure):
diff --git a/lyricalignment_amd/csrc/la_attention_f16x2.hip b/lyricalignment_amd/csrc/la_attention_f16x2.hip
--- a/lyricalignment_amd/csrc/la_attention_f16x2.hip
+++ b/lyricalignment_amd/csrc/la_attention_f16x2.hip
@@ -24,6 +24,8 @@
     int64_t ld_out;
     float *lse;
     int q_len, kv_len, n_head, causal, batch;
+    unsigned short *out_planes = nullptr;
+    float *out_inv = nullptr;
 };
 
 __global__ __launch_bounds__(1024) void heads_split_kernel(const float *x, int64_t ld, int T, int H, unsigned short *planes, float *inv_scale) {
@@ -132,7 +134,7 @@
         : "v"(hi), "v"(a), "v"(b));
 }
 
-template <int NW>
+template <int NW, bool PLANES = false>
 __global__ __launch_bounds__(64 * NW, 2) void attention_x2_fwd_kernel(FwdParams p) {
     constexpr int QT = 32 * NW, PER = 8 / NW;
     __shared__ __attribute__((aligned(16))) unsigned char lds[8 * IMG];
@@ -326,7 +328,25 @@
     const float l = l_part + __shfl_xor(l_part, 32);
     const float inv = p.sv[bh] / l;
     if (p.lse && q_valid && h == 0) p.lse[((int64_t)clip * p.n_head + head) * p.q_len + qrow] = fmaf(m_run - 13.0f, kLn2, __logf(l));
-    if (q_valid) {
+    if constexpr (PLANES) {
+        float ic = p.sv[clip * p.n_head];
+        for (int hh = 1; hh < p.n_head; ++hh) ic = fmaxf(ic, p.sv[clip * p.n_head + hh]);
+        const float so = 1.0f / ic;
+        if (q_valid) {
+            unsigned short *prow = p.out_planes + ((int64_t)clip * p.q_len + qrow) * 2 * C + head * 64;
+#pragma unroll
+            for (int b = 0; b < 2; ++b)
+#pragma unroll
+                for (int r4 = 0; r4 < 4; ++r4) {
+                    const unsigned a = la::x2::pack_hi_lo(o[b][4 * r4 + 0] * inv * so), bq = la::x2::pack_hi_lo(o[b][4 * r4 + 1] * inv * so),
+                                   c = la::x2::pack_hi_lo(o[b][4 * r4 + 2] * inv * so), d = la::x2::pack_hi_lo(o[b][4 * r4 + 3] * inv * so);
+                    unsigned short *dst = prow + 32 * b + 8 * r4 + 4 * h;
+                    *reinterpret_cast<uint2 *>(dst) = make_uint2((a & 0xffffu) | (bq << 16), (c & 0xffffu) | (d << 16));
+                    *reinterpret_cast<uint2 *>(dst + C) = make_uint2((a >> 16) | (bq & 0xffff0000u), (c >> 16) | (d & 0xffff0000u));
+                }
+            if (head == 0 && h == 0) p.out_inv[(int64_t)clip * p.q_len + qrow] = ic;
+        }
+    } else if (q_valid) {
         float *orow = p.out + ((int64_t)clip * p.q_len + qrow) * p.ld_out + head * 64;
 #pragma unroll
         for (int b = 0; b < 2; ++b)
@@ -733,6 +753,31 @@
     hipLaunchKernelGGL(heads_split_kernel, sgrid, dim3(1024), 0, stream, v, ld_kv, kv_len, n_head, ws.vp, ws.sv);
     FwdParams p{ws.qp, ws.kp, ws.vp, ws.sq, ws.sk, ws.sv, out, ld_out, lse, q_len, kv_len, n_head, causal ? 1 : 0, batch};
     hipLaunchKernelGGL((attention_x2_fwd_kernel<8>), dim3(la::cdiv(q_len, 256) * n_head * batch), dim3(512), 0, stream, p);
+    LA_LAUNCH_CHECK();
+    return LA_OK;
+}
+
+extern "C" int la_attention_f16x2_planes(const float *q, int64_t ld_q, const float *k, const float *v, int64_t ld_kv, void *planes_out,
+                                         float *inv_out, int32_t batch, int32_t q_len, int32_t kv_len, int32_t n_head, int32_t causal,
+                                         void *workspace, size_t workspace_bytes, void *stream_) {
+    hipStream_t stream = (hipStream_t)stream_;
+    if (batch == 0 || q_len == 0) return LA_OK;
+    LA_CHECK_ARG(q && k && v && planes_out && inv_out && batch > 0 && q_len > 0 && kv_len > 0 && n_head > 0, "attention_f16x2_planes: bad arguments");
+    LA_CHECK_ARG(!causal || q_len == kv_len, "attention_f16x2_planes: causal masking is defined for self-attention (q_len == kv_len)");
+    LA_CHECK_ARG(ld_q >= n_head * 64 && ld_kv >= n_head * 64, "attention_f16x2_planes: leading dimensions too small");
+    LA_CHECK_ARG(ld_q % 4 == 0 && ld_kv % 4 == 0 && (uintptr_t)q % 16 == 0 && (uintptr_t)k % 16 == 0 && (uintptr_t)v % 16 == 0 &&
+                     (uintptr_t)planes_out % 16 == 0, "attention_f16x2_planes: rows must be 16-byte aligned");
+    const FwdWorkspace ws = fwd_workspace(workspace, batch, q_len, kv_len, n_head);
+    LA_CHECK_ARG(workspace && (uintptr_t)workspace % 256 == 0 && workspace_bytes >= ws.bytes, "attention_f16x2_planes: workspace missing, misaligned or too small");
+    la::TimerScope ts("attention_f16x2", stream);
+    const dim3 sgrid = heads_split_grid(n_head, batch);
+    hipLaunchKernelGGL(heads_split_kernel, sgrid, dim3(1024), 0, stream, q, ld_q, q_len, n_head, ws.qp, ws.sq);
+    hipLaunchKernelGGL(heads_split_kernel, sgrid, dim3(1024), 0, stream, k, ld_kv, kv_len, n_head, ws.kp, ws.sk);
+    hipLaunchKernelGGL(heads_split_kernel, sgrid, dim3(1024), 0, stream, v, ld_kv, kv_len, n_head, ws.vp, ws.sv);
+    FwdParams p{ws.qp, ws.kp, ws.vp, ws.sq, ws.sk, ws.sv, nullptr, 0, nullptr, q_len, kv_len, n_head, causal ? 1 : 0, batch};
+    p.out_planes = reinterpret_cast<unsigned short *>(planes_out);
+    p.out_inv = inv_out;
+    hipLaunchKernelGGL((attention_x2_fwd_kernel<8, true>), dim3(la::cdiv(q_len, 256) * n_head * batch), dim3(512), 0, stream, p);
     LA_LAUNCH_CHECK();
     return LA_OK;
 }
diff --git a/lyricalignment_amd/csrc/la_common.h b/lyricalignment_amd/csrc/la_common.h
--- a/lyricalignment_amd/csrc/la_common.h
+++ b/lyricalignment_amd/csrc/la_common.h
@@ -43,7 +43,7 @@
 
 struct Options {
     int gemm_tile = 0, gemm_loop = 0, gemm_splitk = 1, attn_nw = 0, gru_nw = 0, gru_fence = 0, gru_handoff = 0, gru_poll_delay = 0, viterbi_dpp = 1,
-        head_clip_cap = 0, ln_fusion = 1, resid_split = 1, x2_inference = 1, gru_timeout_us = 0, gru_fault_step = 0, x2_small = 0;
+        head_clip_cap = 0, ln_fusion = 1, resid_split = 1, x2_inference = 1, gru_timeout_us = 0, gru_fault_step = 0, x2_small = 0, x2_planes_out = 1;
 };
 Options &opts();
 #ifdef LA_EXPERIMENTS
diff --git a/lyricalignment_amd/csrc/la_f32x2.hip b/lyricalignment_amd/csrc/la_f32x2.hip
--- a/lyricalignment_amd/csrc/la_f32x2.hip
+++ b/lyricalignment_amd/csrc/la_f32x2.hip
@@ -23,6 +23,10 @@
     const _Float16 l = (_Float16)(xs - (float)h);
     hi = __builtin_bit_cast(unsigned short, h);
     lo = __builtin_bit_cast(unsigned short, l);
+}
+
+__device__ __forceinline__ float x2_value(unsigned short hi, unsigned short lo) {
+    return (float)__builtin_bit_cast(_Float16, hi) + (float)__builtin_bit_cast(_Float16, lo);
 }
 
 __device__ __forceinline__ float x2_act(float v, int act) { return act == 1 ? la::gelu_erf(v) : v; }
@@ -93,8 +97,9 @@
     if (lane == 0) inv_scale[row] = inv;
 }
 
-__global__ __launch_bounds__(256) void ln_split_rows_kernel(const float *x, int64_t ldx, int rows, int d, const float *gamma, const float *beta,
-                                                            unsigned short *planes, int64_t kp, float *inv_scale) {
+template <bool BOUND>
+__device__ __forceinline__ void ln_split_rows_body(const float *x, int64_t ldx, int rows, int d, const float *gamma, const float *beta,
+                                                   unsigned short *planes, int64_t kp, float *inv_scale, float wmax, float bmax, float *inv_out) {
     const int lane = threadIdx.x & 63;
     const int row = blockIdx.x * 4 + (threadIdx.x >> 6);
     if (row >= rows) return;
@@ -142,6 +147,7 @@
     float inv;
     const float s = x2_scale(mx, &inv);
     unsigned short *hi = planes + (int64_t)row * 2 * kp, *lo = hi + kp;
+    float nsq = 0.f;
 #pragma unroll
     for (int j = 0; j < NV; ++j) {
         const int i = lane + 64 * j;
@@ -150,10 +156,33 @@
             x2_split(v[j].x * s, h.x, l.x); x2_split(v[j].y * s, h.y, l.y); x2_split(v[j].z * s, h.z, l.z); x2_split(v[j].w * s, h.w, l.w);
             reinterpret_cast<ushort4 *>(hi)[i] = h;
             reinterpret_cast<ushort4 *>(lo)[i] = l;
+            if constexpr (BOUND) {
+                const float a = x2_value(h.x, l.x), b = x2_value(h.y, l.y), c = x2_value(h.z, l.z), e = x2_value(h.w, l.w);
+                nsq += (a * a + b * b) + (c * c + e * e);
+            }
         }
     }
     for (int i = d + lane; i < kp; i += 64) { hi[i] = 0; lo[i] = 0; }
     if (lane == 0) inv_scale[row] = inv;
+    if constexpr (BOUND) {
+#pragma unroll
+        for (int o = 32; o > 0; o >>= 1) nsq += __shfl_xor(nsq, o);
+        const float bound = (sqrtf(nsq) * inv * wmax + bmax) * (1.0f + 0x1p-8f);
+        float io;
+        (void)x2_scale(bound, &io);
+        if (lane == 0) inv_out[row] = io;
+    }
+}
+
+__global__ __launch_bounds__(256) void ln_split_rows_kernel(const float *x, int64_t ldx, int rows, int d, const float *gamma, const float *beta,
+                                                            unsigned short *planes, int64_t kp, float *inv_scale) {
+    ln_split_rows_body<false>(x, ldx, rows, d, gamma, beta, planes, kp, inv_scale, 0.f, 0.f, nullptr);
+}
+
+__global__ __launch_bounds__(256) void ln_split_rows_bound_kernel(const float *x, int64_t ldx, int rows, int d, const float *gamma, const float *beta,
+                                                                  unsigned short *planes, int64_t kp, float *inv_scale, float wmax, float bmax,
+                                                                  float *inv_out) {
+    ln_split_rows_body<true>(x, ldx, rows, d, gamma, beta, planes, kp, inv_scale, wmax, bmax, inv_out);
 }
 
 __global__ __launch_bounds__(256) void colmax_kernel(const float *x, int64_t ldx, int rows, int cols, int rows_per_block, unsigned *colmax, int act) {
@@ -338,6 +367,22 @@
     return LA_OK;
 }
 
+extern "C" int la_layernorm_f16x2_bound(const float *x, int64_t ldx, int32_t rows, int32_t d, const float *gamma, const float *beta, void *planes,
+                                        int64_t kp, float *inv_scale, float wmax, float bmax, float *inv_out, void *stream_) {
+    if (rows == 0) return LA_OK;
+    LA_CHECK_ARG(x && gamma && beta && planes && inv_scale && inv_out && rows > 0, "layernorm_f16x2_bound: bad arguments");
+    LA_CHECK_ARG(wmax >= 0.f && bmax >= 0.f && wmax < 3.0e38f && bmax < 3.0e38f, "layernorm_f16x2_bound: wmax / bmax must be finite and non-negative");
+    LA_CHECK_ARG(d > 0 && d % 4 == 0 && d <= 4096 && ldx % 4 == 0 && ldx >= d && (uintptr_t)x % 16 == 0 && (uintptr_t)gamma % 16 == 0 && (uintptr_t)beta % 16 == 0,
+                 "layernorm_f16x2_bound: d=%d unsupported (a multiple of 4, at most 4096) or misaligned rows", d);
+    LA_CHECK_ARG(kp >= d && kp % 8 == 0 && (uintptr_t)planes % 16 == 0, "layernorm_f16x2_bound: kp must be >= d and a multiple of 8, planes 16-byte aligned");
+    hipStream_t stream = (hipStream_t)stream_;
+    la::TimerScope ts("split_f16x2", stream, (double)rows * d * 8.0);
+    hipLaunchKernelGGL(ln_split_rows_bound_kernel, dim3(la::cdiv(rows, 4)), dim3(256), 0, stream, x, ldx, rows, d, gamma, beta,
+                       reinterpret_cast<unsigned short *>(planes), kp, inv_scale, wmax, bmax, inv_out);
+    LA_LAUNCH_CHECK();
+    return LA_OK;
+}
+
 extern "C" int la_colsum_f32(const float *in, int64_t ld, int32_t rows, int32_t cols, float *out, void *stream);
 
 extern "C" int la_split_f16x2_t_tmax(const float *x, int64_t ldx, int32_t rows, int32_t cols, void *planes_t, int64_t mp, float *inv_scale_t,
@@ -444,6 +489,29 @@
                        residual, ldr, epilogue);
     LA_LAUNCH_CHECK();
     return LA_OK;
+}
+
+extern "C" int la_gemm_f16x2_planes(int32_t M, int32_t N, int32_t K, const void *A, const float *sa, const void *W, const float *sw,
+                                    void *planes_out, int64_t kp_out, const float *inv_out, const float *bias, int32_t epilogue, void *stream_) {
+    if (M == 0 || N == 0) return LA_OK;
+    LA_CHECK_ARG(A && sa && W && sw && planes_out && inv_out, "gemm_f16x2_planes: null pointer");
+    LA_CHECK_ARG(M > 0 && N > 0 && K > 0, "gemm_f16x2_planes: bad sizes");
+    LA_CHECK_ARG((epilogue & ~(LA_EPI_BIAS | LA_EPI_GELU)) == 0, "gemm_f16x2_planes: epilogue takes BIAS and GELU only");
+    LA_CHECK_ARG(!(epilogue & LA_EPI_BIAS) || bias, "gemm_f16x2_planes: bias epilogue without pointer");
+    LA_CHECK_ARG((uintptr_t)A % 16 == 0 && (uintptr_t)W % 16 == 0, "gemm_f16x2_planes: planes must be 16-byte aligned");
+    LA_CHECK_ARG(kp_out >= N && kp_out % 8 == 0 && N % 8 == 0 && (uintptr_t)planes_out % 16 == 0,
+                 "gemm_f16x2_planes: N and kp_out must be multiples of 8 (kp_out >= N), planes_out 16-byte aligned");
+    if (K % 128 != 0 || K < 256 || N <= 128 || (int64_t)la::cdiv(M, 256) * la::cdiv(N, 256) < 192) {
+        la::set_error("gemm_f16x2_planes: M=%d N=%d K=%d outside the 256x256 kernel's domain (K a multiple of 128 and >= 256, N > 128, >= 192 tiles)", M, N, K);
+        return LA_EUNSUPPORTED;
+    }
+    hipStream_t stream = (hipStream_t)stream_;
+    GemmParams p{M, N, K, A, (int64_t)2 * K, (int64_t)K, W, (int64_t)2 * K, (int64_t)K, planes_out, 2 * kp_out, 0,
+                 bias, 0, nullptr, 0, 0, epilogue | LA_EPI_OUT_F32, 0, la::cdiv(N, BN), pick_group(3 * K, 2, la::cdiv(N, BN))};
+    p.plane_a = K; p.plane_w = K;
+    p.ln_stats = sa; p.ln_csum = sw;
+    p.out_inv = inv_out;
+    return launch_x2_planes_f16(p, stream);
 }
 
 namespace {
diff --git a/lyricalignment_amd/csrc/la_gemm_epilogue.h b/lyricalignment_amd/csrc/la_gemm_epilogue.h
--- a/lyricalignment_amd/csrc/la_gemm_epilogue.h
+++ b/lyricalignment_amd/csrc/la_gemm_epilogue.h
@@ -16,6 +16,12 @@
 }
 __device__ __forceinline__ float half_bits_to_f32(unsigned short b, bf16_t) { return __uint_as_float((unsigned)b << 16); }
 __device__ __forceinline__ float half_bits_to_f32(unsigned short b, la::f16_t) { return (float)__builtin_bit_cast(_Float16, b); }
+__device__ __forceinline__ void x2_split_pair(float xs, unsigned short &hi, unsigned short &lo) {
+    const _Float16 h = (_Float16)xs;
+    const _Float16 l = (_Float16)(xs - (float)h);
+    hi = __builtin_bit_cast(unsigned short, h);
+    lo = __builtin_bit_cast(unsigned short, l);
+}
 
 template <typename T16>
 __device__ __forceinline__ float2 segment_stats(const ushort4 pk) {
@@ -65,8 +71,8 @@
                                               float bias_l, float csum_l, unsigned char *reg, const float2 *stats_tab = nullptr,
                                               int tile_m0 = 0, unsigned char *reg_edge = nullptr, float2 sr0 = float2{0.f, 1.f},
                                               float2 sr1 = float2{0.f, 1.f}, int lane_in = -1) {
-    constexpr bool LNC = LNM == 2 || LNM == 4 || LNM == 5 || LNM == 6;
-    constexpr int EQ = LNM == 6 ? 6 : (LNC ? 2 : LNM);
+    constexpr bool LNC = LNM == 2 || LNM == 4 || LNM == 5 || LNM == 6 || LNM == 7;
+    constexpr int EQ = (LNM == 6 || LNM == 7) ? 6 : (LNC ? 2 : LNM);
     constexpr int NPASS = STG ? 8 : 4, NIT = STG ? 4 : 8, RP = STG ? 16 : 32;
     const int lane = lane_in >= 0 ? lane_in : (int)(threadIdx.x & 63);
     const int r = lane & 15, q = lane >> 4;
@@ -84,8 +90,10 @@
     }
     const float2 *stats = reinterpret_cast<const float2 *>(p.ln_stats);
     constexpr int PITCH = EPI_PITCH;
-    const bool fast_c = ((p.ldc * (int64_t)sizeof(TC)) % 16 == 0) && ((uintptr_t)C % 16 == 0);
+    const bool fast_c = LNM == 7 ? (p.ldc % 8 == 0 && (uintptr_t)p.C % 8 == 0) : ((p.ldc * (int64_t)sizeof(TC)) % 16 == 0) && ((uintptr_t)C % 16 == 0);
     const bool fast_r = do_res && (p.ldr % 4 == 0) && ((uintptr_t)R % 16 == 0);
+    unsigned short *PL = reinterpret_cast<unsigned short *>(p.C);
+    const int64_t plane_c = p.ldc >> 1;
     if (wrow0 + 128 <= p.M && wcol0 + 64 <= p.N && fast_c && (!do_res || fast_r)) {
         TC *cw = C + (int64_t)wrow0 * p.ldc + wcol0 + r * 4;
         const float *rw = do_res ? R + (int64_t)wrow0 * p.ldr + wcol0 + r * 4 : nullptr;
@@ -114,7 +122,7 @@
 #pragma unroll
                     for (int it = 0; it < NIT; ++it) st[it] = stats[wrow0 + h * RP + it * 4 + q];
                 }
-                if constexpr (LNM == 4 || LNM == 6) {
+                if constexpr (LNM == 4 || LNM == 6 || LNM == 7) {
 #pragma unroll
                     for (int it = 0; it < NIT; ++it) st[it] = stats_tab[wrow0 - tile_m0 + h * RP + it * 4 + q];
                 }
@@ -151,6 +159,16 @@
                         } else { v[0] += t[it].x; v[1] += t[it].y; v[2] += t[it].z; v[3] += t[it].w; }
                     }
                     const int64_t off = (int64_t)(h * RP + rl) * p.ldc;
+                    if constexpr (LNM == 7) {
+                        const float so = st[it].x;
+                        ushort4 ph, pl;
+                        x2_split_pair(v[0] * so, ph.x, pl.x); x2_split_pair(v[1] * so, ph.y, pl.y);
+                        x2_split_pair(v[2] * so, ph.z, pl.z); x2_split_pair(v[3] * so, ph.w, pl.w);
+                        unsigned short *c = PL + (int64_t)wrow0 * p.ldc + wcol0 + r * 4 + off;
+                        *reinterpret_cast<ushort4 *>(c) = ph;
+                        *reinterpret_cast<ushort4 *>(c + plane_c) = pl;
+                        continue;
+                    }
                     TC *c = cw + off;
                     if constexpr (sizeof(TC) == 4) {
                         if (!LA_DEV_BIT(epi, 2 << 16) || v[0] == 12345.678f)
@@ -192,7 +210,7 @@
             f32x4 v = *reinterpret_cast<const f32x4 *>(reg + rl * PITCH + r * 16);
             float2 st = make_float2(0.f, 0.f);
             if constexpr (LNM == 2) st = stats[min(m, p.M - 1)];
-            if constexpr (LNM == 4 || LNM == 6) st = stats_tab[wrow0 - tile_m0 + h * 32 + rl];
+            if constexpr (LNM == 4 || LNM == 6 || LNM == 7) st = stats_tab[wrow0 - tile_m0 + h * 32 + rl];
             if constexpr (LNM == 5) {
                 const int src = (((h * 32 + it * 4) & 63) + q) * 4;
                 const float2 sr = h * 32 >= 64 ? sr1 : sr0;
@@ -202,6 +220,20 @@
             epi_quad<OUT_F32, EQ>(v, b4, cs4, st, has_bias, do_gelu, epi);
             if (m >= p.M || n >= p.N) continue;
             const int nv = min(4, p.N - n);
+            if constexpr (LNM == 7) {
+                ushort4 ph, pl;
+                x2_split_pair(v[0] * st.x, ph.x, pl.x); x2_split_pair(v[1] * st.x, ph.y, pl.y);
+                x2_split_pair(v[2] * st.x, ph.z, pl.z); x2_split_pair(v[3] * st.x, ph.w, pl.w);
+                unsigned short *c = PL + (int64_t)m * p.ldc + n;
+                if (fast_c && nv == 4) {
+                    *reinterpret_cast<ushort4 *>(c) = ph;
+                    *reinterpret_cast<ushort4 *>(c + plane_c) = pl;
+                } else {
+                    const unsigned short hh[4] = {ph.x, ph.y, ph.z, ph.w}, ll[4] = {pl.x, pl.y, pl.z, pl.w};
+                    for (int j = 0; j < nv; ++j) { c[j] = hh[j]; c[plane_c + j] = ll[j]; }
+                }
+                continue;
+            }
             if (do_res) {
                 const float *rr = R + (int64_t)m * p.ldr + n;
                 if (LNM == 6 && (epi & LA_EPI_RES_GELU_GRAD)) {
diff --git a/lyricalignment_amd/csrc/la_gemm_params.h b/lyricalignment_amd/csrc/la_gemm_params.h
--- a/lyricalignment_amd/csrc/la_gemm_params.h
+++ b/lyricalignment_amd/csrc/la_gemm_params.h
@@ -26,6 +26,7 @@
     int K_tail = 0;
     int64_t plane_a = 0, plane_w = 0;
     float *ln_part = nullptr;
+    const float *out_inv = nullptr;
 };
 
 constexpr int LA_EPI_SPLIT_INPLACE = 1 << 20;
@@ -37,6 +38,7 @@
 int launch_split_bf16(GemmParams p, int batch, hipStream_t stream);
 int launch_split_f16(GemmParams p, int batch, hipStream_t stream);
 int launch_x2_f16(GemmParams p, int batch, hipStream_t stream);
+int launch_x2_planes_f16(GemmParams p, hipStream_t stream);
 
 #ifdef LA_EXPERIMENTS
 bool lab_try_launch(GemmParams &p, int batch, bool out_f32, int lnm, bool duo, hipStream_t stream, int *rc);
diff --git a/lyricalignment_amd/csrc/la_gemm_pp_f16.hip b/lyricalignment_amd/csrc/la_gemm_pp_f16.hip
--- a/lyricalignment_amd/csrc/la_gemm_pp_f16.hip
+++ b/lyricalignment_amd/csrc/la_gemm_pp_f16.hip
@@ -14,5 +14,7 @@
 
 int launch_x2_f16(GemmParams p, int batch, hipStream_t stream) { return launch_pp_loop<true, true, la::f16_t, 6>(p, batch, stream); }
 
+int launch_x2_planes_f16(GemmParams p, hipStream_t stream) { return launch_pp_loop<true, true, la::f16_t, 7>(p, 1, stream); }
+
 }
 }
diff --git a/lyricalignment_amd/csrc/la_gemm_pp_kernel.h b/lyricalignment_amd/csrc/la_gemm_pp_kernel.h
--- a/lyricalignment_amd/csrc/la_gemm_pp_kernel.h
+++ b/lyricalignment_amd/csrc/la_gemm_pp_kernel.h
@@ -36,13 +36,19 @@
     const int ncol = min(n0 + wc * 64 + lane, p.N - 1);
     const float bias_l = has_bias ? bias[ncol] : 0.f;
     float csum_l = 0.f;
-    if constexpr (LNM == 2 || LNM == 4 || LNM == 6) csum_l = p.ln_csum[ncol];
+    if constexpr (LNM == 2 || LNM == 4 || LNM == 6 || LNM == 7) csum_l = p.ln_csum[ncol];
     float2 st_pre = make_float2(0.f, 1.f);
     if constexpr (LNM == 2) {
         if (lane < 32) st_pre = reinterpret_cast<const float2 *>(p.ln_stats)[min(m0 + wr * 128 + wc * 32 + lane, p.M - 1)];
     }
     if constexpr (LNM == 6) {
         if (lane < 32) st_pre = make_float2(0.f, p.ln_stats[min(m0 + wr * 128 + wc * 32 + lane, p.M - 1)]);
+    }
+    if constexpr (LNM == 7) {
+        if (lane < 32) {
+            const int row = min(m0 + wr * 128 + wc * 32 + lane, p.M - 1);
+            st_pre = make_float2(1.0f / p.out_inv[row], p.ln_stats[row]);
+        }
     }
 
     f32x4 acc[8][4];
@@ -72,15 +78,15 @@
             const float var = fmaxf(fmaf(-mean, mean, s2 * inv_k), 0.f);
             if (lane < 16) stats_tab[wr * 128 + (2 * wc + i) * 16 + lane] = make_float2(mean, 1.0f / sqrtf(var + 1e-5f));
         }
-    } else if constexpr (LNM == 6) {
-        static_assert(DUO || LNM != 6, "the segmented-K loop is the hand-placed one");
+    } else if constexpr (LNM == 6 || LNM == 7) {
+        static_assert(DUO || (LNM != 6 && LNM != 7), "the segmented-K loop is the hand-placed one");
         mainloop_duo_seg_asm<T16>(A, p.lda, p.M, W, p.ldw, p.N, p.K, p.plane_a, p.plane_w, m0, n0, lds, acc);
     } else if constexpr (DUO) {
         mainloop_duo_asm<T16>(A, p.lda, p.M, W, p.ldw, p.N, p.K, m0, n0, lds, acc LA_STAMP_ARG);
     } else {
         mainloop_pp<T16>(A, p.lda, p.M, W, p.ldw, p.N, p.K, m0, n0, lds, acc);
     }
-    if constexpr (LNM == 2 || LNM == 6) {
+    if constexpr (LNM == 2 || LNM == 6 || LNM == 7) {
         if (lane < 32) stats_tab[wr * 128 + wc * 32 + lane] = st_pre;
     }
 #ifdef LA_TILE_STAMPS
@@ -116,11 +122,11 @@
     p.tiles_m = la::cdiv(p.M, PP::TM);
     p.tiles_n = la::cdiv(p.N, PP::TN);
     p.group = la::dev_env("LA_GEMM_GROUP") ? std::min(p.group, p.tiles_n) : std::min(p.tiles_n, std::max(4, p.group / 2));
-    p.mblock = p.tiles_n > p.group ? (LNM == 6 ? 8 : 32) : 0;
+    p.mblock = p.tiles_n > p.group ? (LNM >= 6 ? 8 : 32) : 0;
     if (const char *g = la::dev_env("LA_GEMM_MBLOCK")) p.mblock = atoi(g);
     if (const char *g = la::dev_env("LA_GELU_PK")) p.epilogue |= atoi(g) == 2 ? 8192 : 4096;
     if (const char *g = la::dev_env("LA_EPI_PROBE")) p.epilogue |= (atoi(g) & 7) << 16;
-    la::TimerScope ts(LNM == 6 ? "gemm_f16x2" : "gemm_bf16", stream, 2.0 * p.M * p.N * p.K * batch);
+    la::TimerScope ts(LNM >= 6 ? "gemm_f16x2" : "gemm_bf16", stream, 2.0 * p.M * p.N * p.K * batch);
     hipLaunchKernelGGL(kern, dim3(p.tiles_m * p.tiles_n, batch), dim3(PP::THREADS), PP::LDS, stream, p);
     LA_LAUNCH_CHECK();
     return LA_OK;
diff --git a/lyricalignment_amd/csrc/la_model.cpp b/lyricalignment_amd/csrc/la_model.cpp
--- a/lyricalignment_amd/csrc/la_model.cpp
+++ b/lyricalignment_amd/csrc/la_model.cpp
@@ -21,7 +21,7 @@
     void *rows0, *y1, *h, *qkv, *att, *u;
     float *x, *stats;
     void *pl_d = nullptr, *pl_u = nullptr, *attn_ws = nullptr;
-    float *inv = nullptr;
+    float *inv = nullptr, *inv_u = nullptr;
     size_t attn_ws_bytes = 0;
     size_t total;
 };
@@ -44,6 +44,13 @@
             const float *residual, int64_t ldr, int epilogue, hipStream_t stream) {
     if (x2_big_ok(M, N, K)) return la_gemm_f16x2(M, N, K, 1, A, sa, W, sw, C, ldc, bias, residual, ldr, epilogue, stream);
     return la_gemm_f16x2_small(M, N, K, 0, A, sa, W, sw, C, ldc, bias, residual, ldr, epilogue, stream);
+}
+
+bool encoder_x2_planes_out(const la_encoder_weights *w, int batch) {
+    if (!la::opts().x2_planes_out || !(w->dtype & LA_X2_BOUNDS) || !w->x2_bounds) return false;
+    for (int l = 0; l < w->n_layer; ++l)
+        if (!(w->x2_bounds[2 * l] > 0.f) || !(w->x2_bounds[2 * l + 1] >= 0.f)) return false;
+    return x2_big_ok((int64_t)batch * N_CTX, w->d, w->d);
 }
 
 EncBufs carve_encoder(void *ws, int dtype, int batch, int d, bool x2 = false, int n_head = 0) {
@@ -64,6 +71,7 @@
         b.pl_d = c.take(M * 2 * d * 2);
         b.pl_u = c.take(M * 2 * 4 * d * 2);
         b.inv = static_cast<float *>(c.take(M * 4));
+        b.inv_u = static_cast<float *>(c.take(M * 4));
         la_attention_f16x2_workspace_bytes(batch, N_CTX, N_CTX, n_head, &b.attn_ws_bytes);
         b.attn_ws = c.take(b.attn_ws_bytes);
     }
@@ -98,13 +106,15 @@
     hipStream_t stream = (hipStream_t)stream_;
     if (batch == 0) return LA_OK;
     LA_CHECK_ARG(w && mel && out && workspace && batch > 0, "encoder_forward: null pointer / bad batch");
-    LA_CHECK_ARG(((w->dtype & 0xff) == LA_F32 && !(w->dtype & LA_Q_LOG2)) || (w->dtype & ~LA_Q_LOG2) == LA_BF16 || (w->dtype & ~LA_Q_LOG2) == LA_F16,
+    const int wdt = w->dtype & ~LA_X2_BOUNDS;
+    LA_CHECK_ARG(((wdt & 0xff) == LA_F32 && !(wdt & LA_Q_LOG2)) || (wdt & ~LA_Q_LOG2) == LA_BF16 || (wdt & ~LA_Q_LOG2) == LA_F16,
                  "encoder_forward: bad compute dtype");
     LA_CHECK_ARG(w->d > 0 && w->d % 64 == 0 && w->n_head * 64 == w->d, "encoder_forward: kernels are built for head_dim 64 (d = %d, heads = %d)", w->d, w->n_head);
     LA_CHECK_ARG(w->n_mels > 0 && w->n_mels <= C_PAD && w->n_layer >= 0 && (w->n_layer == 0 || w->blocks), "encoder_forward: bad dimensions");
     LA_CHECK_ARG((uintptr_t)workspace % 256 == 0, "encoder_forward: workspace must be 256-byte aligned");
-    const int dt = w->dtype & 0xff, dt_attn = w->dtype, d = w->d, M = batch * N_CTX;
+    const int dt = w->dtype & 0xff, dt_attn = wdt, d = w->d, M = batch * N_CTX;
     const bool x2 = encoder_x2(w, batch);
+    const bool planes_out = x2 && encoder_x2_planes_out(w, batch);
     const EncBufs b = carve_encoder(workspace, dt, batch, d, x2, w->n_head);
     LA_CHECK_ARG(workspace_bytes >= b.total, "encoder_forward: workspace too small (%zu < %zu)", workspace_bytes, b.total);
     const size_t es = esize(dt);
@@ -158,6 +168,15 @@
             float *qkv = static_cast<float *>(b.qkv), *att = static_cast<float *>(b.att), *u = static_cast<float *>(b.u);
             LA_TRY(la_layernorm_f16x2(b.x, d, M, d, k.ln1_g, k.ln1_b, b.pl_d, d, b.inv, stream));
             LA_TRY(x2_gemm(M, 3 * d, d, b.pl_d, b.inv, k.wqkv_x2, k.wqkv_x2s, qkv, 3 * d, k.bqkv, nullptr, 0, LA_EPI_BIAS, stream));
+            if (planes_out) {
+                LA_TRY(la_attention_f16x2_planes(qkv, 3 * d, qkv + d, qkv + 2 * d, 3 * d, b.pl_d, b.inv, batch, N_CTX, N_CTX, w->n_head, 0, b.attn_ws,
+                                                 b.attn_ws_bytes, stream));
+                LA_TRY(x2_gemm(M, d, d, b.pl_d, b.inv, k.wo_x2, k.wo_x2s, b.x, d, k.bo, b.x, d, LA_EPI_BIAS | LA_EPI_RESIDUAL, stream));
+                LA_TRY(la_layernorm_f16x2_bound(b.x, d, M, d, k.ln2_g, k.ln2_b, b.pl_d, d, b.inv, w->x2_bounds[2 * l], w->x2_bounds[2 * l + 1], b.inv_u, stream));
+                LA_TRY(la_gemm_f16x2_planes(M, 4 * d, d, b.pl_d, b.inv, k.w1_x2, k.w1_x2s, b.pl_u, 4 * d, b.inv_u, k.b1, LA_EPI_BIAS | LA_EPI_GELU, stream));
+                LA_TRY(x2_gemm(M, d, 4 * d, b.pl_u, b.inv_u, k.w2_x2, k.w2_x2s, b.x, d, k.b2, b.x, d, LA_EPI_BIAS | LA_EPI_RESIDUAL, stream));
+                continue;
+            }
             LA_TRY(la_attention_lse_f16x2(qkv, 3 * d, qkv + d, qkv + 2 * d, 3 * d, att, d, batch, N_CTX, N_CTX, w->n_head, 0, nullptr, b.attn_ws,
                                           b.attn_ws_bytes, stream));
             LA_TRY(la_split_f16x2(att, d, M, d, b.pl_d, d, b.inv, stream));
diff --git a/lyricalignment_amd/csrc/la_runtime.cpp b/lyricalignment_amd/csrc/la_runtime.cpp
--- a/lyricalignment_amd/csrc/la_runtime.cpp
+++ b/lyricalignment_amd/csrc/la_runtime.cpp
@@ -54,6 +54,7 @@
     {"viterbi_dpp", "LA_VITERBI_NO_DPP", &Options::viterbi_dpp, true}, {"head_clip_cap", "LA_HEAD_CLIP_CAP", &Options::head_clip_cap, false},
     {"ln_fusion", "LA_LN_FUSION", &Options::ln_fusion, false},       {"resid_split", "LA_RESID_SPLIT", &Options::resid_split, false},
     {"x2_inference", "LA_X2_INFERENCE", &Options::x2_inference, false}, {"x2_small", "LA_X2_SMALL", &Options::x2_small, false},
+    {"x2_planes_out", "LA_X2_PLANES_OUT", &Options::x2_planes_out, false},
     {"gru_timeout_us", "LA_GRU_TIMEOUT_US", &Options::gru_timeout_us, false}, {"gru_fault_step", "LA_GRU_FAULT_STEP", &Options::gru_fault_step, false},
 };
 }
diff --git a/lyricalignment_amd/engine.py b/lyricalignment_amd/engine.py
--- a/lyricalignment_amd/engine.py
+++ b/lyricalignment_amd/engine.py
@@ -37,6 +37,7 @@
     wqkv_ln: Optional[torch.Tensor] = None; cqkv: Optional[torch.Tensor] = None; bqkv_ln: Optional[torch.Tensor] = None
     w1_ln: Optional[torch.Tensor] = None; c1: Optional[torch.Tensor] = None; b1_ln: Optional[torch.Tensor] = None
     x2: Optional[List[Tuple[torch.Tensor, torch.Tensor]]] = None
+    x2_bound: Optional[Tuple[float, float]] = None
 
 
 def _x2_planes(w: torch.Tensor) -> Tuple[torch.Tensor, torch.Tensor]:
@@ -53,6 +54,10 @@
 
 def _x2_domain(M: int, N: int, K: int) -> bool:
     return K % 128 == 0 and K >= 256 and N > 128 and -(-M // 256) * -(-N // 256) >= 192
+
+
+def x2_planes_out_on() -> bool:
+    return _lib.get_option("x2_planes_out") != 0
 
 
 def x2_small_on() -> bool:
@@ -146,6 +151,8 @@
             g(b + "mlp.2.weight").detach().to(device=device, dtype=dtype).contiguous(), _f32(g(b + "mlp.2.bias"), device))
         if dtype == torch.float32 and X2_PACK and d % 128 == 0 and d >= 256 and torch.device(device).type == "cuda":
             blk.x2 = [_x2_planes(t) for t in (blk.wqkv, blk.wo, blk.w1, blk.w2)]
+            w1_64 = blk.w1.detach().double()
+            blk.x2_bound = (float(w1_64.pow(2).sum(dim=1).sqrt().max()), float(blk.b1.detach().abs().max()))
         if dtype in (torch.bfloat16, torch.float16):
             blk.wqkv_ln, blk.cqkv, blk.bqkv_ln = _fold_ln(wqkv, bqkv, g(b + "attn_ln.weight"), g(b + "attn_ln.bias"), dtype, device)
             blk.w1_ln, blk.c1, blk.b1_ln = _fold_ln(g(b + "mlp.0.weight"), g(b + "mlp.0.bias"), g(b + "mlp_ln.weight"),
@@ -267,6 +274,11 @@
         c = _lib.EncoderWeightsC(_lib.dtype_code(e.dtype) | (_lib.LA_Q_LOG2 if e.q_log2 else 0), e.d, e.n_head, len(e.blocks), e.n_mels, P(e.conv1_w), P(e.conv1_b), P(e.conv2_w),
                                  P(e.conv2_b), P(e.pos), P(e.lnp_g), P(e.lnp_b), blocks)
         c._keep = blocks
+        if e.blocks and all(b.x2_bound is not None for b in e.blocks):
+            bounds = (ctypes.c_float * (2 * len(e.blocks)))(*[v for b in e.blocks for v in b.x2_bound])
+            c.x2_bounds = ctypes.cast(bounds, ctypes.POINTER(ctypes.c_float))
+            c.dtype |= _lib.LA_X2_BOUNDS
+            c._keep_bounds = bounds
         return c
 
     @staticmethod
@@ -360,9 +372,15 @@
               and (-(-M // 256) * -(-d // 256) >= 192 or (x2_small_on() and d % 32 == 0))):
             from . import f32x2
             pl = lambda t: f32x2.Planes(t[0], t[1], t[0].shape[0], t[0].shape[2], t[0].shape[2])
+            planes_out = (x2_planes_out_on() and all(b_.x2_bound is not None and b_.x2_bound[0] > 0 for b_ in e.blocks) and _x2_domain(M, d, d))
             for blk in e.blocks:
                 wq, wo_, w1_, w2_ = (pl(t) for t in blk.x2)
                 _x2_gemm(f32x2.layernorm_split(x, blk.ln1_g, blk.ln1_b), wq, out=qkv, bias=blk.bqkv)
+                if planes_out:
+                    _x2_gemm(f32x2.attention_planes(qkv[:, :d], qkv[:, d:2 * d], qkv[:, 2 * d:], B, N_CTX, N_CTX, e.n_head), wo_, out=x, bias=blk.bo, residual=x)
+                    a2, inv_u = f32x2.layernorm_split_bound(x, blk.ln2_g, blk.ln2_b, *blk.x2_bound)
+                    _x2_gemm(f32x2.gemm_planes(a2, w1_, inv_u, bias=blk.b1, gelu=True), w2_, out=x, bias=blk.b2, residual=x)
+                    continue
                 ops.attention_ex(qkv[:, :d], qkv[:, d:2 * d], qkv[:, 2 * d:], B, N_CTX, N_CTX, e.n_head, out=att, x2=True)
                 _x2_gemm(f32x2.split(att, d), wo_, out=x, bias=blk.bo, residual=x)
                 _x2_gemm(f32x2.layernorm_split(x, blk.ln2_g, blk.ln2_b), w1_, out=u, bias=blk.b1)
diff --git a/lyricalignment_amd/f32x2.py b/lyricalignment_amd/f32x2.py
--- a/lyricalignment_amd/f32x2.py
+++ b/lyricalignment_amd/f32x2.py
@@ -71,6 +71,51 @@
     check(lib().la_layernorm_f16x2(ptr(x), x.stride(0), rows, d, ptr(gamma.contiguous()), ptr(beta.contiguous()), ptr(planes), kp, ptr(inv), stream_ptr()),
           "layernorm_f16x2")
     return Planes(planes, inv, rows, d, kp)
+
+
+def layernorm_split_bound(x: torch.Tensor, gamma: torch.Tensor, beta: torch.Tensor, wmax: float, bmax: float):
+    if x.dtype != torch.float32 or x.dim() != 2 or x.stride(1) != 1:
+        raise ValueError("f32x2.layernorm_split_bound: a float32 [rows, d] row view is expected")
+    rows, d = x.shape
+    planes = torch.empty((rows, 2, d), dtype=torch.float16, device=x.device)
+    inv = torch.empty((rows,), dtype=torch.float32, device=x.device)
+    inv_out = torch.empty((rows,), dtype=torch.float32, device=x.device)
+    check(lib().la_layernorm_f16x2_bound(ptr(x), x.stride(0), rows, d, ptr(gamma.contiguous()), ptr(beta.contiguous()), ptr(planes), d, ptr(inv),
+                                         float(wmax), float(bmax), ptr(inv_out), stream_ptr()), "layernorm_f16x2_bound")
+    return Planes(planes, inv, rows, d, d), inv_out
+
+
+def gemm_planes(a: Planes, w: Planes, inv_out: torch.Tensor, bias: Optional[torch.Tensor] = None, gelu: bool = False) -> Planes:
+    if a.kp != w.kp:
+        raise ValueError(f"f32x2.gemm_planes: operands were split to different plane lengths ({a.kp}, {w.kp})")
+    M, N = a.rows, w.rows
+    if inv_out.dtype != torch.float32 or inv_out.numel() != M or not inv_out.is_contiguous():
+        raise ValueError("f32x2.gemm_planes: inv_out is [rows] float32")
+    out = torch.empty((M, 2, N), dtype=torch.float16, device=a.planes.device)
+    epi = (_lib.EPI_BIAS if bias is not None else 0) | (_lib.EPI_GELU if gelu else 0)
+    check(lib().la_gemm_f16x2_planes(M, N, a.kp, ptr(a.planes), ptr(a.inv_scale), ptr(w.planes), ptr(w.inv_scale), ptr(out), N, ptr(inv_out),
+                                     ptr(bias), epi, stream_ptr()), "gemm_f16x2_planes")
+    return Planes(out, inv_out, M, N, N)
+
+
+def attention_planes(q: torch.Tensor, k: torch.Tensor, v: torch.Tensor, batch: int, q_len: int, kv_len: int, n_head: int,
+                     causal: bool = False) -> Planes:
+    import ctypes
+    d = n_head * 64
+    for t in (q, k, v):
+        if t.dtype != torch.float32 or t.dim() != 2 or t.stride(1) != 1 or t.shape[1] < d:
+            raise ValueError("f32x2.attention_planes: float32 row views of at least 64 n_head columns are expected")
+    if k.stride(0) != v.stride(0) or q.shape[0] < batch * q_len or k.shape[0] < batch * kv_len or v.shape[0] < batch * kv_len:
+        raise ValueError("f32x2.attention_planes: inconsistent views")
+    planes = torch.empty((batch * q_len, 2, d), dtype=torch.float16, device=q.device)
+    inv = torch.empty((batch * q_len,), dtype=torch.float32, device=q.device)
+    need = ctypes.c_size_t(0)
+    check(lib().la_attention_f16x2_workspace_bytes(batch, q_len, kv_len, n_head, ctypes.byref(need)), "attention_f16x2_workspace_bytes")
+    ws = torch.empty((need.value + 256,), dtype=torch.uint8, device=q.device)
+    off = (-ws.data_ptr()) % 256
+    check(lib().la_attention_f16x2_planes(ptr(q), q.stride(0), ptr(k), ptr(v), k.stride(0), ptr(planes), ptr(inv), batch, q_len, kv_len, n_head,
+                                          1 if causal else 0, ws.data_ptr() + off, need.value, stream_ptr()), "attention_f16x2_planes")
+    return Planes(planes, inv, batch * q_len, d, d)
 
 
 def split_t(x: torch.Tensor, mp: Optional[int] = None, act: Optional[str] = None, colsum: Optional[torch.Tensor] = None,
```

Result: no change. 23620 audio-sec/sec, median of 2 (-0.1%).
